# snarkify/sirius

Measured on AMD Instinct MI355X. Metric: IVC fold-steps/s (CycleFold IVC::next hot path, Poseidon-shaped synthetic trace, 2^k rows), higher is better.
Workload: dtype u256 (modular; 9 x 29-bit / 8 x 32-bit limbs)

## Files before the change

include/sirius_amd.h:

```cpp
#ifndef SIRIUS_AMD_H
#define SIRIUS_AMD_H

#include <stddef.h>
#include <stdint.h>

#ifdef __cplusplus
extern "C" {
#endif

typedef struct { uint64_t l[4]; } srs_fe;
typedef struct { srs_fe x, y; } srs_affine;

typedef struct srs_ck srs_ck;
typedef struct srs_structure srs_structure;

enum {
    SRS_OK = 0,
    SRS_ERR_TOO_LONG_INPUT = 1,
    SRS_ERR_NOT_POW2 = 2,
    SRS_ERR_K_TOO_LARGE = 3,
    SRS_ERR_INVALID = 4,
    SRS_ERR_DEVICE = 5,
    SRS_ERR_LAYOUT = 6,
    SRS_ERR_EVAL_INDEX = 7,
    SRS_ERR_IO = 8,
    SRS_ERR_INVALID_DATA = 9,
    SRS_ERR_UNSUPPORTED = 10
};

enum { SRS_CURVE_BN256 = 0, SRS_CURVE_GRUMPKIN = 1 };
enum { SRS_FIELD_FR = 0, SRS_FIELD_FQ = 1 };
enum { SRS_SPACE_HOST = 0, SRS_SPACE_DEVICE = 1 };
enum { SRS_REPR_MONT = 0, SRS_REPR_CANON = 1 };

int srs_init(int device_ordinal);
int srs_init_thread(int device_ordinal);
const char *srs_last_error(void);
const char *srs_version(void);
int srs_tuning_set(const char *name, int64_t value);
int srs_tuning_get(const char *name, int64_t *value);
void srs_tuning_reset(void);
const char *srs_tuning_name(int index);
int srs_scalar_field_of(int curve);
int srs_layout_selftest(int field, const srs_fe *one, const srs_fe *two);
int srs_layout_selftest_point(int curve, const srs_affine *generator);

int srs_dev_alloc(size_t bytes, void **out);
void srs_dev_free(void *p);
int srs_host_alloc(size_t bytes, void **out);
void srs_host_free(void *p);
int srs_upload(void *dst_dev, const void *src_host, size_t bytes, void *stream);
int srs_download(void *dst_host, const void *src_dev, size_t bytes, void *stream);

int srs_ck_create(int curve, const srs_affine *bases, size_t len, int space, srs_ck **out);
int srs_ck_create_sharded(int curve, const srs_affine *bases, size_t len, int space,
                          uint32_t rank, uint32_t world, srs_ck **out);
int srs_ck_setup_synthetic(int curve, size_t len, uint64_t seed, uint32_t rank, uint32_t world, srs_ck **out);
int srs_ck_setup_uniform_bytes(const uint8_t *label, size_t label_len, size_t first, size_t count, uint8_t *out);
int srs_ck_setup(int curve, uint32_t k, const uint8_t *label, size_t label_len, srs_ck **out);
int srs_ck_get_bases(const srs_ck *ck, srs_affine *out);
size_t srs_ck_local_len(const srs_ck *ck);
int srs_ck_load_file(int curve, const char *path, size_t k, uint32_t rank, uint32_t world, srs_ck **out);
int srs_ck_save_file(const srs_ck *ck, const char *path);
int srs_ck_count_off_curve(const srs_ck *ck, size_t *bad);
void srs_ck_free(srs_ck *ck);
size_t srs_ck_len(const srs_ck *ck);

int srs_commit(srs_ck *ck, const srs_fe *scalars, size_t n, int space, int repr, void *stream,
               srs_affine *out);
int srs_commit_batch(srs_ck *ck, const srs_fe *const *scalars, const size_t *n, size_t batch,
                     int space, int repr, void *stream, srs_affine *out);
int srs_commit_upload(srs_ck *ck, const srs_fe *scalars_host, size_t n, srs_fe *dev_copy, int repr, void *stream,
                      srs_affine *out);

size_t srs_concat_len(const size_t *lens, size_t n_columns, size_t pad_size);
int srs_concat_with_padding(srs_fe *out_dev, const srs_fe *const *columns_host, const size_t *lens, size_t n_columns, size_t pad_size,
                            void *stream);
int srs_commit_upload_columns(srs_ck *ck, const srs_fe *const *columns_host, const size_t *lens, size_t n_columns, size_t pad_size,
                              srs_fe *dev_copy, int repr, void *stream, srs_affine *out);

int srs_ck_create_multi(int curve, const srs_affine *bases, size_t len, int space, int n_devices, srs_ck **out);
int srs_ck_setup_synthetic_multi(int curve, size_t len, uint64_t seed, int n_devices, srs_ck **out);
int srs_ck_num_shards(const srs_ck *ck);
int srs_ck_msm_stats(const srs_ck *ck, uint64_t *out4);
int srs_ck_has_wide_table(const srs_ck *ck);
int srs_ck_is_compact(const srs_ck *ck);
size_t srs_ck_table_bytes(const srs_ck *ck);
int srs_glv_constants(int curve, srs_fe *lambda, srs_fe *beta);
int srs_glv_decompose(int curve, const srs_fe *k, int repr, srs_fe *k1_abs, srs_fe *k2_abs, int *neg1, int *neg2);
int srs_ck_shard_stats(const srs_ck *ck, int shard, uint64_t *out4);

int srs_point_sum(int curve, const srs_affine *points, size_t n, srs_affine *out);
int srs_point_mul(int curve, const srs_fe *scalar, int repr, const srs_affine *p, srs_affine *out);
int srs_point_lincomb(int curve, const srs_affine *acc, const srs_affine *points, const srs_fe *scalars, size_t n,
                      int repr, srs_affine *out);
int srs_fe_powers(int field, const srs_fe *r, size_t n, srs_fe *out);
int srs_point_lincomb_async(int curve, const srs_affine *acc, const srs_affine *points, const srs_fe *scalars, size_t n,
                            int repr, srs_affine *out, uint64_t *job);
int srs_job_wait(uint64_t job);

void srs_profile_enable(int on);
void srs_profile_reset(void);
void srs_profile_sampling(unsigned every);
int srs_profile_get(const char *name, double *total_ms, uint64_t *launches, uint64_t *units);

int srs_ntt(int field, srs_fe *a, size_t n, int inverse, int coset, int space, void *stream);
int srs_ntt_batch(int field, srs_fe *a, size_t n, size_t stride, size_t batch, int inverse, int coset,
                  int space, void *stream);
int srs_ntt_set_max_radix_bits(int bits);

enum { SRS_EX_CONST = 0, SRS_EX_POLY = 1, SRS_EX_CHALLENGE = 2, SRS_EX_NEG = 3, SRS_EX_SUM = 4,
       SRS_EX_PRODUCT = 5, SRS_EX_SCALED = 6, SRS_EX_END = 7 };
int srs_structure_create(int field, uint32_t k, size_t num_selectors, size_t num_fixed, size_t num_advice,
                         const uint8_t *const *selectors, const srs_fe *const *fixed, int space,
                         const uint64_t *gates, size_t gates_words, size_t num_gates, srs_structure **out);
int srs_structure_create_lookup(int field, uint32_t k, size_t num_selectors, size_t num_fixed, size_t num_advice,
                                const uint8_t *const *selectors, const srs_fe *const *fixed, int space,
                                const uint64_t *gates, size_t gates_words, size_t num_gates,
                                size_t num_lookups, int has_vector_lookup,
                                const uint64_t *lookup_exprs, size_t lookup_words, srs_structure **out);
void srs_structure_free(srs_structure *S);
int srs_structure_set_shard(srs_structure *S, uint32_t rank, uint32_t world);
int srs_structure_upload_shard_halo(const srs_structure *S, const srs_fe *witness_host, srs_fe *dev_copy, size_t n, int reference_compat,
                                    void *stream);
size_t srs_structure_num_witness_columns(const srs_structure *S);
size_t srs_structure_num_cross_terms(const srs_structure *S);
size_t srs_structure_num_challenges(const srs_structure *S);
size_t srs_structure_program_source(srs_structure *S, int which, char *buf, size_t cap, uint64_t *fingerprint, int *spec_id);
enum { SRS_KERNEL_INTERPRETER = 0, SRS_KERNEL_AHEAD_OF_TIME = 1, SRS_KERNEL_RUNTIME_COMPILED = 2 };
int srs_structure_kernel_kind(const srs_structure *S, int which);
int srs_jit_selfcheck(size_t *code_bytes, char *log, size_t log_cap);

int srs_cross_terms(srs_structure *S, const srs_fe *W1, const srs_fe *W2, const srs_fe *challenges,
                    size_t n_challenges, int space, void *stream, srs_fe *const *T_out);
int srs_commit_cross_terms(srs_structure *S, srs_ck *ck, const srs_fe *W1, const srs_fe *W2,
                           const srs_fe *challenges, size_t n_challenges, int space, void *stream,
                           srs_fe *const *T_out, srs_affine *commits_out);
int srs_eval_gates(srs_structure *S, int homogeneous, const srs_fe *W, const srs_fe *challenges,
                   size_t n_challenges, int space, void *stream, srs_fe *out);

int srs_is_sat_gates(srs_structure *S, int homogeneous, const srs_fe *W, const srs_fe *challenges, size_t n_challenges,
                     const srs_fe *E, int space, void *stream, size_t *mismatch_count);

typedef struct srs_poseidon srs_poseidon;
int srs_poseidon_new(int field, size_t t, size_t rate, size_t r_f, size_t r_p, srs_poseidon **out);
void srs_poseidon_free(srs_poseidon *H);
void srs_poseidon_reset(srs_poseidon *H);
int srs_poseidon_absorb_field(srs_poseidon *H, const srs_fe *v, size_t n);
int srs_poseidon_absorb_point(srs_poseidon *H, int curve, const srs_affine *p);
int srs_poseidon_squeeze(srs_poseidon *H, size_t num_bits, int out_field, srs_fe *out);
int srs_poseidon_squeeze_device(srs_poseidon *H, size_t num_bits, int out_field, srs_fe *out, double *kernel_ms);

typedef struct srs_sparse srs_sparse;
int srs_sparse_create(int field, size_t n, const uint64_t *rows, const uint64_t *cols, const srs_fe *values, size_t nnz,
                      srs_sparse **out);
void srs_sparse_free(srs_sparse *M);
int srs_sparse_matvec(srs_sparse *M, const srs_fe *Z, int space, void *stream, srs_fe *y);
int srs_is_sat_permutation(srs_sparse *M, const srs_fe *Z, int space, void *stream, size_t *mismatch_count);
int srs_is_sat_witness_commit(srs_ck *ck, const srs_fe *const *W, const size_t *n, size_t n_rounds,
                              const srs_affine *W_commitments, const srs_fe *E, size_t n_E, const srs_affine *E_commitment,
                              int space, void *stream, size_t *w_mismatch_count, int *e_mismatch);

int srs_lookup_coeff_1(srs_structure *S, const srs_fe *advice, const srs_fe *r, int space, void *stream,
                       srs_fe *const *ls, srs_fe *const *ts, srs_fe *const *ms);
int srs_lookup_coeff_2(int field, const srs_fe *l, const srs_fe *t, const srs_fe *m, const srs_fe *r, size_t n,
                       int space, void *stream, srs_fe *h, srs_fe *g);
int srs_is_sat_log_derivative(srs_structure *S, const srs_fe *W, int space, void *stream, size_t *mismatch_count);
int srs_batch_invert_assigned(int field, const srs_fe *numerators, const srs_fe *denominators, const uint8_t *has_denominator,
                              size_t n, int space, void *stream, srs_fe *out);

int srs_fold_witness(int field, srs_fe *out, const srs_fe *w1, const srs_fe *w2, const srs_fe *r, size_t n,
                     int space, void *stream);
int srs_fold_error(int field, srs_fe *out, const srs_fe *e, const srs_fe *const *T, size_t n_terms,
                   const srs_fe *r, size_t n, int space, void *stream);

int srs_sangria_prove(srs_structure *S, srs_ck *ck, srs_poseidon *ro, const srs_fe *challenges, size_t n_challenges, srs_fe *W1, const srs_fe *W2,
                      srs_fe *E, void *stream, srs_fe *r_io, srs_fe *const *T_dev, srs_affine *cross_term_commits,
                      const srs_affine *W_commitments, const srs_affine *E_commitment, srs_affine *folded_commitments, uint64_t *jobs);

int srs_sangria_prove_incoming(srs_structure *S, srs_ck *ck, srs_poseidon *ro, const srs_fe *challenges, size_t n_challenges, srs_fe *W1, srs_fe *W2,
                               const srs_fe *W2_host, const srs_fe *u2_tail, size_t n_u2_tail, srs_fe *E, void *stream, srs_fe *r_io,
                               srs_fe *const *T_dev, srs_affine *cross_term_commits, srs_affine *W_commitments, const srs_affine *E_commitment,
                               srs_affine *folded_commitments, uint64_t *jobs);

typedef struct {
    size_t count_of_evaluation_with_padding;
    size_t betas_count;
    size_t fft_points_count_F;
    size_t fft_points_count_G;
    size_t instances_to_fold;
    size_t lagrange_domain;
    uint32_t fft_log_domain_size_K;
} srs_pg_context;
int srs_pg_context_new(const srs_structure *S, size_t traces_len, srs_pg_context *out);
int srs_pg_prove(srs_structure *S, srs_poseidon *ro, const srs_fe *betas, size_t n_betas, const srs_fe *delta,
                 const srs_fe *const *W, const srs_fe *const *challenges, size_t n_challenges, size_t n_instances, int reference_compat,
                 void *stream, srs_fe *alpha_gamma, srs_fe *poly_F, srs_fe *poly_K, srs_fe *betas_stroke, srs_fe *e, srs_fe *lagrange,
                 srs_fe *W_folded);
int srs_pg_beta_stroke(const srs_fe *betas, size_t n, const srs_fe *alpha, const srs_fe *delta, srs_fe *out);
int srs_pg_compute_F(srs_structure *S, const srs_fe *betas, size_t n_betas, const srs_fe *delta, const srs_fe *W,
                     const srs_fe *challenges, size_t n_challenges, int space, int reference_compat, void *stream,
                     srs_fe *poly_F);
int srs_pg_compute_G(srs_structure *S, const srs_fe *betas_stroke, size_t n_betas, const srs_fe *const *W,
                     const srs_fe *const *challenges, size_t n_challenges, size_t n_instances, int space,
                     int reference_compat, void *stream, srs_fe *poly_G);
int srs_pg_compute_K_from_G(const srs_fe *poly_G, size_t n_G, const srs_fe *poly_F_in_alpha, size_t instances_to_fold,
                            uint32_t fft_log_domain_size_K, void *stream, srs_fe *poly_K);
int srs_pg_evaluate_e(srs_structure *S, const srs_fe *betas, size_t n_betas, const srs_fe *W, const srs_fe *challenges,
                      size_t n_challenges, int space, int reference_compat, void *stream, srs_fe *e);
int srs_pg_closed_form(const srs_fe *gate_values, size_t n_gates, uint32_t k, const srs_fe *weights, size_t n_weights,
                       const srs_fe *delta, srs_fe *out);
int srs_pg_calculate_e(const srs_fe *poly_F, size_t n_F, const srs_fe *poly_K, size_t n_K, const srs_fe *gamma,
                       const srs_fe *alpha, uint32_t log_n, srs_fe *out);
int srs_lagrange_eval(const srs_fe *X, uint32_t log_n, srs_fe *out);
int srs_poly_eval(const srs_fe *coeffs, size_t n, const srs_fe *x, srs_fe *out);
int srs_fold_lincomb(int field, srs_fe *out, const srs_fe *const *W, const srs_fe *coefs, size_t J, size_t n,
                     int space, void *stream);
int srs_fold_lincomb_sharded(int field, srs_fe *out, const srs_fe *const *W, const srs_fe *coefs, size_t J, size_t n, uint32_t rank,
                             uint32_t world, void *stream);
int srs_structure_fold_sharded(srs_structure *S, srs_fe *out, const srs_fe *const *W, const srs_fe *coefs, size_t J, int reference_compat,
                               void *stream);

#ifdef __cplusplus
}
#endif
#endif
```

shim/src/sys.rs:

```rust
#![allow(non_camel_case_types, non_snake_case, dead_code)]
use std::os::raw::{c_char, c_int, c_void};

#[repr(C)] #[derive(Clone, Copy, Debug, PartialEq, Eq)] pub struct srs_fe { pub l: [u64; 4] }
#[repr(C)] #[derive(Clone, Copy, Debug, PartialEq, Eq)] pub struct srs_affine { pub x: srs_fe, pub y: srs_fe }
#[repr(C)] pub struct srs_ck { _opaque: [u8; 0] }
#[repr(C)] pub struct srs_structure { _opaque: [u8; 0] }
#[repr(C)] pub struct srs_poseidon { _opaque: [u8; 0] }
#[repr(C)] pub struct srs_sparse { _opaque: [u8; 0] }
#[repr(C)] #[derive(Clone, Copy, Debug, Default)] pub struct srs_pg_context { pub count_of_evaluation_with_padding: usize, pub betas_count: usize, pub fft_points_count_F: usize, pub fft_points_count_G: usize, pub instances_to_fold: usize, pub lagrange_domain: usize, pub fft_log_domain_size_K: u32 }

pub const SRS_OK: c_int = 0;
pub const SRS_ERR_TOO_LONG_INPUT: c_int = 1;
pub const SRS_ERR_NOT_POW2: c_int = 2;
pub const SRS_ERR_K_TOO_LARGE: c_int = 3;
pub const SRS_ERR_INVALID: c_int = 4;
pub const SRS_ERR_DEVICE: c_int = 5;
pub const SRS_ERR_LAYOUT: c_int = 6;
pub const SRS_ERR_EVAL_INDEX: c_int = 7;
pub const SRS_ERR_IO: c_int = 8;
pub const SRS_ERR_INVALID_DATA: c_int = 9;
pub const SRS_ERR_UNSUPPORTED: c_int = 10;
pub const SRS_CURVE_BN256: c_int = 0;
pub const SRS_CURVE_GRUMPKIN: c_int = 1;
pub const SRS_FIELD_FR: c_int = 0;
pub const SRS_FIELD_FQ: c_int = 1;
pub const SRS_SPACE_HOST: c_int = 0;
pub const SRS_SPACE_DEVICE: c_int = 1;
pub const SRS_REPR_MONT: c_int = 0;
pub const SRS_REPR_CANON: c_int = 1;
pub const SRS_EX_CONST: c_int = 0;
pub const SRS_EX_POLY: c_int = 1;
pub const SRS_EX_CHALLENGE: c_int = 2;
pub const SRS_EX_NEG: c_int = 3;
pub const SRS_EX_SUM: c_int = 4;
pub const SRS_EX_PRODUCT: c_int = 5;
pub const SRS_EX_SCALED: c_int = 6;
pub const SRS_EX_END: c_int = 7;
pub const SRS_KERNEL_INTERPRETER: c_int = 0;
pub const SRS_KERNEL_AHEAD_OF_TIME: c_int = 1;
pub const SRS_KERNEL_RUNTIME_COMPILED: c_int = 2;

#[link(name = "sirius_amd")]
extern "C" {
    pub fn srs_init(device_ordinal: c_int) -> c_int;
    pub fn srs_init_thread(device_ordinal: c_int) -> c_int;
    pub fn srs_last_error() -> *const c_char;
    pub fn srs_version() -> *const c_char;
    pub fn srs_tuning_set(name: *const c_char, value: int64_t) -> c_int;
    pub fn srs_tuning_get(name: *const c_char, value: *mut int64_t) -> c_int;
    pub fn srs_tuning_reset();
    pub fn srs_tuning_name(index: c_int) -> *const c_char;
    pub fn srs_scalar_field_of(curve: c_int) -> c_int;
    pub fn srs_layout_selftest(field: c_int, one: *const srs_fe, two: *const srs_fe) -> c_int;
    pub fn srs_layout_selftest_point(curve: c_int, generator: *const srs_affine) -> c_int;
    pub fn srs_dev_alloc(bytes: usize, out: *mut *mut c_void) -> c_int;
    pub fn srs_dev_free(p: *mut c_void);
    pub fn srs_host_alloc(bytes: usize, out: *mut *mut c_void) -> c_int;
    pub fn srs_host_free(p: *mut c_void);
    pub fn srs_upload(dst_dev: *mut c_void, src_host: *const c_void, bytes: usize, stream: *mut c_void) -> c_int;
    pub fn srs_download(dst_host: *mut c_void, src_dev: *const c_void, bytes: usize, stream: *mut c_void) -> c_int;
    pub fn srs_ck_create(curve: c_int, bases: *const srs_affine, len: usize, space: c_int, out: *mut *mut srs_ck) -> c_int;
    pub fn srs_ck_create_sharded(curve: c_int, bases: *const srs_affine, len: usize, space: c_int, rank: u32, world: u32, out: *mut *mut srs_ck) -> c_int;
    pub fn srs_ck_setup_synthetic(curve: c_int, len: usize, seed: u64, rank: u32, world: u32, out: *mut *mut srs_ck) -> c_int;
    pub fn srs_ck_setup_uniform_bytes(label: *const u8, label_len: usize, first: usize, count: usize, out: *mut u8) -> c_int;
    pub fn srs_ck_setup(curve: c_int, k: u32, label: *const u8, label_len: usize, out: *mut *mut srs_ck) -> c_int;
    pub fn srs_ck_get_bases(ck: *const srs_ck, out: *mut srs_affine) -> c_int;
    pub fn srs_ck_local_len(ck: *const srs_ck) -> usize;
    pub fn srs_ck_load_file(curve: c_int, path: *const c_char, k: usize, rank: u32, world: u32, out: *mut *mut srs_ck) -> c_int;
    pub fn srs_ck_save_file(ck: *const srs_ck, path: *const c_char) -> c_int;
    pub fn srs_ck_count_off_curve(ck: *const srs_ck, bad: *mut usize) -> c_int;
    pub fn srs_ck_free(ck: *mut srs_ck);
    pub fn srs_ck_len(ck: *const srs_ck) -> usize;
    pub fn srs_commit(ck: *mut srs_ck, scalars: *const srs_fe, n: usize, space: c_int, repr: c_int, stream: *mut c_void, out: *mut srs_affine) -> c_int;
    pub fn srs_commit_batch(ck: *mut srs_ck, scalars: *const *const srs_fe, n: *const usize, batch: usize, space: c_int, repr: c_int, stream: *mut c_void, out: *mut srs_affine) -> c_int;
    pub fn srs_commit_upload(ck: *mut srs_ck, scalars_host: *const srs_fe, n: usize, dev_copy: *mut srs_fe, repr: c_int, stream: *mut c_void, out: *mut srs_affine) -> c_int;
    pub fn srs_concat_len(lens: *const usize, n_columns: usize, pad_size: usize) -> usize;
    pub fn srs_concat_with_padding(out_dev: *mut srs_fe, columns_host: *const *const srs_fe, lens: *const usize, n_columns: usize, pad_size: usize, stream: *mut c_void) -> c_int;
    pub fn srs_commit_upload_columns(ck: *mut srs_ck, columns_host: *const *const srs_fe, lens: *const usize, n_columns: usize, pad_size: usize, dev_copy: *mut srs_fe, repr: c_int, stream: *mut c_void, out: *mut srs_affine) -> c_int;
    pub fn srs_ck_create_multi(curve: c_int, bases: *const srs_affine, len: usize, space: c_int, n_devices: c_int, out: *mut *mut srs_ck) -> c_int;
    pub fn srs_ck_setup_synthetic_multi(curve: c_int, len: usize, seed: u64, n_devices: c_int, out: *mut *mut srs_ck) -> c_int;
    pub fn srs_ck_num_shards(ck: *const srs_ck) -> c_int;
    pub fn srs_ck_msm_stats(ck: *const srs_ck, out4: *mut u64) -> c_int;
    pub fn srs_ck_has_wide_table(ck: *const srs_ck) -> c_int;
    pub fn srs_ck_is_compact(ck: *const srs_ck) -> c_int;
    pub fn srs_ck_table_bytes(ck: *const srs_ck) -> usize;
    pub fn srs_glv_constants(curve: c_int, lambda: *mut srs_fe, beta: *mut srs_fe) -> c_int;
    pub fn srs_glv_decompose(curve: c_int, k: *const srs_fe, repr: c_int, k1_abs: *mut srs_fe, k2_abs: *mut srs_fe, neg1: *mut c_int, neg2: *mut c_int) -> c_int;
    pub fn srs_ck_shard_stats(ck: *const srs_ck, shard: c_int, out4: *mut u64) -> c_int;
    pub fn srs_point_sum(curve: c_int, points: *const srs_affine, n: usize, out: *mut srs_affine) -> c_int;
    pub fn srs_point_mul(curve: c_int, scalar: *const srs_fe, repr: c_int, p: *const srs_affine, out: *mut srs_affine) -> c_int;
    pub fn srs_point_lincomb(curve: c_int, acc: *const srs_affine, points: *const srs_affine, scalars: *const srs_fe, n: usize, repr: c_int, out: *mut srs_affine) -> c_int;
    pub fn srs_fe_powers(field: c_int, r: *const srs_fe, n: usize, out: *mut srs_fe) -> c_int;
    pub fn srs_point_lincomb_async(curve: c_int, acc: *const srs_affine, points: *const srs_affine, scalars: *const srs_fe, n: usize, repr: c_int, out: *mut srs_affine, job: *mut u64) -> c_int;
    pub fn srs_job_wait(job: u64) -> c_int;
    pub fn srs_profile_enable(on: c_int);
    pub fn srs_profile_reset();
    pub fn srs_profile_sampling(every: unsigned);
    pub fn srs_profile_get(name: *const c_char, total_ms: *mut f64, launches: *mut u64, units: *mut u64) -> c_int;
    pub fn srs_ntt(field: c_int, a: *mut srs_fe, n: usize, inverse: c_int, coset: c_int, space: c_int, stream: *mut c_void) -> c_int;
    pub fn srs_ntt_batch(field: c_int, a: *mut srs_fe, n: usize, stride: usize, batch: usize, inverse: c_int, coset: c_int, space: c_int, stream: *mut c_void) -> c_int;
    pub fn srs_ntt_set_max_radix_bits(bits: c_int) -> c_int;
    pub fn srs_structure_create(field: c_int, k: u32, num_selectors: usize, num_fixed: usize, num_advice: usize, selectors: *const *const u8, fixed: *const *const srs_fe, space: c_int, gates: *const u64, gates_words: usize, num_gates: usize, out: *mut *mut srs_structure) -> c_int;
    pub fn srs_structure_create_lookup(field: c_int, k: u32, num_selectors: usize, num_fixed: usize, num_advice: usize, selectors: *const *const u8, fixed: *const *const srs_fe, space: c_int, gates: *const u64, gates_words: usize, num_gates: usize, num_lookups: usize, has_vector_lookup: c_int, lookup_exprs: *const u64, lookup_words: usize, out: *mut *mut srs_structure) -> c_int;
    pub fn srs_structure_free(S: *mut srs_structure);
    pub fn srs_structure_set_shard(S: *mut srs_structure, rank: u32, world: u32) -> c_int;
    pub fn srs_structure_upload_shard_halo(S: *const srs_structure, witness_host: *const srs_fe, dev_copy: *mut srs_fe, n: usize, reference_compat: c_int, stream: *mut c_void) -> c_int;
    pub fn srs_structure_num_witness_columns(S: *const srs_structure) -> usize;
    pub fn srs_structure_num_cross_terms(S: *const srs_structure) -> usize;
    pub fn srs_structure_num_challenges(S: *const srs_structure) -> usize;
    pub fn srs_structure_program_source(S: *mut srs_structure, which: c_int, buf: *mut c_char, cap: usize, fingerprint: *mut u64, spec_id: *mut c_int) -> usize;
    pub fn srs_structure_kernel_kind(S: *const srs_structure, which: c_int) -> c_int;
    pub fn srs_jit_selfcheck(code_bytes: *mut usize, log: *mut c_char, log_cap: usize) -> c_int;
    pub fn srs_cross_terms(S: *mut srs_structure, W1: *const srs_fe, W2: *const srs_fe, challenges: *const srs_fe, n_challenges: usize, space: c_int, stream: *mut c_void, T_out: *const *mut srs_fe) -> c_int;
    pub fn srs_commit_cross_terms(S: *mut srs_structure, ck: *mut srs_ck, W1: *const srs_fe, W2: *const srs_fe, challenges: *const srs_fe, n_challenges: usize, space: c_int, stream: *mut c_void, T_out: *const *mut srs_fe, commits_out: *mut srs_affine) -> c_int;
    pub fn srs_eval_gates(S: *mut srs_structure, homogeneous: c_int, W: *const srs_fe, challenges: *const srs_fe, n_challenges: usize, space: c_int, stream: *mut c_void, out: *mut srs_fe) -> c_int;
    pub fn srs_is_sat_gates(S: *mut srs_structure, homogeneous: c_int, W: *const srs_fe, challenges: *const srs_fe, n_challenges: usize, E: *const srs_fe, space: c_int, stream: *mut c_void, mismatch_count: *mut usize) -> c_int;
    pub fn srs_poseidon_new(field: c_int, t: usize, rate: usize, r_f: usize, r_p: usize, out: *mut *mut srs_poseidon) -> c_int;
    pub fn srs_poseidon_free(H: *mut srs_poseidon);
    pub fn srs_poseidon_reset(H: *mut srs_poseidon);
    pub fn srs_poseidon_absorb_field(H: *mut srs_poseidon, v: *const srs_fe, n: usize) -> c_int;
    pub fn srs_poseidon_absorb_point(H: *mut srs_poseidon, curve: c_int, p: *const srs_affine) -> c_int;
    pub fn srs_poseidon_squeeze(H: *mut srs_poseidon, num_bits: usize, out_field: c_int, out: *mut srs_fe) -> c_int;
    pub fn srs_poseidon_squeeze_device(H: *mut srs_poseidon, num_bits: usize, out_field: c_int, out: *mut srs_fe, kernel_ms: *mut f64) -> c_int;
    pub fn srs_sparse_create(field: c_int, n: usize, rows: *const u64, cols: *const u64, values: *const srs_fe, nnz: usize, out: *mut *mut srs_sparse) -> c_int;
    pub fn srs_sparse_free(M: *mut srs_sparse);
    pub fn srs_sparse_matvec(M: *mut srs_sparse, Z: *const srs_fe, space: c_int, stream: *mut c_void, y: *mut srs_fe) -> c_int;
    pub fn srs_is_sat_permutation(M: *mut srs_sparse, Z: *const srs_fe, space: c_int, stream: *mut c_void, mismatch_count: *mut usize) -> c_int;
    pub fn srs_is_sat_witness_commit(ck: *mut srs_ck, W: *const *const srs_fe, n: *const usize, n_rounds: usize, W_commitments: *const srs_affine, E: *const srs_fe, n_E: usize, E_commitment: *const srs_affine, space: c_int, stream: *mut c_void, w_mismatch_count: *mut usize, e_mismatch: *mut c_int) -> c_int;
    pub fn srs_lookup_coeff_1(S: *mut srs_structure, advice: *const srs_fe, r: *const srs_fe, space: c_int, stream: *mut c_void, ls: *const *mut srs_fe, ts: *const *mut srs_fe, ms: *const *mut srs_fe) -> c_int;
    pub fn srs_lookup_coeff_2(field: c_int, l: *const srs_fe, t: *const srs_fe, m: *const srs_fe, r: *const srs_fe, n: usize, space: c_int, stream: *mut c_void, h: *mut srs_fe, g: *mut srs_fe) -> c_int;
    pub fn srs_is_sat_log_derivative(S: *mut srs_structure, W: *const srs_fe, space: c_int, stream: *mut c_void, mismatch_count: *mut usize) -> c_int;
    pub fn srs_batch_invert_assigned(field: c_int, numerators: *const srs_fe, denominators: *const srs_fe, has_denominator: *const u8, n: usize, space: c_int, stream: *mut c_void, out: *mut srs_fe) -> c_int;
    pub fn srs_fold_witness(field: c_int, out: *mut srs_fe, w1: *const srs_fe, w2: *const srs_fe, r: *const srs_fe, n: usize, space: c_int, stream: *mut c_void) -> c_int;
    pub fn srs_fold_error(field: c_int, out: *mut srs_fe, e: *const srs_fe, T: *const *const srs_fe, n_terms: usize, r: *const srs_fe, n: usize, space: c_int, stream: *mut c_void) -> c_int;
    pub fn srs_sangria_prove(S: *mut srs_structure, ck: *mut srs_ck, ro: *mut srs_poseidon, challenges: *const srs_fe, n_challenges: usize, W1: *mut srs_fe, W2: *const srs_fe, E: *mut srs_fe, stream: *mut c_void, r_io: *mut srs_fe, T_dev: *const *mut srs_fe, cross_term_commits: *mut srs_affine, W_commitments: *const srs_affine, E_commitment: *const srs_affine, folded_commitments: *mut srs_affine, jobs: *mut u64) -> c_int;
    pub fn srs_sangria_prove_incoming(S: *mut srs_structure, ck: *mut srs_ck, ro: *mut srs_poseidon, challenges: *const srs_fe, n_challenges: usize, W1: *mut srs_fe, W2: *mut srs_fe, W2_host: *const srs_fe, u2_tail: *const srs_fe, n_u2_tail: usize, E: *mut srs_fe, stream: *mut c_void, r_io: *mut srs_fe, T_dev: *const *mut srs_fe, cross_term_commits: *mut srs_affine, W_commitments: *mut srs_affine, E_commitment: *const srs_affine, folded_commitments: *mut srs_affine, jobs: *mut u64) -> c_int;
    pub fn srs_pg_context_new(S: *const srs_structure, traces_len: usize, out: *mut srs_pg_context) -> c_int;
    pub fn srs_pg_prove(S: *mut srs_structure, ro: *mut srs_poseidon, betas: *const srs_fe, n_betas: usize, delta: *const srs_fe, W: *const *const srs_fe, challenges: *const *const srs_fe, n_challenges: usize, n_instances: usize, reference_compat: c_int, stream: *mut c_void, alpha_gamma: *mut srs_fe, poly_F: *mut srs_fe, poly_K: *mut srs_fe, betas_stroke: *mut srs_fe, e: *mut srs_fe, lagrange: *mut srs_fe, W_folded: *mut srs_fe) -> c_int;
    pub fn srs_pg_beta_stroke(betas: *const srs_fe, n: usize, alpha: *const srs_fe, delta: *const srs_fe, out: *mut srs_fe) -> c_int;
    pub fn srs_pg_compute_F(S: *mut srs_structure, betas: *const srs_fe, n_betas: usize, delta: *const srs_fe, W: *const srs_fe, challenges: *const srs_fe, n_challenges: usize, space: c_int, reference_compat: c_int, stream: *mut c_void, poly_F: *mut srs_fe) -> c_int;
    pub fn srs_pg_compute_G(S: *mut srs_structure, betas_stroke: *const srs_fe, n_betas: usize, W: *const *const srs_fe, challenges: *const *const srs_fe, n_challenges: usize, n_instances: usize, space: c_int, reference_compat: c_int, stream: *mut c_void, poly_G: *mut srs_fe) -> c_int;
    pub fn srs_pg_compute_K_from_G(poly_G: *const srs_fe, n_G: usize, poly_F_in_alpha: *const srs_fe, instances_to_fold: usize, fft_log_domain_size_K: u32, stream: *mut c_void, poly_K: *mut srs_fe) -> c_int;
    pub fn srs_pg_evaluate_e(S: *mut srs_structure, betas: *const srs_fe, n_betas: usize, W: *const srs_fe, challenges: *const srs_fe, n_challenges: usize, space: c_int, reference_compat: c_int, stream: *mut c_void, e: *mut srs_fe) -> c_int;
    pub fn srs_pg_closed_form(gate_values: *const srs_fe, n_gates: usize, k: u32, weights: *const srs_fe, n_weights: usize, delta: *const srs_fe, out: *mut srs_fe) -> c_int;
    pub fn srs_pg_calculate_e(poly_F: *const srs_fe, n_F: usize, poly_K: *const srs_fe, n_K: usize, gamma: *const srs_fe, alpha: *const srs_fe, log_n: u32, out: *mut srs_fe) -> c_int;
    pub fn srs_lagrange_eval(X: *const srs_fe, log_n: u32, out: *mut srs_fe) -> c_int;
    pub fn srs_poly_eval(coeffs: *const srs_fe, n: usize, x: *const srs_fe, out: *mut srs_fe) -> c_int;
    pub fn srs_fold_lincomb(field: c_int, out: *mut srs_fe, W: *const *const srs_fe, coefs: *const srs_fe, J: usize, n: usize, space: c_int, stream: *mut c_void) -> c_int;
    pub fn srs_fold_lincomb_sharded(field: c_int, out: *mut srs_fe, W: *const *const srs_fe, coefs: *const srs_fe, J: usize, n: usize, rank: u32, world: u32, stream: *mut c_void) -> c_int;
    pub fn srs_structure_fold_sharded(S: *mut srs_structure, out: *mut srs_fe, W: *const *const srs_fe, coefs: *const srs_fe, J: usize, reference_compat: c_int, stream: *mut c_void) -> c_int;
}
```

sirius_amd/_lib.py:

```python
import ctypes as C
import os

_HERE = os.path.dirname(os.path.abspath(__file__))
LIB_PATH = os.path.join(_HERE, "csrc", "libsirius_amd.so")

OK, ERR_TOO_LONG_INPUT, ERR_NOT_POW2, ERR_K_TOO_LARGE, ERR_INVALID, ERR_DEVICE, ERR_LAYOUT, ERR_EVAL_INDEX, ERR_IO, ERR_INVALID_DATA, ERR_UNSUPPORTED = range(11)
CURVE_BN256, CURVE_GRUMPKIN = 0, 1
FIELD_FR, FIELD_FQ = 0, 1
SPACE_HOST, SPACE_DEVICE = 0, 1
REPR_MONT, REPR_CANON = 0, 1

_lib = None


class SiriusAmdError(RuntimeError):
    def __init__(self, rc, msg):
        super().__init__(f"sirius_amd rc={rc}: {msg}")
        self.rc = rc


def _prototypes():
    vp, sz, i32, u32 = C.c_void_p, C.c_size_t, C.c_int, C.c_uint32
    return {
        "srs_init": (i32, [i32]),
        "srs_init_thread": (i32, [i32]),
        "srs_last_error": (C.c_char_p, []),
        "srs_version": (C.c_char_p, []),
        "srs_tuning_set": (i32, [C.c_char_p, C.c_int64]),
        "srs_tuning_get": (i32, [C.c_char_p, C.POINTER(C.c_int64)]),
        "srs_tuning_reset": (None, []),
        "srs_tuning_name": (C.c_char_p, [i32]),
        "srs_scalar_field_of": (i32, [i32]),
        "srs_layout_selftest": (i32, [i32, vp, vp]),
        "srs_layout_selftest_point": (i32, [i32, vp]),
        "srs_dev_alloc": (i32, [sz, C.POINTER(vp)]),
        "srs_dev_free": (None, [vp]),
        "srs_host_alloc": (i32, [sz, C.POINTER(vp)]),
        "srs_host_free": (None, [vp]),
        "srs_upload": (i32, [vp, vp, sz, vp]),
        "srs_download": (i32, [vp, vp, sz, vp]),
        "srs_commit_upload": (i32, [vp, vp, sz, vp, i32, vp, vp]),
        "srs_concat_len": (sz, [C.POINTER(sz), sz, sz]),
        "srs_concat_with_padding": (i32, [vp, C.POINTER(vp), C.POINTER(sz), sz, sz, vp]),
        "srs_commit_upload_columns": (i32, [vp, C.POINTER(vp), C.POINTER(sz), sz, sz, vp, i32, vp, vp]),
        "srs_ck_create_multi": (i32, [i32, vp, sz, i32, i32, C.POINTER(vp)]),
        "srs_ck_setup_synthetic_multi": (i32, [i32, sz, C.c_uint64, i32, C.POINTER(vp)]),
        "srs_ck_num_shards": (i32, [vp]),
        "srs_ck_msm_stats": (i32, [vp, C.POINTER(C.c_uint64)]),
        "srs_ck_has_wide_table": (i32, [vp]),
        "srs_ck_is_compact": (i32, [vp]),
        "srs_ck_table_bytes": (sz, [vp]),
        "srs_glv_constants": (i32, [i32, vp, vp]),
        "srs_glv_decompose": (i32, [i32, vp, i32, vp, vp, C.POINTER(i32), C.POINTER(i32)]),
        "srs_ck_shard_stats": (i32, [vp, i32, C.POINTER(C.c_uint64)]),
        "srs_structure_kernel_kind": (i32, [vp, i32]),
        "srs_ck_create": (i32, [i32, vp, sz, i32, C.POINTER(vp)]),
        "srs_ck_create_sharded": (i32, [i32, vp, sz, i32, u32, u32, C.POINTER(vp)]),
        "srs_ck_setup_synthetic": (i32, [i32, sz, C.c_uint64, u32, u32, C.POINTER(vp)]),
        "srs_ck_setup_uniform_bytes": (i32, [C.c_char_p, sz, sz, sz, vp]),
        "srs_ck_setup": (i32, [i32, u32, C.c_char_p, sz, C.POINTER(vp)]),
        "srs_ck_get_bases": (i32, [vp, vp]),
        "srs_ck_local_len": (sz, [vp]),
        "srs_point_lincomb": (i32, [i32, vp, vp, vp, sz, i32, vp]),
        "srs_point_lincomb_async": (i32, [i32, vp, vp, vp, sz, i32, vp, C.POINTER(C.c_uint64)]),
        "srs_job_wait": (i32, [C.c_uint64]),
        "srs_fe_powers": (i32, [i32, vp, sz, vp]),
        "srs_jit_selfcheck": (i32, [C.POINTER(sz), C.c_char_p, sz]),
        "srs_profile_enable": (None, [i32]),
        "srs_profile_reset": (None, []),
        "srs_profile_sampling": (None, [C.c_uint]),
        "srs_profile_get": (i32, [C.c_char_p, C.POINTER(C.c_double), C.POINTER(C.c_uint64), C.POINTER(C.c_uint64)]),
        "srs_ck_load_file": (i32, [i32, C.c_char_p, sz, u32, u32, C.POINTER(vp)]),
        "srs_ck_save_file": (i32, [vp, C.c_char_p]),
        "srs_ck_count_off_curve": (i32, [vp, C.POINTER(sz)]),
        "srs_is_sat_gates": (i32, [vp, i32, vp, vp, sz, vp, i32, vp, C.POINTER(sz)]),
        "srs_ck_free": (None, [vp]),
        "srs_ck_len": (sz, [vp]),
        "srs_commit": (i32, [vp, vp, sz, i32, i32, vp, vp]),
        "srs_commit_batch": (i32, [vp, C.POINTER(vp), C.POINTER(sz), sz, i32, i32, vp, vp]),
        "srs_point_sum": (i32, [i32, vp, sz, vp]),
        "srs_point_mul": (i32, [i32, vp, i32, vp, vp]),
        "srs_structure_create": (i32, [i32, u32, sz, sz, sz, C.POINTER(vp), C.POINTER(vp), i32, vp, sz, sz, C.POINTER(vp)]),
        "srs_structure_create_lookup": (i32, [i32, u32, sz, sz, sz, C.POINTER(vp), C.POINTER(vp), i32, vp, sz, sz, sz, i32, vp, sz,
                                              C.POINTER(vp)]),
        "srs_structure_num_witness_columns": (sz, [vp]),
        "srs_lookup_coeff_1": (i32, [vp, vp, vp, i32, vp, C.POINTER(vp), C.POINTER(vp), C.POINTER(vp)]),
        "srs_lookup_coeff_2": (i32, [i32, vp, vp, vp, vp, sz, i32, vp, vp, vp]),
        "srs_is_sat_log_derivative": (i32, [vp, vp, i32, vp, C.POINTER(sz)]),
        "srs_sparse_create": (i32, [i32, sz, vp, vp, vp, sz, C.POINTER(vp)]),
        "srs_sparse_free": (None, [vp]),
        "srs_sparse_matvec": (i32, [vp, vp, i32, vp, vp]),
        "srs_is_sat_permutation": (i32, [vp, vp, i32, vp, C.POINTER(sz)]),
        "srs_is_sat_witness_commit": (i32, [vp, C.POINTER(vp), C.POINTER(sz), sz, vp, vp, sz, vp, i32, vp, C.POINTER(sz), C.POINTER(i32)]),
        "srs_structure_set_shard": (i32, [vp, u32, u32]),
        "srs_structure_upload_shard_halo": (i32, [vp, vp, vp, sz, i32, vp]),
        "srs_poseidon_new": (i32, [i32, sz, sz, sz, sz, C.POINTER(vp)]),
        "srs_poseidon_free": (None, [vp]),
        "srs_poseidon_reset": (None, [vp]),
        "srs_poseidon_absorb_field": (i32, [vp, vp, sz]),
        "srs_poseidon_absorb_point": (i32, [vp, i32, vp]),
        "srs_poseidon_squeeze": (i32, [vp, sz, i32, vp]),
        "srs_poseidon_squeeze_device": (i32, [vp, sz, i32, vp, C.POINTER(C.c_double)]),
        "srs_batch_invert_assigned": (i32, [i32, vp, vp, vp, sz, i32, vp, vp]),
        "srs_structure_free": (None, [vp]),
        "srs_structure_num_cross_terms": (sz, [vp]),
        "srs_structure_num_challenges": (sz, [vp]),
        "srs_structure_program_source": (sz, [vp, i32, vp, sz, C.POINTER(C.c_uint64), C.POINTER(i32)]),
        "srs_cross_terms": (i32, [vp, vp, vp, vp, sz, i32, vp, C.POINTER(vp)]),
        "srs_commit_cross_terms": (i32, [vp, vp, vp, vp, vp, sz, i32, vp, C.POINTER(vp), vp]),
        "srs_eval_gates": (i32, [vp, i32, vp, vp, sz, i32, vp, vp]),
        "srs_fold_witness": (i32, [i32, vp, vp, vp, vp, sz, i32, vp]),
        "srs_fold_error": (i32, [i32, vp, vp, C.POINTER(vp), sz, vp, sz, i32, vp]),
        "srs_pg_context_new": (i32, [vp, sz, vp]),
        "srs_pg_beta_stroke": (i32, [vp, sz, vp, vp, vp]),
        "srs_pg_prove": (i32, [vp, vp, vp, sz, vp, C.POINTER(vp), C.POINTER(vp), sz, sz, i32, vp, vp, vp, vp, vp, vp, vp, vp]),
        "srs_sangria_prove": (i32, [vp, vp, vp, vp, sz, vp, vp, vp, vp, vp, C.POINTER(vp), vp, vp, vp, vp, C.POINTER(C.c_uint64)]),
        "srs_sangria_prove_incoming": (i32, [vp, vp, vp, vp, sz, vp, vp, vp, vp, sz, vp, vp, vp, C.POINTER(vp), vp, vp, vp, vp,
                                             C.POINTER(C.c_uint64)]),
        "srs_pg_compute_F": (i32, [vp, vp, sz, vp, vp, vp, sz, i32, i32, vp, vp]),
        "srs_pg_compute_G": (i32, [vp, vp, sz, C.POINTER(vp), C.POINTER(vp), sz, sz, i32, i32, vp, vp]),
        "srs_pg_compute_K_from_G": (i32, [vp, sz, vp, sz, u32, vp, vp]),
        "srs_pg_evaluate_e": (i32, [vp, vp, sz, vp, vp, sz, i32, i32, vp, vp]),
        "srs_pg_closed_form": (i32, [vp, sz, u32, vp, sz, vp, vp]),
        "srs_pg_calculate_e": (i32, [vp, sz, vp, sz, vp, vp, u32, vp]),
        "srs_lagrange_eval": (i32, [vp, u32, vp]),
        "srs_poly_eval": (i32, [vp, sz, vp, vp]),
        "srs_fold_lincomb": (i32, [i32, vp, C.POINTER(vp), vp, sz, sz, i32, vp]),
        "srs_fold_lincomb_sharded": (i32, [i32, vp, C.POINTER(vp), vp, sz, sz, u32, u32, vp]),
        "srs_structure_fold_sharded": (i32, [vp, vp, vp, vp, sz, i32, vp]),
        "srs_ntt": (i32, [i32, vp, sz, i32, i32, i32, vp]),
        "srs_ntt_set_max_radix_bits": (i32, [i32]),
        "srs_ntt_batch": (i32, [i32, vp, sz, sz, sz, i32, i32, i32, vp]),
    }


def load(path=None):
    global _lib
    if _lib is not None and path is None:
        return _lib
    p = path or os.environ.get("SRS_AMD_LIB") or LIB_PATH
    if not os.path.exists(p):
        raise ImportError(
            f"{p} not found: build the HIP extension first (__graft_entry__.build()); "
            "sirius_amd has no CPU fallback")
    if path is None:
        try:
            import torch
        except Exception:
            pass
    lib = C.CDLL(p)
    for name, (res, args) in _prototypes().items():
        fn = getattr(lib, name)
        fn.restype = res
        fn.argtypes = args
    _lib = lib
    for item in filter(None, os.environ.get("SRS_TEST_TUNING", "").split(",")):
        name, _, value = item.partition("=")
        if lib.srs_tuning_set(name.strip().encode(), int(value)) != 0:
            raise ValueError(f"SRS_TEST_TUNING: unknown tunable {name!r}")
    return lib


def lib():
    return load()


def check(rc):
    if rc != OK:
        raise SiriusAmdError(rc, (lib().srs_last_error() or b"").decode())
```

sirius_amd/commitment.py:

```python
import ctypes as C

import numpy as np

from . import _lib as L


class TooLongInput(ValueError):

    def __init__(self, input_len, limit):
        super().__init__(f"Can't commit too long input: input len: {input_len}, but limit is {limit}")
        self.input_len, self.limit = input_len, limit


def _is_torch(x):
    return type(x).__module__.startswith("torch")


def _buf(x, last):
    if _is_torch(x):
        assert x.is_contiguous() and x.shape[-1] == last and x.element_size() == 8, (x.shape, x.dtype)
        space = L.SPACE_DEVICE if x.is_cuda else L.SPACE_HOST
        return x.data_ptr(), space, x.numel() // last, x
    a = np.ascontiguousarray(x, dtype=np.uint64)
    assert a.shape[-1] == last, a.shape
    return a.ctypes.data, L.SPACE_HOST, a.size // last, a


_torch_cuda = None


def _stream():
    global _torch_cuda
    if _torch_cuda is None:
        try:
            import torch
            if not torch.cuda.is_available():
                return None
            _torch_cuda = torch.cuda
        except Exception:
            return None
    return _torch_cuda.current_stream().cuda_stream


class CommitmentKey:

    def __init__(self, curve, bases, rank=0, world=1):
        addr, space, n, keep = _buf(bases, 8)
        self.curve, self._len = curve, n
        self.rank, self.world = rank, world
        h = C.c_void_p()
        L.check(L.lib().srs_ck_create_sharded(curve, addr, n, space, rank, world, C.byref(h)))
        self._h = h

    @classmethod
    def setup_synthetic(cls, curve, n, seed=0, rank=0, world=1):
        self = cls.__new__(cls)
        self.curve, self._len, self.rank, self.world = curve, n, rank, world
        h = C.c_void_p()
        L.check(L.lib().srs_ck_setup_synthetic(curve, n, seed, rank, world, C.byref(h)))
        self._h = h
        return self

    @staticmethod
    def setup_uniform_bytes(label, first, count):
        out = np.zeros((count, 32), dtype=np.uint8)
        L.check(L.lib().srs_ck_setup_uniform_bytes(bytes(label), len(label), first, count, out.ctypes.data))
        return out

    @classmethod
    def setup(cls, curve, k, label):
        assert k < 32
        h = C.c_void_p()
        L.check(L.lib().srs_ck_setup(curve, k, bytes(label), len(label), C.byref(h)))
        raise AssertionError("srs_ck_setup returned OK")

    @classmethod
    def create_multi(cls, curve, bases, n_devices=0):
        addr, space, n, keep = _buf(bases, 8)
        self = cls.__new__(cls)
        self.curve, self._len, self.rank, self.world = curve, n, 0, 1
        h = C.c_void_p()
        L.check(L.lib().srs_ck_create_multi(curve, addr, n, space, n_devices, C.byref(h)))
        self._h = h
        return self

    @classmethod
    def setup_synthetic_multi(cls, curve, n, seed=0, n_devices=0):
        self = cls.__new__(cls)
        self.curve, self._len, self.rank, self.world = curve, n, 0, 1
        h = C.c_void_p()
        L.check(L.lib().srs_ck_setup_synthetic_multi(curve, n, seed, n_devices, C.byref(h)))
        self._h = h
        return self

    @property
    def num_shards(self):
        return L.lib().srs_ck_num_shards(self._h)

    def msm_stats(self):
        out = (C.c_uint64 * 4)()
        L.check(L.lib().srs_ck_msm_stats(self._h, out))
        return dict(slot_sets=int(out[0]), hot_sets=int(out[1]), redo=int(out[2]), other_sets=int(out[3]))

    def shard_stats(self, shard):
        out = (C.c_uint64 * 4)()
        L.check(L.lib().srs_ck_shard_stats(self._h, shard, out))
        return dict(h2d_bytes=int(out[0]), peer_bytes=int(out[1]), streamed_commits=int(out[2]), device=int(out[3]))

    def has_wide_table(self):
        return bool(L.lib().srs_ck_has_wide_table(self._h))

    def is_compact(self):
        return bool(L.lib().srs_ck_is_compact(self._h))

    def table_bytes(self):
        return int(L.lib().srs_ck_table_bytes(self._h))

    @classmethod
    def load_from_file(cls, curve, file_path, k, rank=0, world=1):
        self = cls.__new__(cls)
        self.curve, self._len, self.rank, self.world = curve, 1 << k, rank, world
        h = C.c_void_p()
        rc = L.lib().srs_ck_load_file(curve, str(file_path).encode(), k, rank, world, C.byref(h))
        if rc == L.ERR_IO:
            raise IOError(L.lib().srs_last_error().decode())
        if rc == L.ERR_INVALID_DATA:
            raise ValueError(L.lib().srs_last_error().decode())
        L.check(rc)
        self._h = h
        return self

    def save_to_file(self, file_path):
        rc = L.lib().srs_ck_save_file(self._h, str(file_path).encode())
        if rc == L.ERR_IO:
            raise IOError(L.lib().srs_last_error().decode())
        L.check(rc)

    @classmethod
    def load_or_setup_cache(cls, curve, cache_folder, label, k, setup=None):
        import os
        path = os.path.join(str(cache_folder), label, f"{k}.bin")
        if os.path.exists(path):
            return cls.load_from_file(curve, path, k)
        if setup is None:
            raise FileNotFoundError(path)
        key = setup(k)
        os.makedirs(os.path.dirname(path), exist_ok=True)
        key.save_to_file(path)
        return key

    def count_off_curve(self):
        n = C.c_size_t()
        L.check(L.lib().srs_ck_count_off_curve(self._h, C.byref(n)))
        return n.value

    def bases(self):
        n = L.lib().srs_ck_local_len(self._h)
        out = np.zeros((n, 8), dtype=np.uint64)
        L.check(L.lib().srs_ck_get_bases(self._h, out.ctypes.data))
        return out

    def __len__(self):
        return self._len

    def close(self):
        if getattr(self, "_h", None):
            L.lib().srs_ck_free(self._h)
            self._h = None

    def __del__(self):
        try:
            self.close()
        except Exception:
            pass

    def commit(self, v, repr=L.REPR_MONT):
        addr, space, n, keep = _buf(v, 4)
        if n > self._len:
            raise TooLongInput(n, self._len)
        out = np.zeros(8, dtype=np.uint64)
        L.check(L.lib().srs_commit(self._h, addr, n, space, repr, _stream(), out.ctypes.data))
        return out

    def commit_upload(self, v_host, dev_copy=None, repr=L.REPR_MONT):
        a = np.ascontiguousarray(v_host, dtype=np.uint64)
        assert a.shape[-1] == 4
        n = a.size // 4
        if n > self._len:
            raise TooLongInput(n, self._len)
        dptr = None
        if dev_copy is not None:
            assert _is_torch(dev_copy) and dev_copy.is_contiguous() and dev_copy.numel() == 4 * n
            dptr = dev_copy.data_ptr()
        out = np.zeros(8, dtype=np.uint64)
        L.check(L.lib().srs_commit_upload(self._h, a.ctypes.data, n, dptr, repr, _stream(), out.ctypes.data))
        return out

    def commit_upload_columns(self, columns, pad_size, dev_copy=None, repr=L.REPR_MONT):
        cols = [np.ascontiguousarray(c, dtype=np.uint64).reshape(-1, 4) for c in columns]
        lens = (C.c_size_t * max(len(cols), 1))(*[c.shape[0] for c in cols])
        ptrs = (C.c_void_p * max(len(cols), 1))(*[c.ctypes.data for c in cols])
        n = L.lib().srs_concat_len(lens, len(cols), pad_size)
        if n > self._len:
            raise TooLongInput(n, self._len)
        dptr = None
        if dev_copy is not None:
            assert _is_torch(dev_copy) and dev_copy.is_contiguous() and dev_copy.numel() == 4 * n
            dptr = dev_copy.data_ptr()
        out = np.zeros(8, dtype=np.uint64)
        L.check(L.lib().srs_commit_upload_columns(self._h, ptrs, lens, len(cols), pad_size, dptr, repr, _stream(), out.ctypes.data))
        return out

    def commit_batch(self, vs, repr=L.REPR_MONT):
        bufs = [_buf(v, 4) for v in vs]
        if not bufs:
            return np.zeros((0, 8), dtype=np.uint64)
        spaces = {b[1] for b in bufs}
        assert len(spaces) == 1, "all vectors of a batch must live in the same memory space"
        for b in bufs:
            if b[2] > self._len:
                raise TooLongInput(b[2], self._len)
        ptrs = (C.c_void_p * len(bufs))(*[b[0] for b in bufs])
        ns = (C.c_size_t * len(bufs))(*[b[2] for b in bufs])
        out = np.zeros((len(bufs), 8), dtype=np.uint64)
        L.check(L.lib().srs_commit_batch(self._h, ptrs, ns, len(bufs), spaces.pop(), repr, _stream(), out.ctypes.data))
        return out


def point_sum(curve, points):
    a = np.ascontiguousarray(points, dtype=np.uint64).reshape(-1, 8)
    out = np.zeros(8, dtype=np.uint64)
    L.check(L.lib().srs_point_sum(curve, a.ctypes.data, a.shape[0], out.ctypes.data))
    return out


def point_lincomb(curve, acc, points, scalars, repr=L.REPR_MONT):
    pts = np.ascontiguousarray(points, dtype=np.uint64).reshape(-1, 8)
    sc = np.ascontiguousarray(scalars, dtype=np.uint64).reshape(-1, 4)
    assert pts.shape[0] == sc.shape[0]
    a = None if acc is None else np.ascontiguousarray(acc, dtype=np.uint64).reshape(8)
    out = np.zeros(8, dtype=np.uint64)
    L.check(L.lib().srs_point_lincomb(curve, None if a is None else a.ctypes.data, pts.ctypes.data, sc.ctypes.data,
                                      pts.shape[0], repr, out.ctypes.data))
    return out


class PendingPoint:

    def __init__(self, job, out, lib):
        self._job, self._out, self._lib = job, out, lib

    def wait(self):
        if self._job is not None:
            L.check(self._lib.srs_job_wait(self._job))
            self._job = None
# ... 61 lines not shown
```

sirius_amd/csrc/capi.hip:

```cpp
#include "../../include/sirius_amd.h"

#include <cstdio>
#include <cstring>
#include <deque>
#include <map>
#include <memory>
#include <set>
#include <thread>
#include <condition_variable>
#include <functional>
#include <mutex>
#include <atomic>
#include <chrono>
#include <string>
#include <vector>

#include "curve.cuh"
#include "decider.h"
#include "devrt.h"
#include "msm.h"
#include "ntt.h"
#include "poseidon.h"
#include "prof.h"
#include "rowprog.h"
// ... 624 lines not shown

static int read_shard_bases(const msm::Key &key, hipStream_t st, srs_affine *out) {
    if (!key.len) return SRS_OK;
    affine_t *tmp = nullptr;
    SRS_HIP_CHECK(hipMalloc((void **)&tmp, key.len * sizeof(affine_t)));
    try {
        msm::read_bases(key, tmp, st);
        SRS_HIP_CHECK(hipMemcpyAsync(out, tmp, key.len * sizeof(affine_t), hipMemcpyDeviceToHost, st));
        SRS_HIP_CHECK(hipStreamSynchronize(st));
    } catch (...) {
        (void)hipFree(tmp);
        throw;
    }
    (void)hipFree(tmp);
    return SRS_OK;
}

int srs_ck_get_bases(const srs_ck *ck, srs_affine *out) {
    if (!ck || ((ck->key.len || !ck->shards.empty()) && !out)) return fail(SRS_ERR_INVALID, "srs_ck_get_bases: bad argument");
    int rc = ensure_device();
    if (rc) return rc;
    if (!ck->shards.empty()) {
        return guarded([&]() -> int {
            const uint32_t world = (uint32_t)ck->shards.size();
            for (uint32_t d = 0; d < world; ++d) {
                CkShard *sh = ck->shards[d].get();
                std::vector<srs_affine> loc(sh->key.len);
                SRS_HIP_CHECK(hipSetDevice(sh->device));
                read_shard_bases(sh->key, sh->stream, loc.data());
                Stripes{d, world}.each_piece(0, ck->key.global_len, [&](size_t g, size_t l, size_t cnt) {
                    std::memcpy(out + g, loc.data() + l, cnt * sizeof(srs_affine));
                });
            }
            return ensure_device();
        });
    }
    return guarded([&]() -> int {
        if (ck->key.len) {
            affine_t *tmp = nullptr;
            SRS_HIP_CHECK(hipMalloc((void **)&tmp, ck->key.len * sizeof(affine_t)));
            try {
                msm::read_bases(ck->key, tmp, nullptr);
                SRS_HIP_CHECK(hipMemcpy(out, tmp, ck->key.len * sizeof(affine_t), hipMemcpyDeviceToHost));
            } catch (...) {
                (void)hipFree(tmp);
                throw;
            }
            (void)hipFree(tmp);
        }
        return SRS_OK;
    });
}
size_t srs_ck_local_len(const srs_ck *ck) { return ck ? (ck->shards.empty() ? ck->key.len : ck->key.global_len) : 0; }

int srs_ck_load_file(int curve, const char *path, size_t k, uint32_t rank, uint32_t world, srs_ck **out) {
    if (!valid_curve(curve) || !path || !out) return fail(SRS_ERR_INVALID, "srs_ck_load_file: bad argument");
    if (k > 27) return fail(SRS_ERR_INVALID, "srs_ck_load_file: key longer than 2^27 bases");
    const size_t len = (size_t)1 << k;
    std::vector<srs_affine> host;
    int rc = guarded([&]() -> int {
        host.resize(len);
        FILE *f = std::fopen(path, "rb");
        if (!f) return fail(SRS_ERR_IO, std::string("srs_ck_load_file: cannot open ") + path);
        size_t got = std::fread(host.data(), sizeof(srs_affine), len, f);
        std::fclose(f);
        if (got != len) return fail(SRS_ERR_IO, "srs_ck_load_file: failed to fill whole buffer");
        return SRS_OK;
    });
    if (rc) return rc;
    srs_ck *ck = nullptr;
    rc = srs_ck_create_sharded(curve, host.data(), len, SRS_SPACE_HOST, rank, world, &ck);
    if (rc) return rc;
    size_t bad = 0;
    rc = srs_ck_count_off_curve(ck, &bad);
    if (rc == SRS_OK && bad) rc = fail(SRS_ERR_INVALID_DATA, "Wrong file in cache, some ptr out of curve");
    if (rc) { srs_ck_free(ck); return rc; }
    *out = ck;
    return SRS_OK;
}

int srs_ck_save_file(const srs_ck *ck, const char *path) {
    if (!ck || !path) return fail(SRS_ERR_INVALID, "srs_ck_save_file: bad argument");
    if (ck->key.world != 1) return fail(SRS_ERR_INVALID, "srs_ck_save_file: sharded key");
    std::vector<srs_affine> host(srs_ck_local_len(ck));
    int rc = srs_ck_get_bases(ck, host.data());
    if (rc) return rc;
    FILE *f = std::fopen(path, "wb");
    if (!f) return fail(SRS_ERR_IO, std::string("srs_ck_save_file: cannot create ") + path);
    size_t put = std::fwrite(host.data(), sizeof(srs_affine), host.size(), f);
    int cl = std::fclose(f);
    if (put != host.size() || cl != 0) return fail(SRS_ERR_IO, "srs_ck_save_file: short write");
    return SRS_OK;
}

int srs_ck_count_off_curve(const srs_ck *ck, size_t *bad) {
    if (!ck || !bad) return fail(SRS_ERR_INVALID, "srs_ck_count_off_curve: bad argument");
    int rc = ensure_device();
    if (rc) return rc;
    return guarded([&]() -> int {
        if (ck->shards.empty()) {
            *bad = msm::count_off_curve(ck->key, nullptr);
            return SRS_OK;
        }
        size_t total = 0;
        for (auto &sp : ck->shards) {
            SRS_HIP_CHECK(hipSetDevice(sp->device));
            total += msm::count_off_curve(sp->key, sp->stream);
        }
        *bad = total;
        return ensure_device();
    });
}

int srs_ck_create(int curve, const srs_affine *bases, size_t len, int space, srs_ck **out) {
    return srs_ck_create_sharded(curve, bases, len, space, 0, 1, out);
}

int srs_ck_create_multi(int curve, const srs_affine *bases, size_t len, int space, int n_devices, srs_ck **out) {
    if (!valid_curve(curve) || !out || (!bases && len) || n_devices < 0) return fail(SRS_ERR_INVALID, "srs_ck_create_multi: bad argument");
    if (len > ((size_t)1 << 27)) return fail(SRS_ERR_INVALID, "srs_ck_create_multi: key longer than 2^27 bases");
    int rc = ensure_device();
    if (rc) return rc;
    return guarded([&]() -> int {
        return create_multi(curve, len, n_devices, [&](CkShard &sh) {
            const hipMemcpyKind kind = space == SRS_SPACE_DEVICE ? hipMemcpyDeviceToDevice : hipMemcpyHostToDevice;
            Stripes{sh.key.rank, sh.key.world}.each_piece(0, len, [&](size_t g, size_t l, size_t cnt) {
                SRS_HIP_CHECK(hipMemcpyAsync(sh.key.table + l, bases + g, cnt * sizeof(affine_t), kind, sh.stream));
            });
        }, out);
    });
}
int srs_ck_setup_synthetic_multi(int curve, size_t len, uint64_t seed, int n_devices, srs_ck **out) {
    if (!valid_curve(curve) || !out || n_devices < 0) return fail(SRS_ERR_INVALID, "srs_ck_setup_synthetic_multi: bad argument");
    if (len > ((size_t)1 << 27)) return fail(SRS_ERR_INVALID, "srs_ck_setup_synthetic_multi: key longer than 2^27 bases");
    int rc = ensure_device();
    if (rc) return rc;
    return guarded([&]() -> int {
        return create_multi(curve, len, n_devices, [&](CkShard &sh) { msm::generate_bases(sh.key, seed, sh.stream); }, out);
    });
}
int srs_ck_num_shards(const srs_ck *ck) { return ck ? (ck->shards.empty() ? 1 : (int)ck->shards.size()) : 0; }
int srs_ck_msm_stats(const srs_ck *ck, uint64_t *out) {
    if (!ck || !out) return fail(SRS_ERR_INVALID, "srs_ck_msm_stats: bad argument");
    for (int i = 0; i < 4; ++i) out[i] = 0;
    auto add = [&](const msm::Key &k) {
        out[0] += k.stat_slot_sets;
        out[1] += k.stat_hot_sets;
        out[2] += k.stat_redo;
        out[3] += k.stat_other_sets;
    };
    if (ck->shards.empty()) add(ck->key);
    for (const auto &sh : ck->shards) add(sh->key);
    return SRS_OK;
}

int srs_ck_shard_stats(const srs_ck *ck, int shard, uint64_t *out) {
    if (!ck || !out || shard < 0) return fail(SRS_ERR_INVALID, "srs_ck_shard_stats: bad argument");
    for (int i = 0; i < 4; ++i) out[i] = 0;
    if (ck->shards.empty()) {
        if (shard != 0) return fail(SRS_ERR_INVALID, "srs_ck_shard_stats: no such shard");
        out[3] = (uint64_t)home_device();
        return SRS_OK;
    }
    if ((size_t)shard >= ck->shards.size()) return fail(SRS_ERR_INVALID, "srs_ck_shard_stats: no such shard");
    const CkShard *sh = ck->shards[shard].get();
    out[0] = sh->stat_h2d_bytes;
    out[1] = sh->stat_peer_bytes;
    out[2] = sh->stat_streamed;
    out[3] = (uint64_t)sh->device;
    return SRS_OK;
}

int srs_ck_has_wide_table(const srs_ck *ck) {
    if (!ck) return 0;
    if (ck->shards.empty()) return ck->key.table_w != nullptr ? 1 : 0;
    for (const auto &sh : ck->shards)
        if (sh->key.len && !sh->key.table_w) return 0;
    return 1;
}

int srs_ck_is_compact(const srs_ck *ck) {
    if (!ck) return 0;
    if (ck->shards.empty()) return ck->key.compact ? 1 : 0;
    for (const auto &sh : ck->shards)
        if (!sh->key.compact) return 0;
    return 1;
}
size_t srs_ck_table_bytes(const srs_ck *ck) {
    if (!ck) return 0;
    if (ck->shards.empty()) return msm::table_bytes(ck->key);
    size_t total = 0;
    for (const auto &sh : ck->shards) total += msm::table_bytes(sh->key);
    return total;
}

int srs_glv_constants(int curve, srs_fe *lambda, srs_fe *beta) {
    if (!valid_curve(curve) || !lambda || !beta) return fail(SRS_ERR_INVALID, "srs_glv_constants: bad argument");
    auto go = [&](auto tag) {
        using K = GlvConsts<decltype(tag)::ID>;
        fe_t l, b;
        for (int i = 0; i < 8; ++i) {
            l.v[i] = K::lambda(i);
            b.v[i] = K::beta(i);
        }
        std::memcpy(lambda, &l, 32);
        std::memcpy(beta, &b, 32);
    };
    if (curve == SRS_CURVE_BN256) go(Bn256{}); else go(Grumpkin{});
    return SRS_OK;
}
int srs_glv_decompose(int curve, const srs_fe *k, int repr, srs_fe *k1_abs, srs_fe *k2_abs, int *neg1, int *neg2) {
    if (!valid_curve(curve) || !k || !k1_abs || !k2_abs || !neg1 || !neg2) return fail(SRS_ERR_INVALID, "srs_glv_decompose: bad argument");
    auto go = [&](auto tag) {
        using C = decltype(tag);
        fe_t s;
        std::memcpy(&s, k, 32);
        if (repr == SRS_REPR_MONT) s = C::S::from_mont(s);
        const glv_t g = glv_decompose<C>(s);
        fe_t a, b;
        for (int i = 0; i < 8; ++i) {
            a.v[i] = i < 4 ? g.k1[i] : 0u;
            b.v[i] = i < 4 ? g.k2[i] : 0u;
        }
        std::memcpy(k1_abs, &a, 32);
        std::memcpy(k2_abs, &b, 32);
        *neg1 = g.neg1 ? 1 : 0;
        *neg2 = g.neg2 ? 1 : 0;
    };
    if (curve == SRS_CURVE_BN256) go(Bn256{}); else go(Grumpkin{});
    return SRS_OK;
}

void srs_ck_free(srs_ck *ck) {
    if (!ck) return;
    if (!ck->shards.empty()) {
        free_shards(ck);
        (void)ensure_device();
    }
    for (hipEvent_t e : ck->events) (void)hipEventDestroy(e);
    if (ck->copy_stream) (void)hipStreamDestroy(ck->copy_stream);
    if (ck->key.table) (void)hipFree(ck->key.table);
    msm::release(ck->key);
    ck->staging.release();
    delete ck;
}

size_t srs_ck_len(const srs_ck *ck) { return ck ? ck->key.global_len : 0; }

int srs_commit_batch(srs_ck *ck, const srs_fe *const *scalars, const size_t *n, size_t batch, int space,
                     int repr, void *stream, srs_affine *out) {
    if (!ck || !out || (batch && (!scalars || !n))) return fail(SRS_ERR_INVALID, "srs_commit: bad argument");
    if (batch == 0) return SRS_OK;
    std::lock_guard<std::recursive_mutex> key_lock(ck->mu);
    for (size_t m = 0; m < batch; ++m) {
        if (n[m] > ck->key.global_len)
            return fail(SRS_ERR_TOO_LONG_INPUT, "Can't commit too long input: input len: " + std::to_string(n[m]) +
                                                    ", but limit is " + std::to_string(ck->key.global_len));
        if (n[m] && !scalars[m]) return fail(SRS_ERR_INVALID, "srs_commit: null scalar vector");
    }
    int rc = ensure_device();
    if (rc) return rc;
    if (!ck->shards.empty()) {
        return guarded([&]() -> int {
            hipStream_t st = (hipStream_t)stream;
            hipEvent_t ready = nullptr;
            if (space == SRS_SPACE_DEVICE) {
                if (ck->events.empty()) { hipEvent_t e; SRS_HIP_CHECK(hipEventCreateWithFlags(&e, hipEventDisableTiming)); ck->events.push_back(e); }
                ready = ck->events[0];
                SRS_HIP_CHECK(hipEventRecord(ready, st));
            }
            std::vector<xyzz_t> res(batch);
            int mrc = multi_commit(ck, scalars, n, batch, space, repr, ready, res.data());
            if (mrc) return mrc;
            std::vector<affine_t> aff(batch);
            to_affine_batch(ck->key.curve, res.data(), aff.data(), batch);
            std::memcpy(out, aff.data(), batch * sizeof(affine_t));
            return SRS_OK;
        });
    }
    return guarded([&]() -> int {
        hipStream_t st = (hipStream_t)stream;
        const uint32_t world = ck->key.world, rank = ck->key.rank;
        std::vector<uint32_t> nloc(batch);
        std::vector<const fe_t *> dptr(batch);
        for (size_t m = 0; m < batch; ++m) nloc[m] = (uint32_t)Stripes{rank, world}.count(n[m]);
        if (space == SRS_SPACE_DEVICE) {
            for (size_t m = 0; m < batch; ++m) dptr[m] = reinterpret_cast<const fe_t *>(scalars[m]);
        } else {
            size_t total = 0;
            for (size_t m = 0; m < batch; ++m) total += Arena::pad(n[m] * sizeof(fe_t));
            ck->staging.reserve(total + 256);
            ck->staging.reset();
            for (size_t m = 0; m < batch; ++m) {
                fe_t *d = ck->staging.take<fe_t>(n[m] ? n[m] : 1);
                if (n[m]) SRS_HIP_CHECK(hipMemcpyAsync(d, scalars[m], n[m] * sizeof(fe_t), hipMemcpyHostToDevice, st));
                dptr[m] = d;
            }
        }
        std::vector<xyzz_t> res(batch);
        msm::run(ck->key, dptr.data(), nloc.data(), (uint32_t)batch, repr == SRS_REPR_MONT, st, res.data());
        std::vector<affine_t> aff(batch);
        to_affine_batch(ck->key.curve, res.data(), aff.data(), batch);
        std::memcpy(out, aff.data(), batch * sizeof(affine_t));
        return SRS_OK;
    });
}
// ... 1651 lines not shown
```

sirius_amd/csrc/curve29.cuh:

```cuda
#pragma once
#include "curve.cuh"
#include "field29.cuh"

namespace srs {

struct aff29_t {
    f29_t x, y;
};
struct xyzz29_t {
    f29_t x, y, zz, zzz;
};

template <int K>
SRS_D f29_t quad_bcast29(const f29_t &x) {
    f29_t o;
    quad_bcast_words<K, 9>(x.v, o.v);
    return o;
}
SRS_D f29_t quad_select29(uint32_t q, f29_t a0, f29_t a1, f29_t a2, f29_t a3) {
    f29_t o;
#pragma unroll
    for (int i = 0; i < 9; ++i) {
        uint32_t x = a0.v[i];
        x = q == 1 ? a1.v[i] : x;
// ... 131 lines not shown
            return o;
        }
        f29_t u2 = F::mul(a.zz, q.x);
        f29_t s2 = F::mul(a.zzz, q.y);
        f29_t p = F::normalize(F::template sub_lazy<10, 0>(u2, a.x));
        f29_t rpos = F::template sub_lazy<6, 0>(s2, a.y);
        f29_t rneg = F::template neg_lazy<8, 1>(F::add_lazy(s2, a.y));
        f29_t r = F::normalize(F::select(neg, rneg, rpos));
        f29_t pp = F::sqr(p);
        f29_t rr = F::sqr(r);
        if (F::is_zero_mod(pp)) {
            if (F::is_zero_mod(rr)) {
                aff29_t qq = q;
                if (neg) qq.y = F::normalize(F::template neg_lazy<1, 0>(q.y));
                xyzz29_t d = dbl_affine(qq);
                d.y = F::normalize(d.y);
                return d;
            }
            return identity();
        }
        f29_t ppp = F::mul(p, pp);
        f29_t qv = F::mul(a.x, pp);
        xyzz29_t o;
        f29_t sub = F::add_lazy(ppp, F::add_lazy(qv, qv));
        o.x = F::normalize(F::template sub_lazy<7, 2>(rr, sub));
        f29_t t = F::normalize(F::template sub_lazy<10, 0>(qv, o.x));
        f29_t yn = F::template neg_lazy<6, 0>(a.y);
        o.y = F::mul2(t, r, yn, ppp);
        o.zz = F::mul(a.zz, pp);
        o.zzz = F::mul(a.zzz, ppp);
        return o;
    }
    SRS_HD static xyzz29_t madd_signed_fast(const xyzz29_t &a, const aff29_t &q, bool neg, bool &exc) {
        f29_t u2 = F::mul(a.zz, q.x);
        f29_t s2 = F::mul(a.zzz, q.y);
        f29_t p = F::normalize(F::template sub_lazy<10, 0>(u2, a.x));
        f29_t rpos = F::template sub_lazy<6, 0>(s2, a.y);
        f29_t rneg = F::template neg_lazy<8, 1>(F::add_lazy(s2, a.y));
        f29_t r = F::normalize(F::select(neg, rneg, rpos));
        f29_t pp = F::sqr(p);
        f29_t rr = F::sqr(r);
        exc = exc || F::is_zero_mod(pp) || F::is_zero_exact(q.y) || F::is_zero_exact(a.zz);
        f29_t ppp = F::mul(p, pp);
        f29_t qv = F::mul(a.x, pp);
        xyzz29_t o;
        f29_t sub = F::add_lazy(ppp, F::add_lazy(qv, qv));
        o.x = F::normalize(F::template sub_lazy<7, 2>(rr, sub));
        f29_t t = F::normalize(F::template sub_lazy<10, 0>(qv, o.x));
        f29_t yn = F::template neg_lazy<6, 0>(a.y);
        o.y = F::mul2(t, r, yn, ppp);
        o.zz = F::mul(a.zz, pp);
        o.zzz = F::mul(a.zzz, ppp);
        return o;
    }
    SRS_HD static aff29_t load_raw(const affine_t &q) {
        aff29_t o;
        o.x = F::unpack(q.x);
        o.y = F::unpack(q.y);
        return o;
    }

    SRS_HD static xyzz29_t unpack(const xyzz_t &p) {
        xyzz29_t o;
        o.x = F::unpack(p.x);
        o.y = F::unpack(p.y);
        o.zz = F::unpack(p.zz);
        o.zzz = F::unpack(p.zzz);
        return o;
    }
    SRS_HD static xyzz_t pack(const xyzz29_t &a) {
        xyzz_t o;
        o.x = F::to_canonical_fe(F::reduce_lazy(F::normalize(a.x)));
        o.y = F::to_canonical_fe(F::reduce_lazy(F::normalize(a.y)));
        o.zz = F::to_canonical_fe(a.zz);
        o.zzz = F::to_canonical_fe(a.zzz);
        return o;
    }
    SRS_HD static xyzz29_t dbl(const xyzz29_t &a) {
        if (is_identity(a)) return a;
        xyzz29_t o;
        const f29_t yn = F::normalize(a.y);
        const f29_t u = F::add_lazy(yn, yn);
        const f29_t v = F::sqr(u);
        const f29_t w = F::mul(u, v);
        const f29_t s = F::mul(a.x, v);
        const f29_t xx = F::sqr(a.x);
        const f29_t m = F::normalize(F::add_lazy(F::add_lazy(xx, xx), xx));
        const f29_t mm = F::sqr(m);
        o.x = F::normalize(F::template sub_lazy<5, 1>(mm, F::add_lazy(s, s)));
        const f29_t t = F::template sub_lazy<8, 0>(s, o.x);
        const f29_t m1 = F::mul(t, m);
        const f29_t m2 = F::mul(yn, w);
        o.y = F::template sub_lazy<3, 0>(m1, m2);
        o.zz = F::mul(v, a.zz);
        o.zzz = F::mul(w, a.zzz);
        return o;
    }
    SRS_HD static xyzz29_t add(const xyzz29_t &a, const xyzz29_t &b) {
        if (is_identity(b)) return a;
        if (is_identity(a)) return b;
        const f29_t u1 = F::mul(a.x, b.zz);
        const f29_t u2 = F::mul(b.x, a.zz);
        const f29_t s1 = F::mul(a.y, b.zzz);
        const f29_t s2 = F::mul(b.y, a.zzz);
        const f29_t p = F::normalize(F::template sub_lazy<3, 0>(u2, u1));
        const f29_t r = F::normalize(F::template sub_lazy<3, 0>(s2, s1));
        const f29_t pp = F::sqr(p);
        const f29_t rr = F::sqr(r);
        if (F::is_zero_mod(pp)) {
            if (F::is_zero_mod(rr)) return dbl(a);
            return identity();
        }
        const f29_t ppp = F::mul(p, pp);
        const f29_t qv = F::mul(u1, pp);
        xyzz29_t o;
        o.x = F::normalize(F::template sub_lazy<7, 2>(rr, F::add_lazy(ppp, F::add_lazy(qv, qv))));
        const f29_t t = F::template sub_lazy<10, 0>(qv, o.x);
        const f29_t m1 = F::mul(t, r);
        const f29_t m2 = F::mul(s1, ppp);
        o.y = F::template sub_lazy<3, 0>(m1, m2);
        o.zz = F::mul(F::mul(a.zz, b.zz), pp);
        o.zzz = F::mul(F::mul(a.zzz, b.zzz), ppp);
        return o;
    }

    SRS_D static xyzz29_t add_quad(const xyzz29_t &a, const xyzz29_t &b, uint32_t q) {
        const bool ia = is_identity(a), ib = is_identity(b);
        xyzz29_t o;
        if (ia || ib) {
            o.x = F::select(ib, a.x, b.x);
            o.y = F::select(ib, a.y, b.y);
            o.zz = F::select(ib, a.zz, b.zz);
            o.zzz = F::select(ib, a.zzz, b.zzz);
            return o;
        }
        const f29_t m1 = F::mul(quad_select29(q, a.x, b.x, a.y, b.y), quad_select29(q, b.zz, a.zz, b.zzz, a.zzz));
        const f29_t u1 = quad_bcast29<0>(m1), u2 = quad_bcast29<1>(m1), s1 = quad_bcast29<2>(m1), s2 = quad_bcast29<3>(m1);
        const f29_t p = F::normalize(F::template sub_lazy<3, 0>(u2, u1)), r = F::normalize(F::template sub_lazy<3, 0>(s2, s1));
        const f29_t m2 = F::mul(quad_select29(q, p, r, a.zz, a.zzz), quad_select29(q, p, r, b.zz, b.zzz));
        const f29_t pp = quad_bcast29<0>(m2), rr = quad_bcast29<1>(m2), zzz12 = quad_bcast29<3>(m2);
        const f29_t m3 = F::mul(quad_select29(q, p, u1, m2, p), pp);
        const f29_t ppp = quad_bcast29<0>(m3), qv = quad_bcast29<1>(m3), zz3 = quad_bcast29<2>(m3);
        const f29_t x3 = F::normalize(F::template sub_lazy<7, 2>(rr, F::add_lazy(ppp, F::add_lazy(qv, qv))));
        const f29_t m4 = F::mul(quad_select29(q, F::template sub_lazy<10, 0>(qv, x3), s1, zzz12, s1), quad_select29(q, r, ppp, ppp, ppp));
        const f29_t t2 = quad_bcast29<0>(m4), t1 = quad_bcast29<1>(m4), zzz3 = quad_bcast29<2>(m4);
        o.x = x3;
        o.y = F::template sub_lazy<3, 0>(t2, t1);
        o.zz = zz3;
        o.zzz = zzz3;
        if (F::is_zero_mod(pp)) o = F::is_zero_mod(rr) ? dbl(a) : identity();
        return o;
    }

    SRS_HD static xyzz_t to_xyzz(const xyzz29_t &a) {
        f29_t c;
#pragma unroll
        for (int i = 0; i < 9; ++i) c.v[i] = r256_limb(i);
        xyzz_t o;
        o.x = F::to_canonical_fe(F::mul(a.x, c));
        o.y = F::to_canonical_fe(F::mul(a.y, c));
        o.zz = F::to_canonical_fe(F::mul(a.zz, c));
        o.zzz = F::to_canonical_fe(F::mul(a.zzz, c));
        return o;
    }
    SRS_HD static affine_t table_form(const affine_t &q) {
        using G = typename C::F;
        fe_t c = G::one();
        for (int d = 0; d < 5; ++d) c = G::dbl(c);
        affine_t o;
        o.x = G::mul(q.x, c);
        o.y = G::mul(q.y, c);
        return o;
    }
};

}
```

sirius_amd/csrc/msm.h:

```cpp
#pragma once
#include "curve.cuh"
#include "devrt.h"
#include "glv.cuh"
#include "stripes.h"
#include "tuning.h"

#include <cstdlib>

namespace srs {
namespace msm {

constexpr int WBITS = 16;
constexpr int NWIN = 16;
constexpr int NWIN_COMPACT = 8;
constexpr uint32_t PAY_ENDO = 1u << 30;
constexpr uint32_t NBUCKET = 1u << (WBITS - 1);

constexpr uint32_t SORT_THREADS = 1024;
constexpr uint32_t SORT_TILE_MIN = 8192;
constexpr uint32_t SORT_TARGET_BLOCKS = 256;
constexpr uint32_t SEG = 128, SEG_BUCKETS = NBUCKET / SEG;
constexpr uint32_t SORT_TILE2 = 8192;
constexpr uint64_t TWO_PASS_MIN_SLOTS = 1ull << 23;
constexpr uint32_t PLAN_THREADS = 1024;
constexpr uint32_t ACC_THREADS = 256;
constexpr uint32_t ACC_L0_LOG = 4, ACC_L0 = 1u << ACC_L0_LOG;
constexpr uint32_t ACC_L1_LOG = 3, ACC_L1 = 1u << ACC_L1_LOG;
constexpr uint32_t FINAL_THREADS = 256;
constexpr uint32_t FINAL_FANIN = 512;
constexpr int MAX_LEVELS = 8;
constexpr uint32_t RED_ROWS = 256;
constexpr uint32_t RED_COLS = NBUCKET / RED_ROWS;
constexpr uint32_t RED_THREADS = 4 * RED_COLS;
constexpr uint32_t ACC1_QUAD_MAX = 1u << 17;
constexpr uint32_t BATCH_ARGS = 16;
constexpr uint32_t LANDING_SLOTS = 16;
constexpr uint32_t NORM_G = 16;
constexpr uint32_t SLOT_LOG = 6;
constexpr uint32_t SLOT_L0_MIN_LOG = 2, SLOT_L0_MAX_LOG = 16;
constexpr int WBITS_W = 20;
constexpr int NWIN_W = 13;
constexpr uint32_t NSEG_W = 16;
constexpr uint32_t WIDE_THREADS = 256, WIDE_PER = 2, WIDE_TILE = WIDE_THREADS * WIDE_PER;
constexpr uint32_t WIDE_MIN_KEY_LOG = 23;
constexpr uint32_t WIDE_MIN_N_LOG = 23;

static_assert(RED_ROWS == 256 && RED_COLS == 128, "k_rowcol lane layout");
static_assert(NBUCKET % PLAN_THREADS == 0, "k_plan tiling");

inline bool expect_ovf_initial() { return tuning::get_or(tuning::MSM_EXPECT_OVF, 1) != 0; }

struct Key {
    int curve = 0;
    size_t len = 0;
    size_t global_len = 0;
    uint32_t rank = 0, world = 1;
    bool compact = false;
    bool compact_scalars = false;
    affine_t *table = nullptr;
    affine_t *table_w = nullptr;
    uint64_t stat_slot_sets = 0, stat_hot_sets = 0, stat_redo = 0, stat_other_sets = 0;
    uint64_t last_entries = 0;
    uint64_t last_scalars = 0;

    Arena arena;
    void *h_result = nullptr;
    struct Landing { bool wide = false, slot_mode = false, ovf_on = false; uint32_t batch = 0; } landing[LANDING_SLOTS];
    xyzz_t *fold_buckets = nullptr;
    xyzz_t *slots = nullptr;
    size_t slots_pts = 0;
    uint8_t *used = nullptr;
    uint32_t *h_ovf = nullptr;
    uint32_t slot_s = 0;
    uint32_t seq = 0;
    bool commit_ovf = false;
    bool expect_ovf = expect_ovf_initial();
    uint32_t cold_streak = 0;
};

int choose_windows(Key &k);
void build_table(Key &k, hipStream_t stream);
size_t table_bytes(const Key &k);
void release(Key &k);
void generate_bases(Key &k, uint64_t seed, hipStream_t stream);

void read_bases(const Key &k, affine_t *out_dev, hipStream_t stream);

size_t count_off_curve(const Key &k, hipStream_t stream);

size_t workspace_bytes(uint32_t n_max, uint32_t batch);

void run(Key &k, const fe_t *const *scalars_dev, const uint32_t *n_host, uint32_t batch, int is_mont,
         hipStream_t stream, xyzz_t *result_host);

enum Fold { FOLD_NONE = 0, FOLD_FIRST = 1, FOLD_MIDDLE = 2, FOLD_LAST = 3 };
bool enqueue(Key &k, const fe_t *const *scalars_dev, const uint32_t *n_host, const uint32_t *base_host, uint32_t batch, int is_mont,
             hipStream_t stream, uint32_t slot, Fold fold = FOLD_NONE);
void finish(Key &k, uint32_t batch, uint32_t slot, bool launched, xyzz_t *result_host);
void reserve(Key &k, uint32_t n_max, uint32_t batch);
bool overflow_missed(const Key &k, uint32_t slot);
void note_commit(Key &k, const uint32_t *slots_used, uint32_t n_slots, uint64_t scalars);

}
}
```

sirius_amd/csrc/msm.hip:

```cpp
#define SRS_F29_CHAIN 1
#include "msm.h"
#include "tuning.h"
#include "curve29.cuh"
#include "prof.h"

#include <algorithm>
#include <cstdlib>
#include <numeric>
#include <vector>

namespace srs {
namespace msm {

__device__ __forceinline__ uint32_t upper_bucket(const uint32_t *__restrict__ tp, uint32_t t) {
    uint32_t lo = 0, hi = NBUCKET;
    while (hi - lo > 1) {
        uint32_t mid = (lo + hi) >> 1;
        if (tp[mid] <= t) lo = mid; else hi = mid;
    }
    return lo;
}

template <class C>
__global__ void k_table_step(const affine_t *__restrict__ prev, xyzz_t *__restrict__ tmp, uint32_t n, int nbits) {
// ... 911 lines not shown
    __shared__ uint32_t tile[NBUCKET + NBUCKET / PER];
    __shared__ uint32_t lds[64];
    const uint32_t t = threadIdx.x, m = blockIdx.x, role = blockIdx.y;
    const uint32_t *cnt = count + (size_t)m * NBUCKET;
    uint32_t *pl = plan + (size_t)m * plan_stride;
    {
        uint32_t c[PER];
#pragma unroll
        for (uint32_t j = 0; j < PER; ++j) c[j] = cnt[t + j * PLAN_THREADS];
#pragma unroll
        for (uint32_t j = 0; j < PER; ++j) {
            const uint32_t i = t + j * PLAN_THREADS;
            tile[i + i / PER] = c[j];
        }
    }
    __syncthreads();
    const uint32_t base = t * PER + t;
    uint32_t local = 0;
#pragma unroll 8
    for (uint32_t j = 0; j < PER; ++j) local += tile[base + j];
    uint32_t total_entries;
    uint32_t run = block_exclusive_scan(local, lds, &total_entries);
    const uint32_t l0_log = slot_l0_log(total_entries, S, want_cap);
    uint32_t total = total_entries;
    const bool dense = role == (uint32_t)nlevels + 1;
    const uint32_t lv = role >= 2 && !dense ? role - 1 : 0;
    auto value = [&](uint32_t c) -> uint32_t {
        if (role == 0) return c;
        uint32_t p = (c + (1u << l0_log) - 1) >> l0_log;
        if (dense) return p;
        p = p > S - 1 ? p - (S - 1) : 0u;
        for (uint32_t l = 0; l < lv; ++l) p = (p + (1u << l1_log) - 1) >> l1_log;
        return p;
    };
    if (role != 0) {
        local = 0;
        uint32_t mx = 0;
#pragma unroll 4
        for (uint32_t j = 0; j < PER; ++j) {
            const uint32_t c = tile[base + j];
            local += value(c);
            if (!dense) {
                const uint32_t p = (c + (1u << l0_log) - 1) >> l0_log, o = p > S - 1 ? p - (S - 1) : 0u;
                mx = o > mx ? o : mx;
            }
        }
        if (!dense) {
            uint32_t p = block_max(mx, lds);
            int needed = 1;
            while (p > FINAL_FANIN && needed < nlevels) {
                p = (p + (1u << l1_log) - 1) >> l1_log;
                ++needed;
            }
            if (role == 1 && t == 0) {
                pl[plan_stride - 4] = (uint32_t)needed;
                pl[plan_stride - 3] = 0;
                pl[plan_stride - 2] = l0_log;
            }
            if ((int)role - 1 >= needed) return;
        }
        run = block_exclusive_scan(local, lds, &total);
    }
    static_assert(PER == 32, "k_plan_s: used[] travels as 2 x uint4 per thread");
    uint32_t was_w[8] = {0, 0, 0, 0, 0, 0, 0, 0}, now_w[8] = {0, 0, 0, 0, 0, 0, 0, 0};
    if (dense && !first) {
        const uint4 *up = reinterpret_cast<const uint4 *>(used_prev + (size_t)m * NBUCKET + (size_t)t * PER);
        const uint4 a = up[0], b = up[1];
        was_w[0] = a.x; was_w[1] = a.y; was_w[2] = a.z; was_w[3] = a.w; was_w[4] = b.x; was_w[5] = b.y; was_w[6] = b.z; was_w[7] = b.w;
    }
#pragma unroll
    for (uint32_t j = 0; j < PER; ++j) {
        const uint32_t c = tile[base + j], v = value(c);
        tile[base + j] = run;
        run += v;
        if (dense) {
            const uint32_t now = v < S - 1 ? v : S - 1, was = (was_w[j >> 2] >> (8 * (j & 3))) & 0xFFu;
            now_w[j >> 2] |= (now > was ? now : was) << (8 * (j & 3));
        }
    }
    if (dense) {
        uint4 *un = reinterpret_cast<uint4 *>(used_next + (size_t)m * NBUCKET + (size_t)t * PER);
        uint4 lo, hi;
        lo.x = now_w[0]; lo.y = now_w[1]; lo.z = now_w[2]; lo.w = now_w[3];
        hi.x = now_w[4]; hi.y = now_w[5]; hi.z = now_w[6]; hi.w = now_w[7];
        un[0] = lo;
        un[1] = hi;
    }
    __syncthreads();
    uint32_t *o = pl + (size_t)role * (NBUCKET + 1);
    uint32_t *cur = cursor + (size_t)m * NBUCKET;
    for (uint32_t i = t; i < NBUCKET; i += PLAN_THREADS) {
        const uint32_t v = tile[i + i / PER];
        o[i] = v;
        if (role == 0) cur[i] = v;
    }
    if (t == PLAN_THREADS - 1) {
        o[NBUCKET] = total;
        if (role == 1) {
            pl[plan_stride - 1] = total;
            h_ovf[m] = total;
        }
        if (role == 0) h_ovf[(size_t)LANDING_SLOTS * BATCH_ARGS + m] = total;
    }
}

__global__ void k_link(const uint32_t *__restrict__ plan, size_t plan_stride, int nlevels, Link *__restrict__ link) {
    const uint32_t t = threadIdx.x;
    for (int l = 0; l < nlevels; ++l) {
        uint32_t c = 0;
        if (t < NSEG_W) {
            const uint32_t *pl = plan + (size_t)t * plan_stride;
            if ((uint32_t)l < pl[plan_stride - 4]) c = pl[(size_t)(l + 1) * (NBUCKET + 1) + NBUCKET];
        }
        uint32_t x = c;
#pragma unroll
        for (uint32_t d = 1; d < NSEG_W; d <<= 1) {
            uint32_t y = __shfl_up(x, d, 64);
            if (t >= d) x += y;
        }
        if (t < NSEG_W) link->base[l][t] = x - c;
        if (t == NSEG_W - 1) link->base[l][NSEG_W] = x;
    }
}

__global__ void SRS_KERNEL_BOUNDS(256, 1)
    k_expand(const uint32_t *__restrict__ plan, size_t plan_stride, uint16_t *__restrict__ tb, size_t tb_stride,
             const Link *__restrict__ link, uint32_t arr ) {
    const uint32_t m = blockIdx.y, lane = threadIdx.x & 63u;
    const uint32_t b = blockIdx.x * 4 + (threadIdx.x >> 6);
    const uint32_t *tp = plan + (size_t)m * plan_stride + (size_t)arr * (NBUCKET + 1);
    uint16_t *out = tb + (link ? (size_t)link->base[0][m] : (size_t)m * tb_stride);
    const uint32_t s = tp[b], e = tp[b + 1];
    for (uint32_t t = s + lane; t < e; t += 64) out[t] = (uint16_t)b;
}

template <class C, bool COMPACT>
__device__ __forceinline__ aff29_t load_entry(const affine_t &p, uint32_t v) {
    aff29_t q = Ec29<C>::load_raw(p);
    if (COMPACT) {
        if (v & PAY_ENDO) {
            f29_t beta;
#pragma unroll
            for (int i = 0; i < 9; ++i) beta.v[i] = GlvConsts<C::ID>::beta29(i);
            q.x = Ec29<C>::F::mul(q.x, beta);
        }
    }
    return q;
}
template <bool COMPACT>
__device__ __forceinline__ uint32_t entry_index(uint32_t v) { return v & (COMPACT ? PAY_ENDO - 1u : 0x7FFFFFFFu); }

template <class C, bool COMPACT>
__device__ __forceinline__ xyzz29_t accumulate_part(const uint32_t *__restrict__ src, uint32_t s, uint32_t e, const affine_t *__restrict__ table,
                                                    const xyzz_t *__restrict__ init) {
    using E29 = Ec29<C>;
    using F = typename E29::F;
    bool exc = false;
    xyzz29_t acc;
    {
        uint32_t v = src[s];
        uint32_t vn = s + 1 < e ? src[s + 1] : 0u;
        affine_t p = table[entry_index<COMPACT>(v)];
        uint32_t j = s;
        if (init) {
            acc = E29::unpack(*init);
        } else {
            affine_t pn = p;
            uint32_t vnn = 0;
            if (s + 1 < e) {
                pn = table[entry_index<COMPACT>(vn)];
                if (s + 2 < e) vnn = src[s + 2];
            }
            const aff29_t q = load_entry<C, COMPACT>(p, v);
            acc.x = q.x;
            acc.y = (v >> 31) ? F::normalize(F::template neg_lazy<1, 0>(q.y)) : q.y;
            acc.zz = E29::one();
            acc.zzz = acc.zz;
            exc = F::is_zero_exact(q.y);
            v = vn;
            vn = vnn;
            p = pn;
            j = s + 1;
        }
        for (; j < e; ++j) {
            uint32_t vnn = 0;
            affine_t pn = p;
            if (j + 1 < e) {
                pn = table[entry_index<COMPACT>(vn)];
                if (j + 2 < e) vnn = src[j + 2];
            }
            acc = E29::madd_signed_fast(acc, load_entry<C, COMPACT>(p, v), (v >> 31) != 0, exc);
            v = vn;
            vn = vnn;
            p = pn;
        }
    }
    if (exc) {
        acc = init ? E29::unpack(*init) : E29::identity();
#pragma unroll 1
        for (uint32_t j = s; j < e; ++j) {
            const uint32_t v = src[j];
            acc = E29::madd_signed(acc, load_entry<C, COMPACT>(table[entry_index<COMPACT>(v)], v), (v >> 31) != 0);
        }
    }
    return acc;
}

template <class C, bool COMPACT>
__device__ __forceinline__ void accum0_thread(const uint32_t *__restrict__ sorted, size_t sorted_stride, const uint32_t *__restrict__ plan,
                                              size_t plan_stride, const uint16_t *__restrict__ tb, size_t tb_stride,
                                              const affine_t *__restrict__ table, xyzz_t *__restrict__ parts, size_t parts_stride, uint32_t l0,
                                              const Link *__restrict__ link) {
    uint32_t m = blockIdx.y;
    uint32_t t = blockIdx.x * blockDim.x + threadIdx.x;
    size_t slot;
    if (link) {
        if (t >= link->base[0][NSEG_W]) return;
        m = link_segment(link->base[0], t);
        slot = t;
        t -= link->base[0][m];
    } else {
        slot = (size_t)m * parts_stride + t;
    }
    const uint32_t *off = plan + (size_t)m * plan_stride;
    const uint32_t *tp = off + (NBUCKET + 1);
    if (t >= tp[NBUCKET]) return;
    uint32_t b = tb[link ? slot : (size_t)m * tb_stride + t];
    uint32_t part = t - tp[b];
    uint32_t s = off[b] + part * l0;
    uint32_t e = off[b + 1];
    if (e > s + l0) e = s + l0;
    const uint32_t *src = link ? sorted : sorted + (size_t)m * sorted_stride;
    using E29 = Ec29<C>;
    const xyzz29_t acc = s < e ? accumulate_part<C, COMPACT>(src, s, e, table, nullptr) : E29::identity();
    parts[slot] = E29::pack(acc);
}
template <class C>
__global__ void SRS_KERNEL_BOUNDS(ACC_THREADS, 1)
    k_accum0(const uint32_t *__restrict__ sorted, size_t sorted_stride, const uint32_t *__restrict__ plan,
             size_t plan_stride, const uint16_t *__restrict__ tb, size_t tb_stride, const affine_t *__restrict__ table,
             xyzz_t *__restrict__ parts, size_t parts_stride, uint32_t l0, const Link *__restrict__ link) {
    accum0_thread<C, false>(sorted, sorted_stride, plan, plan_stride, tb, tb_stride, table, parts, parts_stride, l0, link);
}
template <class C>
__global__ void SRS_KERNEL_BOUNDS(ACC_THREADS, 1)
    k_accum0c(const uint32_t *__restrict__ sorted, size_t sorted_stride, const uint32_t *__restrict__ plan,
              size_t plan_stride, const uint16_t *__restrict__ tb, size_t tb_stride, const affine_t *__restrict__ table,
              xyzz_t *__restrict__ parts, size_t parts_stride, uint32_t l0, const Link *__restrict__ link) {
    accum0_thread<C, true>(sorted, sorted_stride, plan, plan_stride, tb, tb_stride, table, parts, parts_stride, l0, link);
}

__device__ __forceinline__ xyzz_t shfl_down_point(const xyzz_t &p, unsigned delta) {
    xyzz_t o;
    shfl_down_words<32>(reinterpret_cast<const uint32_t *>(&p), reinterpret_cast<uint32_t *>(&o), delta, 64);
    return o;
}

__device__ __forceinline__ xyzz29_t shfl_down_point29(const xyzz29_t &p, unsigned delta, int width) {
    xyzz29_t o;
    shfl_down_words<36>(reinterpret_cast<const uint32_t *>(&p), reinterpret_cast<uint32_t *>(&o), delta, width);
    return o;
}

template <class C>
__global__ void SRS_KERNEL_BOUNDS(ACC_THREADS, 1)
    k_accum1(const xyzz_t *__restrict__ in, size_t in_stride, const uint32_t *__restrict__ plan,
             size_t plan_stride, int level, xyzz_t *__restrict__ out, size_t out_stride, uint32_t l1,
             const Link *__restrict__ link, uint32_t quad_max) {
    uint32_t m = blockIdx.y;
    const uint32_t lin = blockIdx.x * blockDim.x + threadIdx.x;
    uint32_t t;
    bool quad;
    size_t in_off, out_off;
    if (link) {
        const uint32_t n_all = link->base[level][NSEG_W];
        quad = n_all <= quad_max;
        t = quad ? (lin >> 2) : lin;
        if (t >= n_all) return;
        m = link_segment(link->base[level], t);
        t -= link->base[level][m];
        in_off = link->base[(level - 1) & 1][m];
        out_off = link->base[level & 1][m];
    } else {
        in_off = (size_t)m * in_stride;
        out_off = (size_t)m * out_stride;
    }
    if ((uint32_t)level >= plan[(size_t)m * plan_stride + plan_stride - 4]) return;
    const uint32_t *tp_prev = plan + (size_t)m * plan_stride + (size_t)level * (NBUCKET + 1);
    const uint32_t *tp = tp_prev + (NBUCKET + 1);
    const uint32_t n_out = tp[NBUCKET];
    if (!link) {
        quad = (uint64_t)n_out * gridDim.y <= quad_max;
        t = quad ? (lin >> 2) : lin;
    }
    if (t >= n_out) return;
    uint32_t b = upper_bucket(tp, t);
    uint32_t part = t - tp[b];
    uint32_t s = tp_prev[b] + part * l1;
    uint32_t e = tp_prev[b + 1];
    if (e > s + l1) e = s + l1;
    using E29 = Ec29<C>;
    const xyzz_t *src = in + in_off;
    xyzz29_t acc = E29::unpack(src[s]);
    if (quad) {
        const uint32_t q = threadIdx.x & 3u;
        for (uint32_t j = s + 1; j < e; ++j) acc = E29::add_quad(acc, E29::unpack(src[j]), q);
        if (q == 0) out[out_off + t] = E29::pack(acc);
    } else {
        for (uint32_t j = s + 1; j < e; ++j) acc = E29::add(acc, E29::unpack(src[j]));
        out[out_off + t] = E29::pack(acc);
    }
}

template <class C>
__global__ void SRS_KERNEL_BOUNDS(FINAL_THREADS, 1)
    k_accum_final(const xyzz_t *__restrict__ ping, size_t ping_stride, const xyzz_t *__restrict__ pong,
                  size_t pong_stride, const uint32_t *__restrict__ plan, size_t plan_stride,
                  xyzz_t *__restrict__ buckets, const Link *__restrict__ link) {
    uint32_t m = blockIdx.y;
    if (plan[(size_t)m * plan_stride + plan_stride - 3]) return;
    const uint32_t level = plan[(size_t)m * plan_stride + plan_stride - 4];
    const xyzz_t *in = (level & 1u) ? ping : pong;
    const size_t in_stride = (level & 1u) ? ping_stride : pong_stride;
    const uint32_t *tp = plan + (size_t)m * plan_stride + (size_t)level * (NBUCKET + 1);
    uint32_t lane = threadIdx.x & 63u;
    uint32_t b = blockIdx.x * (blockDim.x >> 6) + (threadIdx.x >> 6);
    uint32_t s = tp[b], e = tp[b + 1];
    const xyzz_t *src = in + (link ? (size_t)link->base[(level - 1u) & 1u][m] : (size_t)m * in_stride);
    xyzz_t *dst = buckets + (size_t)m * NBUCKET;
    if (e - s == 1) {
        if (lane == 0) dst[b] = src[s];
        return;
    }
    using E29 = Ec29<C>;
    xyzz29_t acc = E29::identity();
    for (uint32_t j = s + lane; j < e; j += 64) acc = E29::add(acc, E29::unpack(src[j]));
    for (unsigned d = 32; d >= 1; d >>= 1) {
        xyzz29_t other = shfl_down_point29(acc, d, 64);
        if (lane < d) acc = E29::add(acc, other);
    }
    if (lane == 0) dst[b] = E29::pack(acc);
}

template <class C, bool COMPACT>
__device__ __forceinline__ void accum0s_thread(const uint32_t *__restrict__ sorted, size_t sorted_stride, const uint32_t *__restrict__ plan,
                                               size_t plan_stride, uint32_t arr, const uint16_t *__restrict__ tb, size_t tb_stride,
                                               const affine_t *__restrict__ table, xyzz_t *__restrict__ slots, uint32_t S,
                                               const uint8_t *__restrict__ used_prev, int first, xyzz_t *__restrict__ ovf, size_t ovf_stride) {
    const uint32_t m = blockIdx.y;
    const uint32_t t = blockIdx.x * blockDim.x + threadIdx.x;
    const uint32_t *off = plan + (size_t)m * plan_stride;
    const uint32_t *tp = off + (size_t)arr * (NBUCKET + 1);
    if (t >= tp[NBUCKET]) return;
    const uint32_t *tpo = off + (NBUCKET + 1);
    const uint32_t l0 = 1u << off[plan_stride - 2];
    const uint32_t b = tb[(size_t)m * tb_stride + t];
    const uint32_t part = t - tp[b];
    uint32_t s = off[b] + part * l0;
    uint32_t e = off[b + 1];
    if (e > s + l0) e = s + l0;
    const uint32_t *src = sorted + (size_t)m * sorted_stride;
    using E29 = Ec29<C>;
    const bool regular = part < S - 1;
    xyzz_t *slot = regular ? slots + ((size_t)m * NBUCKET + b) * S + part : ovf + (size_t)m * ovf_stride + tpo[b] + (part - (S - 1));
    const bool resume = regular && !first && part < (uint32_t)used_prev[(size_t)m * NBUCKET + b];
    *slot = E29::pack(accumulate_part<C, COMPACT>(src, s, e, table, resume ? slot : nullptr));
}
template <class C>
__global__ void SRS_KERNEL_BOUNDS(ACC_THREADS, 1)
    k_accum0s(const uint32_t *__restrict__ sorted, size_t sorted_stride, const uint32_t *__restrict__ plan, size_t plan_stride, uint32_t arr,
              const uint16_t *__restrict__ tb, size_t tb_stride, const affine_t *__restrict__ table, xyzz_t *__restrict__ slots, uint32_t S,
              const uint8_t *__restrict__ used_prev, int first, xyzz_t *__restrict__ ovf, size_t ovf_stride) {
    accum0s_thread<C, false>(sorted, sorted_stride, plan, plan_stride, arr, tb, tb_stride, table, slots, S, used_prev, first, ovf, ovf_stride);
}
template <class C>
__global__ void SRS_KERNEL_BOUNDS(ACC_THREADS, 1)
    k_accum0sc(const uint32_t *__restrict__ sorted, size_t sorted_stride, const uint32_t *__restrict__ plan, size_t plan_stride, uint32_t arr,
               const uint16_t *__restrict__ tb, size_t tb_stride, const affine_t *__restrict__ table, xyzz_t *__restrict__ slots, uint32_t S,
               const uint8_t *__restrict__ used_prev, int first, xyzz_t *__restrict__ ovf, size_t ovf_stride) {
    accum0s_thread<C, true>(sorted, sorted_stride, plan, plan_stride, arr, tb, tb_stride, table, slots, S, used_prev, first, ovf, ovf_stride);
}

template <class C>
__global__ void SRS_KERNEL_BOUNDS(FINAL_THREADS, 1)
    k_ovf_final(const xyzz_t *__restrict__ ping, size_t ping_stride, const xyzz_t *__restrict__ pong, size_t pong_stride,
                const uint32_t *__restrict__ plan, size_t plan_stride, xyzz_t *__restrict__ slots, uint32_t S, int first) {
    const uint32_t m = blockIdx.y;
    const uint32_t level = plan[(size_t)m * plan_stride + plan_stride - 4];
    const xyzz_t *in = (level & 1u) ? ping + (size_t)m * ping_stride : pong + (size_t)m * pong_stride;
    const uint32_t *tp = plan + (size_t)m * plan_stride + (size_t)level * (NBUCKET + 1);
    const uint32_t lane = threadIdx.x & 63u;
    const uint32_t b = blockIdx.x * (blockDim.x >> 6) + (threadIdx.x >> 6);
    const uint32_t s = tp[b], e = tp[b + 1];
    xyzz_t *dst = slots + ((size_t)m * NBUCKET + b) * S + (S - 1);
    using E29 = Ec29<C>;
    if (e == s) {
        if (first && lane == 0) *dst = E29::pack(E29::identity());
        return;
    }
    xyzz29_t acc = E29::identity();
    for (uint32_t j = s + lane; j < e; j += 64) acc = E29::add(acc, E29::unpack(in[j]));
    for (unsigned d = 32; d >= 1; d >>= 1) {
        xyzz29_t other = shfl_down_point29(acc, d, 64);
        if (lane < d) acc = E29::add(acc, other);
    }
    if (lane == 0) {
        if (!first) acc = E29::add(acc, E29::unpack(*dst));
        *dst = E29::pack(acc);
    }
}

template <class C, bool QUAD>
__global__ void SRS_KERNEL_BOUNDS(256, 1)
    k_slot_reduce(const xyzz_t *__restrict__ in, uint32_t in_pb, const uint8_t *__restrict__ used, size_t used_stride, int extra,
                  xyzz_t *__restrict__ out, uint32_t out_pb) {
    using E29 = Ec29<C>;
    const uint32_t m = blockIdx.y;
    const uint32_t lin = blockIdx.x * blockDim.x + threadIdx.x, t = QUAD ? (lin >> 2) : lin, q = lin & 3u;
    if (t >= NBUCKET * out_pb) return;
    const uint32_t g = t / NBUCKET, b = t % NBUCKET;
    const uint32_t lim = used ? (uint32_t)used[(size_t)m * used_stride + b] : in_pb;
    const xyzz_t *src = in + ((size_t)m * NBUCKET + b) * in_pb;
    xyzz29_t acc = E29::identity();
    for (uint32_t idx = g; idx < in_pb; idx += out_pb) {
        if (!(idx < lim || (int)idx == extra)) continue;
        const xyzz29_t x = E29::unpack(src[idx]);
        if (QUAD) acc = E29::add_quad(acc, x, q); else acc = E29::add(acc, x);
    }
    if (!QUAD || q == 0) out[((size_t)m * NBUCKET + b) * out_pb + g] = E29::pack(acc);
}

template <class C>
__global__ void SRS_KERNEL_BOUNDS(64, 1)
    k_bucket_fold(const xyzz_t *__restrict__ buckets, const xyzz_t *__restrict__ ping, const xyzz_t *__restrict__ pong,
                  const uint32_t *__restrict__ plan, size_t plan_stride, xyzz_t *__restrict__ total, int first) {
    using E29 = Ec29<C>;
    const uint32_t b = blockIdx.x * blockDim.x + threadIdx.x;
    const uint32_t *hdr = plan + plan_stride - 4;
    const xyzz_t *B = hdr[1] ? ((hdr[0] & 1u) ? ping : pong) : buckets;
    if (first) {
        total[b] = B[b];
    } else {
        total[b] = E29::pack(E29::add(E29::unpack(total[b]), E29::unpack(B[b])));
    }
}

template <class C>
__device__ __forceinline__ void lds_tree_sum(xyzz_t *v, uint32_t n_pow2) {
    for (uint32_t s = n_pow2 >> 1; s >= 1; s >>= 1) {
        if (threadIdx.x < s) v[threadIdx.x] = Ec<C>::add(v[threadIdx.x], v[threadIdx.x + s]);
        __syncthreads();
    }
}

__device__ __forceinline__ xyzz_t shfl_down_point_w(const xyzz_t &p, unsigned delta, int width) {
    xyzz_t o;
    shfl_down_words<32>(reinterpret_cast<const uint32_t *>(&p), reinterpret_cast<uint32_t *>(&o), delta, width);
    return o;
}

template <class C>
__global__ void SRS_KERNEL_BOUNDS(128, 1)
    k_rowcol(const xyzz_t *__restrict__ buckets, const xyzz_t *__restrict__ ping, size_t ping_stride,
             const xyzz_t *__restrict__ pong, size_t pong_stride, const uint32_t *__restrict__ plan, size_t plan_stride,
             xyzz_t *__restrict__ rc , const Link *__restrict__ link, int from_buckets) {
    constexpr uint32_t SER = 8;
    __shared__ xyzz_t half[1];
    const uint32_t m = blockIdx.y, wave = threadIdx.x >> 6, lane = threadIdx.x & 63u;
    const uint32_t q = lane & 3u, vl = lane >> 2;
    const uint32_t *hdr = plan + (size_t)m * plan_stride + plan_stride - 4;
    const size_t ping_off = link ? (size_t)link->base[0][m] : (size_t)m * ping_stride;
    const size_t pong_off = link ? (size_t)link->base[1][m] : (size_t)m * pong_stride;
    const xyzz_t *B = (hdr[1] && !from_buckets) ? ((hdr[0] & 1u) ? ping + ping_off : pong + pong_off) : buckets + (size_t)m * NBUCKET;
    using E29 = Ec29<C>;
    xyzz_t *out = rc + (size_t)m * (RED_ROWS + RED_COLS);
    const bool is_row = blockIdx.x < RED_ROWS / 2;
    xyzz29_t acc;
    if (is_row) {
        const uint32_t hi = blockIdx.x * 2 + wave;
        const xyzz_t *src = B + (size_t)hi * RED_COLS + vl * SER;
        acc = E29::unpack(src[0]);
        xyzz_t nx = src[1];
        for (uint32_t j = 1; j < SER; ++j) {
            xyzz_t cur = nx;
            if (j + 1 < SER) nx = src[j + 1];
            acc = E29::add_quad(acc, E29::unpack(cur), q);
        }
    } else {
        const uint32_t lo = blockIdx.x - RED_ROWS / 2, sub = wave * 16 + vl;
        const xyzz_t *src = B + (size_t)(sub * SER) * RED_COLS + lo;
        acc = E29::unpack(src[0]);
        xyzz_t nx = src[RED_COLS];
        for (uint32_t j = 1; j < SER; ++j) {
            xyzz_t cur = nx;
            if (j + 1 < SER) nx = src[(size_t)(j + 1) * RED_COLS];
            acc = E29::add_quad(acc, E29::unpack(cur), q);
        }
    }
    for (unsigned d = 8; d >= 1; d >>= 1) {
        xyzz29_t o = shfl_down_point29(acc, 4 * d, 64);
        if (vl < d) acc = E29::add_quad(acc, o, q);
    }
    if (is_row) {
        if (lane == 0) out[blockIdx.x * 2 + wave] = E29::pack(acc);
        return;
    }
    if (wave == 1 && lane == 0) half[0] = E29::pack(acc);
    __syncthreads();
    if (wave == 0 && vl == 0) {
        acc = E29::add_quad(acc, E29::unpack(half[0]), q);
        if (q == 0) out[RED_ROWS + (blockIdx.x - RED_ROWS / 2)] = E29::pack(acc);
    }
}

template <class C>
__global__ void SRS_KERNEL_BOUNDS(RED_THREADS, 1)
    k_reduce_final(const xyzz_t *__restrict__ rc, xyzz_t *__restrict__ out) {
    constexpr uint32_t N = RED_COLS;
    using E29 = Ec29<C>;
    __shared__ xyzz29_t v[N];
    const uint32_t m = blockIdx.y, t = threadIdx.x >> 2, q = threadIdx.x & 3u, which = blockIdx.x;
    const xyzz_t *rows = rc + (size_t)m * (RED_ROWS + RED_COLS), *cols = rows + RED_ROWS;
    xyzz29_t x;
    if (which == 0) x = E29::add_quad(E29::unpack(rows[2 * t]), E29::unpack(rows[2 * t + 1]), q);
    else if (which == 1 || which == 3) x = E29::unpack(cols[t]);
    else x = E29::unpack(rows[2 * t + 1]);
    if (which < 2) {
        if (q == 0) v[t] = x;
        __syncthreads();
        for (uint32_t s = 1; s < N; s <<= 1) {
            const bool has = t + s < N;
            xyzz29_t o = has ? v[t + s] : E29::identity();
            __syncthreads();
            if (has) x = E29::add_quad(x, o, q);
            if (q == 0) v[t] = x;
            __syncthreads();
        }
        if (which == 0 && t == 0) x = E29::identity();
    }
    if (q == 0) v[t] = x;
    __syncthreads();
    for (uint32_t s = N >> 1; s >= 1; s >>= 1) {
        if (t < s) {
            x = E29::add_quad(x, v[t + s], q);
            if (q == 0) v[t] = x;
        }
        __syncthreads();
    }
    if (threadIdx.x == 0) out[(size_t)m * gridDim.x + which] = E29::pack(v[0]);
}

template <class C>
__global__ void SRS_KERNEL_BOUNDS(256, 1)
    k_wide_combine(const xyzz_t *__restrict__ in , xyzz_t *__restrict__ out ) {
    using E29 = Ec29<C>;
    const uint32_t which = threadIdx.x >> 6, lane = threadIdx.x & 63u, q = lane & 3u, vl = lane >> 2;
    xyzz29_t x = E29::unpack(in[vl * 4 + which]);
    if (which == 3) {
        for (uint32_t s = 1; s < NSEG_W; s <<= 1) {
            xyzz29_t o = shfl_down_point29(x, 4 * s, 64);
            if (vl + s < NSEG_W) x = E29::add_quad(x, o, q);
        }
        if (vl == 0) x = E29::identity();
    }
    for (unsigned d = NSEG_W / 2; d >= 1; d >>= 1) {
        xyzz29_t o = shfl_down_point29(x, 4 * d, 64);
        if (vl < d) x = E29::add_quad(x, o, q);
    }
    if (lane == 0) out[which] = E29::pack(x);
}

static inline uint32_t ceil_div(uint64_t a, uint64_t b) { return (uint32_t)((a + b - 1) / b); }

template <class C>
static void expand_windows(affine_t *table, uint32_t n, int nwin, int nbits, xyzz_t *tmp, hipStream_t stream) {
    for (int w = 1; w < nwin; ++w) {
        const affine_t *prev = table + (size_t)(w - 1) * n;
        affine_t *cur = table + (size_t)w * n;
        SRS_LAUNCH((k_table_step<C>), (ceil_div(n, 256)), (256), 0, stream, prev, tmp, n, nbits);
        SRS_LAUNCH((k_normalize<C>), (ceil_div(ceil_div(n, NORM_G), 128)), (128), 0, stream, (const xyzz_t *)tmp, cur, n);
    }
}

static bool wants_wide_table(size_t len) {
    static const int env_forced = [] { const char *e = std::getenv("SRS_MSM_WIDE"); return e ? std::atoi(e) : -1; }();
    const int forced = (int)tuning::get_or(tuning::MSM_WIDE, env_forced);
    if (forced == 0 || len == 0) return false;
    return forced == 1 || len >= ((size_t)1 << WIDE_MIN_KEY_LOG);
}

template <class C>
static void build_table_t(Key &k, hipStream_t stream) {
    const uint32_t n = (uint32_t)k.len;
    if (k.table_w) {
        SRS_HIP_CHECK(hipFree(k.table_w));
        k.table_w = nullptr;
    }
    if (n == 0) return;
    xyzz_t *tmp = nullptr;
    SRS_HIP_CHECK(hipMalloc((void **)&tmp, (size_t)n * sizeof(xyzz_t)));
    if (!k.compact && wants_wide_table(n) && hipMalloc((void **)&k.table_w, (size_t)n * NWIN_W * sizeof(affine_t)) != hipSuccess) {
        (void)hipGetLastError();
        k.table_w = nullptr;
    }
    if (k.table_w) {
        SRS_HIP_CHECK(hipMemcpyAsync(k.table_w, k.table, (size_t)n * sizeof(affine_t), hipMemcpyDeviceToDevice, stream));
        expand_windows<C>(k.table_w, n, NWIN_W, WBITS_W, tmp, stream);
        const size_t total_w = (size_t)n * NWIN_W;
        SRS_LAUNCH((k_table_form<C>), (ceil_div(total_w, 256)), (256), 0, stream, k.table_w, total_w);
    }
    const int nwin = k.compact ? NWIN_COMPACT : NWIN;
    expand_windows<C>(k.table, n, nwin, WBITS, tmp, stream);
    const size_t total = (size_t)n * nwin;
    SRS_LAUNCH((k_table_form<C>), (ceil_div(total, 256)), (256), 0, stream, k.table, total);
    SRS_HIP_CHECK(hipStreamSynchronize(stream));
    SRS_HIP_CHECK(hipFree(tmp));
}

template <class C>
static void generate_t(Key &k, uint64_t seed, hipStream_t stream) {
    const uint32_t n = (uint32_t)k.len;
    if (n == 0) return;
    xyzz_t *tmp = nullptr;
    SRS_HIP_CHECK(hipMalloc((void **)&tmp, (size_t)n * sizeof(xyzz_t)));
    SRS_LAUNCH((k_gen_bases<C>), (ceil_div(n, 128)), (128), 0, stream, tmp, n, seed, k.rank, k.world);
    SRS_LAUNCH((k_normalize<C>), (ceil_div(ceil_div(n, NORM_G), 128)), (128), 0, stream, (const xyzz_t *)tmp, k.table, n);
    SRS_HIP_CHECK(hipStreamSynchronize(stream));
    SRS_HIP_CHECK(hipFree(tmp));
}
void generate_bases(Key &k, uint64_t seed, hipStream_t stream) {
    if (k.curve == 0) generate_t<Bn256>(k, seed, stream); else generate_t<Grumpkin>(k, seed, stream);
}

size_t count_off_curve(const Key &k, hipStream_t stream) {
    if (k.len == 0) return 0;
    uint32_t *d_bad = nullptr, bad = 0;
    SRS_HIP_CHECK(hipMalloc((void **)&d_bad, sizeof(uint32_t)));
    SRS_HIP_CHECK(hipMemsetAsync(d_bad, 0, sizeof(uint32_t), stream));
    const uint32_t n = (uint32_t)k.len;
    if (k.curve == 0) SRS_LAUNCH((k_on_curve<Bn256>), (ceil_div(n, 256)), (256), 0, stream, (const affine_t *)k.table, n, d_bad);
    else SRS_LAUNCH((k_on_curve<Grumpkin>), (ceil_div(n, 256)), (256), 0, stream, (const affine_t *)k.table, n, d_bad);
    SRS_HIP_CHECK(hipMemcpyAsync(&bad, d_bad, sizeof(uint32_t), hipMemcpyDeviceToHost, stream));
    SRS_HIP_CHECK(hipStreamSynchronize(stream));
    (void)hipFree(d_bad);
    return bad;
}

void read_bases(const Key &k, affine_t *out_dev, hipStream_t stream) {
    if (k.len == 0) return;
    if (k.curve == 0) SRS_LAUNCH((k_table_unform<Bn256>), (ceil_div(k.len, 256)), (256), 0, stream, (const affine_t *)k.table, out_dev, k.len);
    else SRS_LAUNCH((k_table_unform<Grumpkin>), (ceil_div(k.len, 256)), (256), 0, stream, (const affine_t *)k.table, out_dev, k.len);
}

void build_table(Key &k, hipStream_t stream) {
    if (k.curve == 0) build_table_t<Bn256>(k, stream); else build_table_t<Grumpkin>(k, stream);
}

int choose_windows(Key &k) {
    k.compact = tuning::get_or(tuning::MSM_COMPACT, 0) == 1;
    if (k.compact && (uint64_t)NWIN_COMPACT * k.len > PAY_ENDO) {
        set_error("compact key (msm_compact = 1): 8 x " + std::to_string(k.len) + " table entries do not fit below the endomorphism flag (2^30)");
        throw DeviceError{4};
    }
    return k.compact ? NWIN_COMPACT : NWIN;
}
size_t table_bytes(const Key &k) {
    if (!k.table) return 0;
    return k.len * sizeof(affine_t) * ((k.compact ? NWIN_COMPACT : NWIN) + (k.table_w ? NWIN_W : 0));
}


static uint32_t l0_log_for(uint64_t M) {
    const int forced = (int)tuning::get_or(tuning::MSM_L0, 0);
    if (forced >= 1 && forced <= 7) return (uint32_t)forced;
    if (M < (1ull << 20)) return 2;
    if (M < (1ull << 22)) return 3;
    uint32_t lg = ACC_L0_LOG;
    while (lg < 7 && (M >> (lg + 1)) >= (5ull << 20)) ++lg;
    return lg;
}

static uint32_t acc1_quad_max() {
    const int64_t lg = tuning::get_or(tuning::MSM_QUAD_MAX, 0);
    return (lg >= 1 && lg <= 24) ? (1u << lg) : ACC1_QUAD_MAX;
}

static int levels_for(uint64_t parts) {
    int levels = 1;
    while (parts > FINAL_FANIN && levels < MAX_LEVELS) {
        parts = (parts + ACC_L1 - 1) / ACC_L1;
        ++levels;
    }
    return levels;
}

static bool use_two_pass(uint64_t M, uint32_t batch) {
    const int forced = (int)tuning::get_or(tuning::MSM_SORT, 0);
    if (forced == 1) return false;
    if (forced == 2) return true;
    return M * batch >= TWO_PASS_MIN_SLOTS;
}

static uint32_t slot_log() {
    const int64_t lg = tuning::get_or(tuning::MSM_SLOT_LOG, 0);
    return (lg >= 2 && lg <= 8) ? (uint32_t)lg : SLOT_LOG;
}
static uint32_t slot_want_cap() { return 4u; }

struct LevelShape {
    uint64_t M;
    int levels;
    size_t plan_stride;
    uint64_t cap0, cap1;
    uint32_t quad_max;
};
struct SetShape : LevelShape {
    bool two_pass;
    uint32_t tile, tiles;
};
struct NarrowShape : SetShape { uint32_t l0_log; };
struct SlotShape : SetShape { uint32_t S, nred; };
struct WideShape : LevelShape { uint32_t l0_log, T, tiles_g; };
// ... 53 lines not shown
};
template <class Walk>
static size_t sized(Walk walk) {
    Sizer s;
    walk(s);
    return s.used;
}
template <class Walk>
static auto carve(Arena &A, Walk walk) {
    const size_t need = sized(walk);
    A.reserve(need);
    A.reset();
    const auto bufs = walk(A);
    if (A.used != need) {
        set_error("internal: msm workspace: the arena walk and the sizer disagree");
        throw DeviceError{5};
    }
    return bufs;
}

struct SetBufs {
    xyzz_t *d_out, *ping, *pong, *rc;
    uint16_t *dig, *tb;
    uint32_t *sorted, *count, *cursor, *plan;
    uint16_t *gkey;
    uint32_t *gpay, *tile_hist;
};
struct NarrowBufs : SetBufs { xyzz_t *buckets; };
struct SlotBufs : SetBufs { xyzz_t *red_a, *red_b; };
template <class W>
static void take_set_head(W &A, const SetShape &h, uint32_t batch, SetBufs &b) {
    b.d_out = A.template take<xyzz_t>(3 * (size_t)batch);
    b.dig = A.template take<uint16_t>(h.M * batch);
    b.sorted = A.template take<uint32_t>(h.M * batch);
    b.count = A.template take<uint32_t>((size_t)NBUCKET * batch);
    b.cursor = A.template take<uint32_t>((size_t)NBUCKET * batch);
    b.plan = A.template take<uint32_t>(h.plan_stride * batch);
    b.ping = A.template take<xyzz_t>(h.cap0 * batch);
    b.tb = A.template take<uint16_t>(h.cap0 * batch);
    b.pong = A.template take<xyzz_t>(h.cap1 * batch);
}
template <class W>
static void take_set_tail(W &A, const SetShape &h, uint32_t batch, SetBufs &b) {
    b.rc = A.template take<xyzz_t>((size_t)(RED_ROWS + RED_COLS) * batch);
    b.gkey = h.two_pass ? A.template take<uint16_t>(h.M * batch) : nullptr;
    b.gpay = h.two_pass ? A.template take<uint32_t>(h.M * batch) : nullptr;
    b.tile_hist = h.two_pass ? A.template take<uint32_t>((size_t)SEG * (SORT_TARGET_BLOCKS + 2 * NWIN) * batch) : nullptr;
}
template <class W>
static NarrowBufs narrow_layout(W &A, const NarrowShape &h, uint32_t batch) {
    NarrowBufs b;
    take_set_head(A, h, batch, b);
    b.buckets = A.template take<xyzz_t>((size_t)NBUCKET * batch);
    take_set_tail(A, h, batch, b);
    return b;
}
template <class W>
static SlotBufs slot_layout(W &A, const SlotShape &h, uint32_t batch) {
    SlotBufs b;
    take_set_head(A, h, batch, b);
    b.red_a = A.template take<xyzz_t>((size_t)NBUCKET * (h.S / 8 + 1) * batch);
    b.red_b = A.template take<xyzz_t>((size_t)NBUCKET * (h.S / 64 + 1) * batch);
    take_set_tail(A, h, batch, b);
    return b;
}
struct WideBufs {
    xyzz_t *d_out, *d_seg, *ping, *pong, *buckets, *rc;
    uint16_t *gkey, *gkey2, *tb;
    uint32_t *gpay, *gpay2, *tile_cnt, *tile_hist;
    uint32_t *seg3;
    uint32_t *sorted, *count, *cursor, *plan;
    Link *link;
};
template <class W>
static WideBufs wide_layout(W &A, const WideShape &w) {
    WideBufs b;
    b.d_out = A.template take<xyzz_t>(4);
    b.d_seg = A.template take<xyzz_t>(4 * NSEG_W);
    b.gkey = A.template take<uint16_t>(w.M);
    b.gpay = A.template take<uint32_t>(w.M);
    b.sorted = A.template take<uint32_t>(w.M);
    b.tile_cnt = A.template take<uint32_t>((size_t)NSEG_W * w.T);
    b.gkey2 = A.template take<uint16_t>(w.M);
    b.gpay2 = A.template take<uint32_t>(w.M);
    b.tile_hist = A.template take<uint32_t>((size_t)SEG * w.tiles_g);
    b.seg3 = A.template take<uint32_t>(4 * (NSEG_W + 2));
    b.link = A.template take<Link>(1);
    b.count = A.template take<uint32_t>((size_t)NSEG_W * NBUCKET);
    b.cursor = A.template take<uint32_t>((size_t)NSEG_W * NBUCKET);
    b.plan = A.template take<uint32_t>(w.plan_stride * NSEG_W);
    b.ping = A.template take<xyzz_t>(w.cap0);
    b.tb = A.template take<uint16_t>(w.cap0);
    b.pong = A.template take<xyzz_t>(w.cap1);
    b.buckets = A.template take<xyzz_t>((size_t)NSEG_W * NBUCKET);
    b.rc = A.template take<xyzz_t>((size_t)NSEG_W * (RED_ROWS + RED_COLS));
    return b;
}

size_t workspace_bytes(uint32_t n_max, uint32_t batch) {
    return sized([&](auto &A) { return narrow_layout(A, narrow_shape(n_max, batch), batch); });
}
static size_t workspace_bytes_slots(uint32_t n_max, uint32_t batch) {
    return sized([&](auto &A) { return slot_layout(A, slot_shape(n_max, batch), batch); });
}
static size_t workspace_bytes_wide(uint32_t n) {
    return sized([&](auto &A) { return wide_layout(A, wide_shape(n)); });
}

template <class C, class LaunchPlan>
static void sort_front(const Key &k, const SetShape &h, const SetBufs &b, const fe_t *const *scalars_dev, const uint32_t *n_host,
                       const uint32_t *base_host, uint32_t batch, uint32_t n_max, int is_mont, hipStream_t stream, LaunchPlan launch_plan,
                       bool group_maps, uint32_t arr) {
    BatchDesc bd;
    for (uint32_t m = 0; m < BATCH_ARGS; ++m) {
        bd.ptr[m] = m < batch ? scalars_dev[m] : nullptr;
        bd.n[m] = m < batch ? n_host[m] : 0;
        bd.base[m] = (m < batch && base_host) ? base_host[m] : 0;
    }
    const uint32_t s_rank = k.compact_scalars ? 0u : k.rank, s_world = k.compact_scalars ? 1u : k.world;
    const size_t M = (size_t)h.M;
    const auto digits = k.compact ? &k_digits<C, true> : &k_digits<C, false>;
    const auto group = k.compact ? &k_group<true> : &k_group<false>;
    const auto scatter = k.compact ? &k_scatter<true> : &k_scatter<false>;
    SRS_LAUNCH(digits, (ceil_div(n_max, 256), batch), (256), 0, stream, bd, b.dig, M, is_mont, s_rank, s_world, b.count,
               (uint32_t)(NBUCKET * batch));
    SRS_LAUNCH(k_hist, (h.tiles, NWIN, batch), (SORT_THREADS), 0, stream, (const uint16_t *)b.dig, M, bd, b.count, h.tile, b.tile_hist);
    launch_plan();
    if (h.two_pass) {
        const uint32_t T1 = h.tiles * NWIN;
        SRS_LAUNCH(k_scan_seg, (SEG, batch), (1024), 0, stream, b.tile_hist, T1, (const uint32_t *)b.plan, h.plan_stride);
        SRS_LAUNCH(group, (h.tiles, NWIN, batch), (SORT_THREADS), 0, stream, (const uint16_t *)b.dig, M, bd, (const uint32_t *)b.tile_hist,
                   b.gkey, b.gpay, M, (uint32_t)k.len, h.tile, group_maps ? (const uint32_t *)b.plan : nullptr,
                   group_maps ? h.plan_stride : (size_t)0, group_maps ? b.tb : nullptr, group_maps ? (size_t)h.cap0 : (size_t)0,
                   group_maps ? arr : 0u);
        SRS_LAUNCH(k_scatter2, (8 * ceil_div(ceil_div(M, SORT_TILE2), 8), batch), (SORT_THREADS), 0, stream, (const uint16_t *)b.gkey,
                   (const uint32_t *)b.gpay, M, (const uint32_t *)b.plan, h.plan_stride, b.cursor, b.sorted, M, (uint32_t)SORT_TILE2);
    } else {
        SRS_LAUNCH(scatter, (h.tiles, NWIN, batch), (SORT_THREADS), 0, stream, (const uint16_t *)b.dig, M, bd, b.cursor, b.sorted, M,
                   (uint32_t)k.len, h.tile);
    }
    if (!(h.two_pass && group_maps))
        SRS_LAUNCH(k_expand, (NBUCKET / 4, batch), (256), 0, stream, (const uint32_t *)b.plan, h.plan_stride, b.tb, (size_t)h.cap0,
                   (const Link *)nullptr, arr);
}

struct Parts {
    const uint32_t *plan; size_t plan_stride;
    xyzz_t *ping; size_t stride0;
    xyzz_t *pong; size_t stride1;
    const Link *link;
};

template <class C>
static void accum_levels(const Parts &p, const LevelShape &h, uint64_t cap_inc, uint32_t batch, hipStream_t stream) {
    xyzz_t *cur = p.ping, *nxt = p.pong;
    size_t cur_stride = p.stride0, nxt_stride = p.stride1;
    uint64_t cap = h.cap0;
    for (int level = 1; level < h.levels; ++level) {
        cap = cap / ACC_L1 + cap_inc;
        SRS_LAUNCH((k_accum1<C>), (ceil_div(std::max<uint64_t>(cap, 4 * std::min<uint64_t>(cap, h.quad_max)), ACC_THREADS), batch),
                   (ACC_THREADS), 0, stream, (const xyzz_t *)cur, cur_stride, p.plan, h.plan_stride, level, nxt, nxt_stride, (uint32_t)ACC_L1,
                   p.link, h.quad_max);
        std::swap(cur, nxt);
        std::swap(cur_stride, nxt_stride);
    }
}

template <class C>
static void reduce_buckets(const Parts &p, uint32_t nmsm, const xyzz_t *from, int from_buckets, xyzz_t *rc, uint32_t sums, xyzz_t *d_sums,
                           hipStream_t stream) {
    SRS_LAUNCH((k_rowcol<C>), (RED_ROWS / 2 + RED_COLS, nmsm), (128), 0, stream, from, (const xyzz_t *)p.ping, p.stride0,
               (const xyzz_t *)p.pong, p.stride1, p.plan, p.plan_stride, rc, p.link, from_buckets);
    SRS_LAUNCH((k_reduce_final<C>), (sums, nmsm), (RED_THREADS), 0, stream, (const xyzz_t *)rc, d_sums);
}

static void land(Key &k, const xyzz_t *d_out, size_t n, uint32_t slot, hipStream_t stream) {
    if (!k.h_result) SRS_HIP_CHECK(hipHostMalloc(&k.h_result, 3 * (size_t)BATCH_ARGS * LANDING_SLOTS * sizeof(xyzz_t)));
    xyzz_t *dst = static_cast<xyzz_t *>(k.h_result) + 3 * (size_t)BATCH_ARGS * slot;
    SRS_HIP_CHECK(hipMemcpyAsync(dst, d_out, n * sizeof(xyzz_t), hipMemcpyDeviceToHost, stream));
}

template <class C>
static bool enqueue_t(Key &k, const fe_t *const *scalars_dev, const uint32_t *n_host, const uint32_t *base_host, uint32_t batch,
                      uint32_t n_max, int is_mont, hipStream_t stream, uint32_t slot, Fold fold) {
    if (n_max == 0) return false;
    const NarrowShape h = narrow_shape(n_max, batch);
    const NarrowBufs b = carve(k.arena, [&](auto &A) { return narrow_layout(A, h, batch); });
    sort_front<C>(k, h, b, scalars_dev, n_host, base_host, batch, n_max, is_mont, stream, [&] {
        SRS_LAUNCH(k_plan, (batch, h.levels + 1), (PLAN_THREADS), 0, stream, (const uint32_t *)b.count, b.cursor, b.plan, h.plan_stride,
                   h.levels, h.l0_log, (uint32_t)ACC_L1_LOG, (const uint32_t *)nullptr);
    }, false, 1u);
    const Parts p{b.plan, h.plan_stride, b.ping, (size_t)h.cap0, b.pong, (size_t)h.cap1, nullptr};
    const uint64_t units = std::accumulate(n_host, n_host + batch, (uint64_t)0);
    const auto accum0 = k.compact ? &k_accum0c<C> : &k_accum0<C>;
    SRS_LAUNCH_TIMED("msm_accum0", units, accum0, (ceil_div(h.cap0, ACC_THREADS), batch), (ACC_THREADS), 0, stream,
                     (const uint32_t *)b.sorted, (size_t)h.M, p.plan, p.plan_stride, (const uint16_t *)b.tb, p.stride0,
                     (const affine_t *)k.table, p.ping, p.stride0, 1u << h.l0_log, p.link);
    accum_levels<C>(p, h, NBUCKET + 1, batch, stream);
    SRS_LAUNCH((k_accum_final<C>), (NBUCKET / (FINAL_THREADS / 64), batch), (FINAL_THREADS), 0, stream, (const xyzz_t *)p.ping, p.stride0,
               (const xyzz_t *)p.pong, p.stride1, p.plan, p.plan_stride, b.buckets, p.link);
    const xyzz_t *red_from = b.buckets;
    int from_buckets = 0;
    if (fold != FOLD_NONE) {
        if (!k.fold_buckets) SRS_HIP_CHECK(hipMalloc((void **)&k.fold_buckets, (size_t)NBUCKET * sizeof(xyzz_t)));
        SRS_LAUNCH((k_bucket_fold<C>), (NBUCKET / 64), (64), 0, stream, (const xyzz_t *)b.buckets, (const xyzz_t *)p.ping,
                   (const xyzz_t *)p.pong, p.plan, p.plan_stride, k.fold_buckets, fold == FOLD_FIRST ? 1 : 0);
        if (fold != FOLD_LAST) return true;
        red_from = k.fold_buckets;
        from_buckets = 1;
    }
    reduce_buckets<C>(p, batch, red_from, from_buckets, b.rc, 3, b.d_out, stream);
    land(k, b.d_out, 3 * (size_t)batch, slot, stream);
    k.landing[slot].wide = false;
    return true;
}

static bool use_wide(const Key &k, uint32_t n_max, uint32_t batch);
static bool use_slots(const Key &k, uint32_t n_max, uint32_t batch, Fold fold) {
    const int mode = (int)tuning::get_or(tuning::MSM_SLOTS, 1);
    if (mode == 0) return false;
    if (fold != FOLD_NONE) return batch == 1;
    return mode == 2 && !use_wide(k, n_max, batch);
}

template <class C>
static bool enqueue_slots_t(Key &k, const fe_t *const *scalars_dev, const uint32_t *n_host, const uint32_t *base_host, uint32_t batch,
                            uint32_t n_max, int is_mont, hipStream_t stream, uint32_t slot, Fold fold) {
    if (n_max == 0) return false;
    const bool first = fold == FOLD_NONE || fold == FOLD_FIRST, last = fold == FOLD_NONE || fold == FOLD_LAST;
    const SlotShape h = slot_shape(n_max, batch);
    const uint32_t S = h.S;
    if (first) {
        k.slot_s = S;
        k.seq = 0;
        k.commit_ovf = k.expect_ovf;
        const size_t need = (size_t)batch * NBUCKET * S;
        if (k.slots_pts < need) {
            if (k.slots) SRS_HIP_CHECK(hipFree(k.slots));
            k.slots = nullptr;
            k.slots_pts = 0;
            SRS_HIP_CHECK(hipMalloc((void **)&k.slots, need * sizeof(xyzz_t)));
            k.slots_pts = need;
        }
        if (!k.used) SRS_HIP_CHECK(hipMalloc((void **)&k.used, 2 * (size_t)BATCH_ARGS * NBUCKET));
        if (!k.h_ovf) {
            SRS_HIP_CHECK(hipHostMalloc((void **)&k.h_ovf, 2 * (size_t)LANDING_SLOTS * BATCH_ARGS * sizeof(uint32_t)));
            for (size_t i = 0; i < 2 * (size_t)LANDING_SLOTS * BATCH_ARGS; ++i) k.h_ovf[i] = 0;
        }
    } else if (k.slot_s != S || batch != 1) {
        set_error("internal: msm slot mode: a commit's sets must share the slot layout");
        throw DeviceError{5};
    }
    const uint8_t *used_prev = k.used + (size_t)(k.seq & 1u) * BATCH_ARGS * NBUCKET;
    uint8_t *used_next = k.used + (size_t)((k.seq + 1) & 1u) * BATCH_ARGS * NBUCKET;
    ++k.seq;

    const SlotBufs b = carve(k.arena, [&](auto &A) { return slot_layout(A, h, batch); });
    const uint32_t arr = (uint32_t)h.levels + 1;
    sort_front<C>(k, h, b, scalars_dev, n_host, base_host, batch, n_max, is_mont, stream, [&] {
        SRS_LAUNCH(k_plan_s, (batch, h.levels + 2), (PLAN_THREADS), 0, stream, (const uint32_t *)b.count, b.cursor, b.plan, h.plan_stride,
                   h.levels, S, (uint32_t)ACC_L1_LOG, used_prev, used_next, first ? 1 : 0, k.h_ovf + (size_t)slot * BATCH_ARGS, slot_want_cap());
    }, true, arr);
    const Parts p{b.plan, h.plan_stride, b.ping, (size_t)h.cap0, b.pong, (size_t)h.cap1, nullptr};
    const uint64_t units = std::accumulate(n_host, n_host + batch, (uint64_t)0);
    const auto accum0s = k.compact ? &k_accum0sc<C> : &k_accum0s<C>;
    SRS_LAUNCH_TIMED("msm_accum0", units, accum0s, (ceil_div(h.cap0, ACC_THREADS), batch), (ACC_THREADS), 0, stream,
                     (const uint32_t *)b.sorted, (size_t)h.M, p.plan, p.plan_stride, arr, (const uint16_t *)b.tb, p.stride0,
                     (const affine_t *)k.table, k.slots, S, used_prev, first ? 1 : 0, p.ping, p.stride0);
    if (k.commit_ovf) {
        accum_levels<C>(p, h, NBUCKET + 1, batch, stream);
        SRS_LAUNCH((k_ovf_final<C>), (NBUCKET / (FINAL_THREADS / 64), batch), (FINAL_THREADS), 0, stream, (const xyzz_t *)p.ping, p.stride0,
                   (const xyzz_t *)p.pong, p.stride1, p.plan, p.plan_stride, k.slots, S, first ? 1 : 0);
    }
    k.landing[slot] = {false, true, k.commit_ovf, batch};
    ++k.stat_slot_sets;
    if (!last) return true;
    const xyzz_t *in = k.slots;
    uint32_t in_pb = S;
    xyzz_t *outs[2] = {b.red_a, b.red_b};
    for (uint32_t l = 0; l < h.nred; ++l) {
        const uint32_t out_pb = (in_pb + 7) / 8, n_out = NBUCKET * out_pb;
        xyzz_t *out = outs[l & 1u];
        const uint8_t *used = l == 0 ? used_next : nullptr;
        const int extra = (l == 0 && k.commit_ovf) ? (int)S - 1 : -1;
        if (l + 1 == h.nred) {
            SRS_LAUNCH((k_slot_reduce<C, true>), (ceil_div((uint64_t)n_out * 4, 256), batch), (256), 0, stream, in, in_pb, used, (size_t)NBUCKET, extra,
                       out, out_pb);
        } else {
            SRS_LAUNCH((k_slot_reduce<C, false>), (ceil_div(n_out, 256), batch), (256), 0, stream, in, in_pb, used, (size_t)NBUCKET, extra, out,
                       out_pb);
        }
        in = out;
        in_pb = out_pb;
    }
    reduce_buckets<C>(p, batch, in, 1, b.rc, 3, b.d_out, stream);
    land(k, b.d_out, 3 * (size_t)batch, slot, stream);
    return true;
}

bool overflow_missed(const Key &k, uint32_t slot) {
    if (slot >= LANDING_SLOTS || !k.landing[slot].slot_mode || k.landing[slot].ovf_on || !k.h_ovf) return false;
    for (uint32_t m = 0; m < k.landing[slot].batch; ++m)
        if (k.h_ovf[(size_t)slot * BATCH_ARGS + m]) return true;
    return false;
}
void note_commit(Key &k, const uint32_t *slots_used, uint32_t n_slots, uint64_t scalars) {
    bool any = false, slot_sets = false;
    uint64_t entries = 0;
    for (uint32_t i = 0; i < n_slots; ++i) {
        const uint32_t sl = slots_used[i];
        if (sl >= LANDING_SLOTS || !k.landing[sl].slot_mode || !k.h_ovf) continue;
        slot_sets = true;
        for (uint32_t m = 0; m < k.landing[sl].batch; ++m) entries += k.h_ovf[(size_t)(LANDING_SLOTS + sl) * BATCH_ARGS + m];
        bool hot = false;
        for (uint32_t m = 0; m < k.landing[sl].batch; ++m) hot = hot || k.h_ovf[(size_t)sl * BATCH_ARGS + m] != 0;
        if (hot) ++k.stat_hot_sets;
        any = any || hot;
    }
    constexpr uint32_t COLD_COMMITS = 3;
    if (!slot_sets) {
        k.last_entries = k.last_scalars = 0;
        return;
    }
    k.last_entries = entries;
    k.last_scalars = scalars;
    if (any) {
        k.expect_ovf = true;
        k.cold_streak = 0;
    } else if (k.expect_ovf && ++k.cold_streak >= COLD_COMMITS) {
        k.expect_ovf = false;
        k.cold_streak = 0;
    }
}

static bool use_wide(const Key &k, uint32_t n_max, uint32_t batch) {
    const int min_log = (int)tuning::get_or(tuning::MSM_WIDE_MIN, (int64_t)WIDE_MIN_N_LOG);
    return k.table_w != nullptr && batch == 1 && n_max >= (1u << min_log);
}

template <class C>
static bool enqueue_wide_t(Key &k, const fe_t *scalars_dev, uint32_t n, uint32_t base, int is_mont, hipStream_t stream, uint32_t slot) {
    const WideShape w = wide_shape(n);
    const WideBufs b = carve(k.arena, [&](auto &A) { return wide_layout(A, w); });
    uint32_t *seg_total = b.seg3, *seg_off = b.seg3 + (NSEG_W + 2), *tile_base = b.seg3 + 2 * (NSEG_W + 2), *tile_base2 = b.seg3 + 3 * (NSEG_W + 2);

    WideDesc wd;
    wd.ptr = scalars_dev;
    wd.n = n;
    wd.base = base;
    wd.rank = k.compact_scalars ? 0u : k.rank;
    wd.world = k.compact_scalars ? 1u : k.world;
    wd.is_mont = is_mont;
    const uint32_t table_stride = (uint32_t)k.len;

    SRS_HIP_CHECK(hipMemsetAsync(seg_total, 0, (NSEG_W + 1) * sizeof(uint32_t), stream));
    SRS_HIP_CHECK(hipMemsetAsync(b.count, 0, (size_t)NSEG_W * NBUCKET * sizeof(uint32_t), stream));
    SRS_LAUNCH((k_seg_pass<C, false>), (w.T), (WIDE_THREADS), 0, stream, wd, b.tile_cnt, w.T, seg_total, (uint16_t *)nullptr,
               (uint32_t *)nullptr, table_stride);
    const uint32_t small_tiles = (w.M >> 19) < 64 ? 1u : 0u, tile2_host = small_tiles ? SORT_TILE2 / 4 : SORT_TILE2;
    SRS_LAUNCH(k_seg_scan, (NSEG_W), (1024), 0, stream, b.tile_cnt, w.T, (const uint32_t *)seg_total, seg_off, tile_base, tile_base2, small_tiles);
    SRS_LAUNCH((k_seg_pass<C, true>), (w.T), (WIDE_THREADS), 0, stream, wd, b.tile_cnt, w.T, seg_total, b.gkey, b.gpay, table_stride);
    SRS_LAUNCH(k_hist_g, (w.tiles_g), (SORT_THREADS), 0, stream, (const uint16_t *)b.gkey, (const uint32_t *)seg_off,
               (const uint32_t *)tile_base, b.count, b.tile_hist);
    SRS_LAUNCH(k_plan, (NSEG_W, w.levels + 1), (PLAN_THREADS), 0, stream, (const uint32_t *)b.count, b.cursor, b.plan, w.plan_stride, w.levels,
               w.l0_log, (uint32_t)ACC_L1_LOG, (const uint32_t *)seg_off);
    SRS_LAUNCH(k_scan_seg_g, (SEG, NSEG_W), (1024), 0, stream, b.tile_hist, w.tiles_g, (const uint32_t *)tile_base, (const uint32_t *)b.plan,
               w.plan_stride);
    SRS_LAUNCH(k_group_g, (w.tiles_g), (SORT_THREADS), 0, stream, (const uint16_t *)b.gkey, (const uint32_t *)b.gpay, (const uint32_t *)seg_off,
               (const uint32_t *)tile_base, (const uint32_t *)b.tile_hist, b.gkey2, b.gpay2);
    SRS_LAUNCH(k_scatter2_g, (8 * ceil_div(ceil_div(w.M, tile2_host) + NSEG_W, 8)), (SORT_THREADS), 0, stream, (const uint16_t *)b.gkey2,
               (const uint32_t *)b.gpay2, (const uint32_t *)seg_off, (const uint32_t *)tile_base2, b.cursor, b.sorted);
    SRS_LAUNCH(k_link, (1), (64), 0, stream, (const uint32_t *)b.plan, w.plan_stride, w.levels, b.link);
    const Parts p{b.plan, w.plan_stride, b.ping, 0, b.pong, 0, b.link};
    SRS_LAUNCH(k_expand, (NBUCKET / 4, NSEG_W), (256), 0, stream, p.plan, p.plan_stride, b.tb, (size_t)0, p.link, 1u);
    SRS_LAUNCH_TIMED("msm_accum0", n, (k_accum0<C>), (ceil_div(w.cap0, ACC_THREADS)), (ACC_THREADS), 0, stream, (const uint32_t *)b.sorted,
                     (size_t)0, p.plan, p.plan_stride, (const uint16_t *)b.tb, (size_t)0, (const affine_t *)k.table_w, p.ping, (size_t)0,
                     1u << w.l0_log, p.link);
    accum_levels<C>(p, w, (uint64_t)NSEG_W * (NBUCKET + 1), 1, stream);
    SRS_LAUNCH((k_accum_final<C>), (NBUCKET / (FINAL_THREADS / 64), NSEG_W), (FINAL_THREADS), 0, stream, (const xyzz_t *)p.ping, p.stride0,
               (const xyzz_t *)p.pong, p.stride1, p.plan, p.plan_stride, b.buckets, p.link);
    reduce_buckets<C>(p, NSEG_W, b.buckets, 0, b.rc, 4, b.d_seg, stream);
    SRS_LAUNCH((k_wide_combine<C>), (1), (256), 0, stream, (const xyzz_t *)b.d_seg, b.d_out);
    land(k, b.d_out, 4, slot, stream);
    k.landing[slot].wide = true;
    return true;
}

template <class C>
static void finish_t(Key &k, uint32_t batch, uint32_t slot, bool launched, xyzz_t *result_host) {
    if (!launched) {
        for (uint32_t m = 0; m < batch; ++m) result_host[m] = Ec<C>::identity();
        return;
    }
    const xyzz_t *raw = static_cast<const xyzz_t *>(k.h_result) + 3 * (size_t)BATCH_ARGS * slot;
    using F = typename C::F;
    fe_t c = F::one();
    for (int d = 0; d < 5; ++d) c = F::halve(c);
    std::vector<xyzz_t> two(3 * (size_t)batch + (k.landing[slot].wide ? 1 : 0));
    for (size_t i = 0; i < two.size(); ++i) {
        two[i].x = F::mul(raw[i].x, c);
        two[i].y = F::mul(raw[i].y, c);
        two[i].zz = F::mul(raw[i].zz, c);
        two[i].zzz = F::mul(raw[i].zzz, c);
    }
    for (uint32_t m = 0; m < batch; ++m) {
        xyzz_t a = Ec<C>::add(Ec<C>::dbl(two[3 * m]), two[3 * m + 2]);
        for (uint32_t j = 1; j < RED_COLS; j <<= 1) a = Ec<C>::dbl(a);
        result_host[m] = Ec<C>::add(a, two[3 * m + 1]);
    }
    if (k.landing[slot].wide) {
        xyzz_t u = two[3];
        for (uint32_t j = 1; j < NBUCKET; j <<= 1) u = Ec<C>::dbl(u);
        result_host[0] = Ec<C>::add(result_host[0], u);
    }
}

bool enqueue(Key &k, const fe_t *const *scalars_dev, const uint32_t *n_host, const uint32_t *base_host, uint32_t batch, int is_mont,
             hipStream_t stream, uint32_t slot, Fold fold) {
    if (batch > BATCH_ARGS || slot >= LANDING_SLOTS) {
        set_error("internal: msm::enqueue batch / slot out of range");
        throw DeviceError{5};
    }
    if (fold != FOLD_NONE && batch != 1) {
        set_error("internal: msm::enqueue fold needs one MSM per set");
        throw DeviceError{5};
    }
    if (batch == 1 && fold == FOLD_NONE && use_wide(k, n_host[0], 1)) {
        const uint32_t base = base_host ? base_host[0] : 0;
        k.landing[slot].slot_mode = false;
        ++k.stat_other_sets;
        return k.curve == 0 ? enqueue_wide_t<Bn256>(k, scalars_dev[0], n_host[0], base, is_mont, stream, slot)
                            : enqueue_wide_t<Grumpkin>(k, scalars_dev[0], n_host[0], base, is_mont, stream, slot);
    }
    uint32_t n_max = 0;
    for (uint32_t m = 0; m < batch; ++m) n_max = std::max(n_max, n_host[m]);
    const bool first = fold == FOLD_NONE || fold == FOLD_FIRST;
    const bool slots = first ? use_slots(k, n_max, batch, fold) : k.slot_s != 0;
    if (slots)
        return k.curve == 0 ? enqueue_slots_t<Bn256>(k, scalars_dev, n_host, base_host, batch, n_max, is_mont, stream, slot, fold)
                            : enqueue_slots_t<Grumpkin>(k, scalars_dev, n_host, base_host, batch, n_max, is_mont, stream, slot, fold);
    if (first) k.slot_s = 0;
    k.landing[slot].slot_mode = false;
    ++k.stat_other_sets;
    return k.curve == 0 ? enqueue_t<Bn256>(k, scalars_dev, n_host, base_host, batch, n_max, is_mont, stream, slot, fold)
                        : enqueue_t<Grumpkin>(k, scalars_dev, n_host, base_host, batch, n_max, is_mont, stream, slot, fold);
}
void finish(Key &k, uint32_t batch, uint32_t slot, bool launched, xyzz_t *result_host) {
    if (k.curve == 0) finish_t<Bn256>(k, batch, slot, launched, result_host); else finish_t<Grumpkin>(k, batch, slot, launched, result_host);
}
void reserve(Key &k, uint32_t n_max, uint32_t batch) {
    size_t b = use_wide(k, n_max, batch) ? std::max(workspace_bytes_wide(n_max), workspace_bytes(n_max, batch)) : workspace_bytes(n_max, batch);
    if (batch == 1) b = std::max(b, workspace_bytes_slots(n_max, batch));
    k.arena.reserve(b);
}

void release(Key &k) {
    if (k.table_w) (void)hipFree(k.table_w);
    k.table_w = nullptr;
    if (k.fold_buckets) (void)hipFree(k.fold_buckets);
    k.fold_buckets = nullptr;
    if (k.h_result) (void)hipHostFree(k.h_result);
    k.h_result = nullptr;
    if (k.slots) (void)hipFree(k.slots);
    k.slots = nullptr;
    k.slots_pts = 0;
    if (k.used) (void)hipFree(k.used);
    k.used = nullptr;
    if (k.h_ovf) (void)hipHostFree(k.h_ovf);
    k.h_ovf = nullptr;
    k.arena.release();
}

void run(Key &k, const fe_t *const *scalars_dev, const uint32_t *n_host, uint32_t batch, int is_mont,
         hipStream_t stream, xyzz_t *result_host) {
    for (uint32_t at = 0; at < batch;) {
        uint32_t b = std::min<uint32_t>(BATCH_ARGS, batch - at);
        if (use_wide(k, n_host[at], 1)) b = 1;
        bool launched = enqueue(k, scalars_dev + at, n_host + at, nullptr, b, is_mont, stream, 0);
        if (launched) {
            SRS_HIP_CHECK(hipStreamSynchronize(stream));
            SRS_HIP_CHECK(hipGetLastError());
            const uint32_t sl = 0;
            if (overflow_missed(k, sl)) {
                k.expect_ovf = true;
                ++k.stat_redo;
                launched = enqueue(k, scalars_dev + at, n_host + at, nullptr, b, is_mont, stream, 0);
                SRS_HIP_CHECK(hipStreamSynchronize(stream));
                SRS_HIP_CHECK(hipGetLastError());
            }
            uint64_t total = 0;
            for (uint32_t m = 0; m < b; ++m) total += n_host[at + m];
            note_commit(k, &sl, 1, total);
        }
        finish(k, b, 0, launched, result_host + at);
        prof::collect();
        at += b;
    }
}

}
}
```

Measured before the change: 98.62.

## Use fast incomplete point addition with exception-triggered complete recompute in MSM reductions

Adds an add_quad_fast variant that skips the doubling and equal-point handling of the complete quad-lane XYZZ addition and raises an exception flag when the inputs would need it. The MSM accumulation, slot reduction, row/column and final reduction kernels run the fast path first and redo the work with the complete formula only when the flag is set, and a device counter records how many recomputes occur. k_rowcol is also restructured to 512 threads with less serial work per thread, and a recompute-count API is exposed. This is meant to cut per-addition arithmetic and branching in the hot bucket-reduction path. The cost is extra atomics, block-wide syncs and, on rare exceptions, duplicated work.

New measurement: 94.53. 0.958x the previous value.

```diff
diff --git a/include/sirius_amd.h b/include/sirius_amd.h
--- a/include/sirius_amd.h
+++ b/include/sirius_amd.h
@@ -83,6 +83,7 @@
 int srs_ck_setup_synthetic_multi(int curve, size_t len, uint64_t seed, int n_devices, srs_ck **out);
 int srs_ck_num_shards(const srs_ck *ck);
 int srs_ck_msm_stats(const srs_ck *ck, uint64_t *out4);
+int srs_ck_msm_recomputes(const srs_ck *ck, uint64_t *out);
 int srs_ck_has_wide_table(const srs_ck *ck);
 int srs_ck_is_compact(const srs_ck *ck);
 size_t srs_ck_table_bytes(const srs_ck *ck);
diff --git a/shim/src/sys.rs b/shim/src/sys.rs
--- a/shim/src/sys.rs
+++ b/shim/src/sys.rs
@@ -81,6 +81,7 @@
     pub fn srs_ck_setup_synthetic_multi(curve: c_int, len: usize, seed: u64, n_devices: c_int, out: *mut *mut srs_ck) -> c_int;
     pub fn srs_ck_num_shards(ck: *const srs_ck) -> c_int;
     pub fn srs_ck_msm_stats(ck: *const srs_ck, out4: *mut u64) -> c_int;
+    pub fn srs_ck_msm_recomputes(ck: *const srs_ck, out: *mut u64) -> c_int;
     pub fn srs_ck_has_wide_table(ck: *const srs_ck) -> c_int;
     pub fn srs_ck_is_compact(ck: *const srs_ck) -> c_int;
     pub fn srs_ck_table_bytes(ck: *const srs_ck) -> usize;
diff --git a/sirius_amd/_lib.py b/sirius_amd/_lib.py
--- a/sirius_amd/_lib.py
+++ b/sirius_amd/_lib.py
@@ -47,6 +47,7 @@
         "srs_ck_setup_synthetic_multi": (i32, [i32, sz, C.c_uint64, i32, C.POINTER(vp)]),
         "srs_ck_num_shards": (i32, [vp]),
         "srs_ck_msm_stats": (i32, [vp, C.POINTER(C.c_uint64)]),
+        "srs_ck_msm_recomputes": (i32, [vp, C.POINTER(C.c_uint64)]),
         "srs_ck_has_wide_table": (i32, [vp]),
         "srs_ck_is_compact": (i32, [vp]),
         "srs_ck_table_bytes": (sz, [vp]),
diff --git a/sirius_amd/commitment.py b/sirius_amd/commitment.py
--- a/sirius_amd/commitment.py
+++ b/sirius_amd/commitment.py
@@ -101,6 +101,11 @@
         out = (C.c_uint64 * 4)()
         L.check(L.lib().srs_ck_msm_stats(self._h, out))
         return dict(slot_sets=int(out[0]), hot_sets=int(out[1]), redo=int(out[2]), other_sets=int(out[3]))
+
+    def msm_recomputes(self):
+        out = C.c_uint64()
+        L.check(L.lib().srs_ck_msm_recomputes(self._h, C.byref(out)))
+        return int(out.value)
 
     def shard_stats(self, shard):
         out = (C.c_uint64 * 4)()
diff --git a/sirius_amd/csrc/capi.hip b/sirius_amd/csrc/capi.hip
--- a/sirius_amd/csrc/capi.hip
+++ b/sirius_amd/csrc/capi.hip
@@ -800,6 +800,15 @@
     if (ck->shards.empty()) add(ck->key);
     for (const auto &sh : ck->shards) add(sh->key);
     return SRS_OK;
+}
+
+int srs_ck_msm_recomputes(const srs_ck *ck, uint64_t *out) {
+    if (!ck || !out) return fail(SRS_ERR_INVALID, "srs_ck_msm_recomputes: bad argument");
+    return guarded([&]() -> int {
+        *out = ck->shards.empty() ? msm::recomputes(ck->key) : 0;
+        for (const auto &sh : ck->shards) *out += msm::recomputes(sh->key);
+        return SRS_OK;
+    });
 }
 
 int srs_ck_shard_stats(const srs_ck *ck, int shard, uint64_t *out) {
diff --git a/sirius_amd/csrc/curve29.cuh b/sirius_amd/csrc/curve29.cuh
--- a/sirius_amd/csrc/curve29.cuh
+++ b/sirius_amd/csrc/curve29.cuh
@@ -307,6 +307,37 @@
         return o;
     }
 
+    SRS_D static xyzz29_t add_quad_fast(const xyzz29_t &a, const xyzz29_t &b, uint32_t q, bool &exc) {
+        const bool ia = is_identity(a), ib = is_identity(b);
+        xyzz29_t o;
+        if (ia || ib) {
+            o.x = F::select(ib, a.x, b.x);
+            o.y = F::select(ib, a.y, b.y);
+            o.zz = F::select(ib, a.zz, b.zz);
+            o.zzz = F::select(ib, a.zzz, b.zzz);
+            return o;
+        }
+        const f29_t m1 = F::mul(quad_select29(q, a.x, b.x, a.y, b.y), quad_select29(q, b.zz, a.zz, b.zzz, a.zzz));
+        const f29_t u1 = quad_bcast29<0>(m1), u2 = quad_bcast29<1>(m1), s1 = quad_bcast29<2>(m1), s2 = quad_bcast29<3>(m1);
+        const f29_t p = F::normalize(F::template sub_lazy<3, 0>(u2, u1)), r = F::normalize(F::template sub_lazy<3, 0>(s2, s1));
+        const f29_t m2 = F::mul(quad_select29(q, p, r, a.zz, a.zzz), quad_select29(q, p, r, b.zz, b.zzz));
+        const f29_t pp = quad_bcast29<0>(m2), rr = quad_bcast29<1>(m2), zzz12 = quad_bcast29<3>(m2);
+        exc = exc || F::is_zero_mod(pp);
+        const f29_t m3 = F::mul(quad_select29(q, p, u1, m2, p), pp);
+        const f29_t ppp = quad_bcast29<0>(m3), qv = quad_bcast29<1>(m3);
+        o.zz = quad_bcast29<2>(m3);
+        o.x = F::normalize(F::template sub_lazy<7, 2>(rr, F::add_lazy(ppp, F::add_lazy(qv, qv))));
+        const f29_t m4 = F::mul(quad_select29(q, F::template sub_lazy<10, 0>(qv, o.x), s1, zzz12, s1), quad_select29(q, r, ppp, ppp, ppp));
+        o.y = F::template sub_lazy<3, 0>(quad_bcast29<0>(m4), quad_bcast29<1>(m4));
+        o.zzz = quad_bcast29<2>(m4);
+        return o;
+    }
+    template <bool FAST>
+    SRS_D static xyzz29_t add_quad_as(const xyzz29_t &a, const xyzz29_t &b, uint32_t q, bool &exc) {
+        if (FAST) return add_quad_fast(a, b, q, exc);
+        return add_quad(a, b, q);
+    }
+
     SRS_HD static xyzz_t to_xyzz(const xyzz29_t &a) {
         f29_t c;
 #pragma unroll
diff --git a/sirius_amd/csrc/msm.h b/sirius_amd/csrc/msm.h
--- a/sirius_amd/csrc/msm.h
+++ b/sirius_amd/csrc/msm.h
@@ -76,10 +76,12 @@
     bool commit_ovf = false;
     bool expect_ovf = expect_ovf_initial();
     uint32_t cold_streak = 0;
+    uint32_t *recomputes = nullptr;
 };
 
 int choose_windows(Key &k);
 void build_table(Key &k, hipStream_t stream);
+uint64_t recomputes(const Key &k);
 size_t table_bytes(const Key &k);
 void release(Key &k);
 void generate_bases(Key &k, uint64_t seed, hipStream_t stream);
diff --git a/sirius_amd/csrc/msm.hip b/sirius_amd/csrc/msm.hip
--- a/sirius_amd/csrc/msm.hip
+++ b/sirius_amd/csrc/msm.hip
@@ -1087,7 +1087,7 @@
 
 template <class C, bool COMPACT>
 __device__ __forceinline__ xyzz29_t accumulate_part(const uint32_t *__restrict__ src, uint32_t s, uint32_t e, const affine_t *__restrict__ table,
-                                                    const xyzz_t *__restrict__ init) {
+                                                    const xyzz_t *__restrict__ init, uint32_t *__restrict__ redo) {
     using E29 = Ec29<C>;
     using F = typename E29::F;
     bool exc = false;
@@ -1131,6 +1131,7 @@
         }
     }
     if (exc) {
+        atomicAdd(redo, 1u);
         acc = init ? E29::unpack(*init) : E29::identity();
 #pragma unroll 1
         for (uint32_t j = s; j < e; ++j) {
@@ -1145,7 +1146,7 @@
 __device__ __forceinline__ void accum0_thread(const uint32_t *__restrict__ sorted, size_t sorted_stride, const uint32_t *__restrict__ plan,
                                               size_t plan_stride, const uint16_t *__restrict__ tb, size_t tb_stride,
                                               const affine_t *__restrict__ table, xyzz_t *__restrict__ parts, size_t parts_stride, uint32_t l0,
-                                              const Link *__restrict__ link) {
+                                              const Link *__restrict__ link, uint32_t *__restrict__ redo) {
     uint32_t m = blockIdx.y;
     uint32_t t = blockIdx.x * blockDim.x + threadIdx.x;
     size_t slot;
@@ -1167,22 +1168,22 @@
     if (e > s + l0) e = s + l0;
     const uint32_t *src = link ? sorted : sorted + (size_t)m * sorted_stride;
     using E29 = Ec29<C>;
-    const xyzz29_t acc = s < e ? accumulate_part<C, COMPACT>(src, s, e, table, nullptr) : E29::identity();
+    const xyzz29_t acc = s < e ? accumulate_part<C, COMPACT>(src, s, e, table, nullptr, redo) : E29::identity();
     parts[slot] = E29::pack(acc);
 }
 template <class C>
 __global__ void SRS_KERNEL_BOUNDS(ACC_THREADS, 1)
     k_accum0(const uint32_t *__restrict__ sorted, size_t sorted_stride, const uint32_t *__restrict__ plan,
              size_t plan_stride, const uint16_t *__restrict__ tb, size_t tb_stride, const affine_t *__restrict__ table,
-             xyzz_t *__restrict__ parts, size_t parts_stride, uint32_t l0, const Link *__restrict__ link) {
-    accum0_thread<C, false>(sorted, sorted_stride, plan, plan_stride, tb, tb_stride, table, parts, parts_stride, l0, link);
+             xyzz_t *__restrict__ parts, size_t parts_stride, uint32_t l0, const Link *__restrict__ link, uint32_t *__restrict__ redo) {
+    accum0_thread<C, false>(sorted, sorted_stride, plan, plan_stride, tb, tb_stride, table, parts, parts_stride, l0, link, redo);
 }
 template <class C>
 __global__ void SRS_KERNEL_BOUNDS(ACC_THREADS, 1)
     k_accum0c(const uint32_t *__restrict__ sorted, size_t sorted_stride, const uint32_t *__restrict__ plan,
               size_t plan_stride, const uint16_t *__restrict__ tb, size_t tb_stride, const affine_t *__restrict__ table,
-              xyzz_t *__restrict__ parts, size_t parts_stride, uint32_t l0, const Link *__restrict__ link) {
-    accum0_thread<C, true>(sorted, sorted_stride, plan, plan_stride, tb, tb_stride, table, parts, parts_stride, l0, link);
+              xyzz_t *__restrict__ parts, size_t parts_stride, uint32_t l0, const Link *__restrict__ link, uint32_t *__restrict__ redo) {
+    accum0_thread<C, true>(sorted, sorted_stride, plan, plan_stride, tb, tb_stride, table, parts, parts_stride, l0, link, redo);
 }
 
 __device__ __forceinline__ xyzz_t shfl_down_point(const xyzz_t &p, unsigned delta) {
@@ -1197,11 +1198,41 @@
     return o;
 }
 
+template <class C, bool FAST>
+__device__ __forceinline__ xyzz29_t wave_tree_sum(xyzz29_t x, uint32_t n, uint32_t vl, uint32_t q, bool &exc) {
+    for (uint32_t d = n >> 1; d >= 1; d >>= 1) {
+        const xyzz29_t o = shfl_down_point29(x, 4 * d, 64);
+        if (vl < d) x = Ec29<C>::template add_quad_as<FAST>(x, o, q, exc);
+    }
+    return x;
+}
+template <class C, bool FAST>
+__device__ __forceinline__ xyzz29_t wave_suffix_scan(xyzz29_t x, uint32_t n, uint32_t vl, uint32_t q, bool &exc) {
+    for (uint32_t s = 1; s < n; s <<= 1) {
+        const xyzz29_t o = shfl_down_point29(x, 4 * s, 64);
+        if (vl + s < n) x = Ec29<C>::template add_quad_as<FAST>(x, o, q, exc);
+    }
+    return x;
+}
+template <class Body>
+__device__ __forceinline__ void fast_then_complete(uint32_t *redo, Body body) {
+    __shared__ uint32_t flagged;
+    if (threadIdx.x == 0) flagged = 0;
+    __syncthreads();
+    bool exc = false;
+    body(std::true_type{}, exc);
+    if (exc) flagged = 1;
+    __syncthreads();
+    if (!flagged) return;
+    if (threadIdx.x == 0) atomicAdd(redo, 1u);
+    body(std::false_type{}, exc);
+}
+
 template <class C>
 __global__ void SRS_KERNEL_BOUNDS(ACC_THREADS, 1)
     k_accum1(const xyzz_t *__restrict__ in, size_t in_stride, const uint32_t *__restrict__ plan,
              size_t plan_stride, int level, xyzz_t *__restrict__ out, size_t out_stride, uint32_t l1,
-             const Link *__restrict__ link, uint32_t quad_max) {
+             const Link *__restrict__ link, uint32_t quad_max, uint32_t *__restrict__ redo) {
     uint32_t m = blockIdx.y;
     const uint32_t lin = blockIdx.x * blockDim.x + threadIdx.x;
     uint32_t t;
@@ -1239,7 +1270,14 @@
     xyzz29_t acc = E29::unpack(src[s]);
     if (quad) {
         const uint32_t q = threadIdx.x & 3u;
-        for (uint32_t j = s + 1; j < e; ++j) acc = E29::add_quad(acc, E29::unpack(src[j]), q);
+        bool exc = false;
+        for (uint32_t j = s + 1; j < e; ++j) acc = E29::add_quad_fast(acc, E29::unpack(src[j]), q, exc);
+        if (exc) {
+            acc = E29::unpack(src[s]);
+#pragma unroll 1
+            for (uint32_t j = s + 1; j < e; ++j) acc = E29::add_quad(acc, E29::unpack(src[j]), q);
+            if (q == 0) atomicAdd(redo, 1u);
+        }
         if (q == 0) out[out_off + t] = E29::pack(acc);
     } else {
         for (uint32_t j = s + 1; j < e; ++j) acc = E29::add(acc, E29::unpack(src[j]));
@@ -1281,7 +1319,8 @@
 __device__ __forceinline__ void accum0s_thread(const uint32_t *__restrict__ sorted, size_t sorted_stride, const uint32_t *__restrict__ plan,
                                                size_t plan_stride, uint32_t arr, const uint16_t *__restrict__ tb, size_t tb_stride,
                                                const affine_t *__restrict__ table, xyzz_t *__restrict__ slots, uint32_t S,
-                                               const uint8_t *__restrict__ used_prev, int first, xyzz_t *__restrict__ ovf, size_t ovf_stride) {
+                                               const uint8_t *__restrict__ used_prev, int first, xyzz_t *__restrict__ ovf, size_t ovf_stride,
+                                               uint32_t *__restrict__ redo) {
     const uint32_t m = blockIdx.y;
     const uint32_t t = blockIdx.x * blockDim.x + threadIdx.x;
     const uint32_t *off = plan + (size_t)m * plan_stride;
@@ -1299,21 +1338,21 @@
     const bool regular = part < S - 1;
     xyzz_t *slot = regular ? slots + ((size_t)m * NBUCKET + b) * S + part : ovf + (size_t)m * ovf_stride + tpo[b] + (part - (S - 1));
     const bool resume = regular && !first && part < (uint32_t)used_prev[(size_t)m * NBUCKET + b];
-    *slot = E29::pack(accumulate_part<C, COMPACT>(src, s, e, table, resume ? slot : nullptr));
+    *slot = E29::pack(accumulate_part<C, COMPACT>(src, s, e, table, resume ? slot : nullptr, redo));
 }
 template <class C>
 __global__ void SRS_KERNEL_BOUNDS(ACC_THREADS, 1)
     k_accum0s(const uint32_t *__restrict__ sorted, size_t sorted_stride, const uint32_t *__restrict__ plan, size_t plan_stride, uint32_t arr,
               const uint16_t *__restrict__ tb, size_t tb_stride, const affine_t *__restrict__ table, xyzz_t *__restrict__ slots, uint32_t S,
-              const uint8_t *__restrict__ used_prev, int first, xyzz_t *__restrict__ ovf, size_t ovf_stride) {
-    accum0s_thread<C, false>(sorted, sorted_stride, plan, plan_stride, arr, tb, tb_stride, table, slots, S, used_prev, first, ovf, ovf_stride);
+              const uint8_t *__restrict__ used_prev, int first, xyzz_t *__restrict__ ovf, size_t ovf_stride, uint32_t *__restrict__ redo) {
+    accum0s_thread<C, false>(sorted, sorted_stride, plan, plan_stride, arr, tb, tb_stride, table, slots, S, used_prev, first, ovf, ovf_stride, redo);
 }
 template <class C>
 __global__ void SRS_KERNEL_BOUNDS(ACC_THREADS, 1)
     k_accum0sc(const uint32_t *__restrict__ sorted, size_t sorted_stride, const uint32_t *__restrict__ plan, size_t plan_stride, uint32_t arr,
                const uint16_t *__restrict__ tb, size_t tb_stride, const affine_t *__restrict__ table, xyzz_t *__restrict__ slots, uint32_t S,
-               const uint8_t *__restrict__ used_prev, int first, xyzz_t *__restrict__ ovf, size_t ovf_stride) {
-    accum0s_thread<C, true>(sorted, sorted_stride, plan, plan_stride, arr, tb, tb_stride, table, slots, S, used_prev, first, ovf, ovf_stride);
+               const uint8_t *__restrict__ used_prev, int first, xyzz_t *__restrict__ ovf, size_t ovf_stride, uint32_t *__restrict__ redo) {
+    accum0s_thread<C, true>(sorted, sorted_stride, plan, plan_stride, arr, tb, tb_stride, table, slots, S, used_prev, first, ovf, ovf_stride, redo);
 }
 
 template <class C>
@@ -1348,7 +1387,7 @@
 template <class C, bool QUAD>
 __global__ void SRS_KERNEL_BOUNDS(256, 1)
     k_slot_reduce(const xyzz_t *__restrict__ in, uint32_t in_pb, const uint8_t *__restrict__ used, size_t used_stride, int extra,
-                  xyzz_t *__restrict__ out, uint32_t out_pb) {
+                  xyzz_t *__restrict__ out, uint32_t out_pb, uint32_t *__restrict__ redo) {
     using E29 = Ec29<C>;
     const uint32_t m = blockIdx.y;
     const uint32_t lin = blockIdx.x * blockDim.x + threadIdx.x, t = QUAD ? (lin >> 2) : lin, q = lin & 3u;
@@ -1357,10 +1396,18 @@
     const uint32_t lim = used ? (uint32_t)used[(size_t)m * used_stride + b] : in_pb;
     const xyzz_t *src = in + ((size_t)m * NBUCKET + b) * in_pb;
     xyzz29_t acc = E29::identity();
+    bool exc = false;
     for (uint32_t idx = g; idx < in_pb; idx += out_pb) {
         if (!(idx < lim || (int)idx == extra)) continue;
         const xyzz29_t x = E29::unpack(src[idx]);
-        if (QUAD) acc = E29::add_quad(acc, x, q); else acc = E29::add(acc, x);
+        if (QUAD) acc = E29::add_quad_fast(acc, x, q, exc); else acc = E29::add(acc, x);
+    }
+    if (QUAD && exc) {
+        acc = E29::identity();
+#pragma unroll 1
+        for (uint32_t idx = g; idx < in_pb; idx += out_pb)
+            if (idx < lim || (int)idx == extra) acc = E29::add_quad(acc, E29::unpack(src[idx]), q);
+        if (q == 0) atomicAdd(redo, 1u);
     }
     if (!QUAD || q == 0) out[((size_t)m * NBUCKET + b) * out_pb + g] = E29::pack(acc);
 }
@@ -1394,13 +1441,15 @@
     return o;
 }
 
-template <class C>
-__global__ void SRS_KERNEL_BOUNDS(128, 1)
+constexpr uint32_t RC_THREADS = 512, RC_SER = 2;
+static_assert(RED_COLS == 4 * 16 * RC_SER && RED_ROWS == 8 * 16 * RC_SER && RC_THREADS == 8 * 64, "k_rowcol: 4 wavefronts per row, 8 per column");
+template <class C>
+__global__ void SRS_KERNEL_BOUNDS(RC_THREADS, 1)
     k_rowcol(const xyzz_t *__restrict__ buckets, const xyzz_t *__restrict__ ping, size_t ping_stride,
              const xyzz_t *__restrict__ pong, size_t pong_stride, const uint32_t *__restrict__ plan, size_t plan_stride,
-             xyzz_t *__restrict__ rc , const Link *__restrict__ link, int from_buckets) {
-    constexpr uint32_t SER = 8;
-    __shared__ xyzz_t half[1];
+             xyzz_t *__restrict__ rc , const Link *__restrict__ link, int from_buckets,
+             uint32_t *__restrict__ redo) {
+    __shared__ xyzz29_t part[RC_THREADS / 64];
     const uint32_t m = blockIdx.y, wave = threadIdx.x >> 6, lane = threadIdx.x & 63u;
     const uint32_t q = lane & 3u, vl = lane >> 2;
     const uint32_t *hdr = plan + (size_t)m * plan_stride + plan_stride - 4;
@@ -1410,99 +1459,97 @@
     using E29 = Ec29<C>;
     xyzz_t *out = rc + (size_t)m * (RED_ROWS + RED_COLS);
     const bool is_row = blockIdx.x < RED_ROWS / 2;
-    xyzz29_t acc;
+    const uint32_t group = is_row ? 4u : 8u, first = wave & ~(group - 1u);
+    const xyzz_t *src;
+    size_t step;
+    xyzz_t *dst;
     if (is_row) {
-        const uint32_t hi = blockIdx.x * 2 + wave;
-        const xyzz_t *src = B + (size_t)hi * RED_COLS + vl * SER;
-        acc = E29::unpack(src[0]);
-        xyzz_t nx = src[1];
-        for (uint32_t j = 1; j < SER; ++j) {
-            xyzz_t cur = nx;
-            if (j + 1 < SER) nx = src[j + 1];
-            acc = E29::add_quad(acc, E29::unpack(cur), q);
-        }
+        const uint32_t hi = blockIdx.x * 2 + (wave >> 2);
+        src = B + (size_t)hi * RED_COLS + ((wave & 3u) * 16 + vl) * RC_SER;
+        step = 1;
+        dst = out + hi;
     } else {
-        const uint32_t lo = blockIdx.x - RED_ROWS / 2, sub = wave * 16 + vl;
-        const xyzz_t *src = B + (size_t)(sub * SER) * RED_COLS + lo;
-        acc = E29::unpack(src[0]);
-        xyzz_t nx = src[RED_COLS];
-        for (uint32_t j = 1; j < SER; ++j) {
-            xyzz_t cur = nx;
-            if (j + 1 < SER) nx = src[(size_t)(j + 1) * RED_COLS];
-            acc = E29::add_quad(acc, E29::unpack(cur), q);
-        }
-    }
-    for (unsigned d = 8; d >= 1; d >>= 1) {
-        xyzz29_t o = shfl_down_point29(acc, 4 * d, 64);
-        if (vl < d) acc = E29::add_quad(acc, o, q);
-    }
-    if (is_row) {
-        if (lane == 0) out[blockIdx.x * 2 + wave] = E29::pack(acc);
-        return;
-    }
-    if (wave == 1 && lane == 0) half[0] = E29::pack(acc);
-    __syncthreads();
-    if (wave == 0 && vl == 0) {
-        acc = E29::add_quad(acc, E29::unpack(half[0]), q);
-        if (q == 0) out[RED_ROWS + (blockIdx.x - RED_ROWS / 2)] = E29::pack(acc);
-    }
+        const uint32_t lo = blockIdx.x - RED_ROWS / 2;
+        src = B + (size_t)((wave * 16 + vl) * RC_SER) * RED_COLS + lo;
+        step = RED_COLS;
+        dst = out + RED_ROWS + lo;
+    }
+    fast_then_complete(redo, [&](auto fast, bool &exc) {
+        constexpr bool FAST = decltype(fast)::value;
+        xyzz_t el[RC_SER];
+#pragma unroll
+        for (uint32_t j = 0; j < RC_SER; ++j) el[j] = src[j * step];
+        xyzz29_t acc = E29::unpack(el[0]);
+#pragma unroll
+        for (uint32_t j = 1; j < RC_SER; ++j) acc = E29::template add_quad_as<FAST>(acc, E29::unpack(el[j]), q, exc);
+        acc = wave_tree_sum<C, FAST>(acc, 16, vl, q, exc);
+        if (lane == 0) part[wave] = acc;
+        __syncthreads();
+        if (wave == first) {
+            xyzz29_t x = vl < group ? part[first + vl] : E29::identity();
+            x = wave_tree_sum<C, FAST>(x, group, vl, q, exc);
+            if (lane == 0) *dst = E29::pack(x);
+        }
+    });
 }
 
 template <class C>
 __global__ void SRS_KERNEL_BOUNDS(RED_THREADS, 1)
-    k_reduce_final(const xyzz_t *__restrict__ rc, xyzz_t *__restrict__ out) {
-    constexpr uint32_t N = RED_COLS;
+    k_reduce_final(const xyzz_t *__restrict__ rc, xyzz_t *__restrict__ out, uint32_t *__restrict__ redo) {
+    constexpr uint32_t NW = RED_THREADS / 64;
+    static_assert(RED_COLS == NW * 16, "k_reduce_final: one quad per element");
     using E29 = Ec29<C>;
-    __shared__ xyzz29_t v[N];
+    __shared__ xyzz29_t tot[NW], behind[NW], sum[NW];
     const uint32_t m = blockIdx.y, t = threadIdx.x >> 2, q = threadIdx.x & 3u, which = blockIdx.x;
+    const uint32_t wave = t >> 4, vl = t & 15u;
     const xyzz_t *rows = rc + (size_t)m * (RED_ROWS + RED_COLS), *cols = rows + RED_ROWS;
-    xyzz29_t x;
-    if (which == 0) x = E29::add_quad(E29::unpack(rows[2 * t]), E29::unpack(rows[2 * t + 1]), q);
-    else if (which == 1 || which == 3) x = E29::unpack(cols[t]);
-    else x = E29::unpack(rows[2 * t + 1]);
-    if (which < 2) {
-        if (q == 0) v[t] = x;
+    xyzz_t *dst = out + (size_t)m * gridDim.x + which;
+    fast_then_complete(redo, [&](auto fast, bool &exc) {
+        constexpr bool FAST = decltype(fast)::value;
+        xyzz29_t x;
+        if (which == 0) x = E29::template add_quad_as<FAST>(E29::unpack(rows[2 * t]), E29::unpack(rows[2 * t + 1]), q, exc);
+        else if (which == 1 || which == 3) x = E29::unpack(cols[t]);
+        else x = E29::unpack(rows[2 * t + 1]);
+        if (which < 2) {
+            x = wave_suffix_scan<C, FAST>(x, 16, vl, q, exc);
+            if (vl == 0 && q == 0) tot[wave] = x;
+            __syncthreads();
+            if (wave == 0) {
+                xyzz29_t u = vl < NW ? tot[vl] : E29::identity();
+                u = wave_suffix_scan<C, FAST>(u, NW, vl, q, exc);
+                if (vl < NW && q == 0) behind[vl] = u;
+            }
+            __syncthreads();
+            if (wave + 1 < NW) x = E29::template add_quad_as<FAST>(x, behind[wave + 1], q, exc);
+            if (which == 0 && t == 0) x = E29::identity();
+        }
+        x = wave_tree_sum<C, FAST>(x, 16, vl, q, exc);
+        if (vl == 0 && q == 0) sum[wave] = x;
         __syncthreads();
-        for (uint32_t s = 1; s < N; s <<= 1) {
-            const bool has = t + s < N;
-            xyzz29_t o = has ? v[t + s] : E29::identity();
-            __syncthreads();
-            if (has) x = E29::add_quad(x, o, q);
-            if (q == 0) v[t] = x;
-            __syncthreads();
-        }
-        if (which == 0 && t == 0) x = E29::identity();
-    }
-    if (q == 0) v[t] = x;
-    __syncthreads();
-    for (uint32_t s = N >> 1; s >= 1; s >>= 1) {
-        if (t < s) {
-            x = E29::add_quad(x, v[t + s], q);
-            if (q == 0) v[t] = x;
-        }
-        __syncthreads();
-    }
-    if (threadIdx.x == 0) out[(size_t)m * gridDim.x + which] = E29::pack(v[0]);
+        if (wave == 0) {
+            xyzz29_t y = vl < NW ? sum[vl] : E29::identity();
+            y = wave_tree_sum<C, FAST>(y, NW, vl, q, exc);
+            if (threadIdx.x == 0) *dst = E29::pack(y);
+        }
+    });
 }
 
 template <class C>
 __global__ void SRS_KERNEL_BOUNDS(256, 1)
-    k_wide_combine(const xyzz_t *__restrict__ in , xyzz_t *__restrict__ out ) {
+    k_wide_combine(const xyzz_t *__restrict__ in , xyzz_t *__restrict__ out , uint32_t *__restrict__ redo) {
+    static_assert(NSEG_W == 16, "k_wide_combine: one quad per segment, one wavefront per sum");
     using E29 = Ec29<C>;
     const uint32_t which = threadIdx.x >> 6, lane = threadIdx.x & 63u, q = lane & 3u, vl = lane >> 2;
-    xyzz29_t x = E29::unpack(in[vl * 4 + which]);
-    if (which == 3) {
-        for (uint32_t s = 1; s < NSEG_W; s <<= 1) {
-            xyzz29_t o = shfl_down_point29(x, 4 * s, 64);
-            if (vl + s < NSEG_W) x = E29::add_quad(x, o, q);
-        }
-        if (vl == 0) x = E29::identity();
-    }
-    for (unsigned d = NSEG_W / 2; d >= 1; d >>= 1) {
-        xyzz29_t o = shfl_down_point29(x, 4 * d, 64);
-        if (vl < d) x = E29::add_quad(x, o, q);
-    }
-    if (lane == 0) out[which] = E29::pack(x);
+    fast_then_complete(redo, [&](auto fast, bool &exc) {
+        constexpr bool FAST = decltype(fast)::value;
+        xyzz29_t x = E29::unpack(in[vl * 4 + which]);
+        if (which == 3) {
+            x = wave_suffix_scan<C, FAST>(x, NSEG_W, vl, q, exc);
+            if (vl == 0) x = E29::identity();
+        }
+        x = wave_tree_sum<C, FAST>(x, NSEG_W, vl, q, exc);
+        if (lane == 0) out[which] = E29::pack(x);
+    });
 }
 
 static inline uint32_t ceil_div(uint64_t a, uint64_t b) { return (uint32_t)((a + b - 1) / b); }
@@ -1862,7 +1909,7 @@
 };
 
 template <class C>
-static void accum_levels(const Parts &p, const LevelShape &h, uint64_t cap_inc, uint32_t batch, hipStream_t stream) {
+static void accum_levels(const Parts &p, const LevelShape &h, uint64_t cap_inc, uint32_t batch, uint32_t *redo, hipStream_t stream) {
     xyzz_t *cur = p.ping, *nxt = p.pong;
     size_t cur_stride = p.stride0, nxt_stride = p.stride1;
     uint64_t cap = h.cap0;
@@ -1870,7 +1917,7 @@
         cap = cap / ACC_L1 + cap_inc;
         SRS_LAUNCH((k_accum1<C>), (ceil_div(std::max<uint64_t>(cap, 4 * std::min<uint64_t>(cap, h.quad_max)), ACC_THREADS), batch),
                    (ACC_THREADS), 0, stream, (const xyzz_t *)cur, cur_stride, p.plan, h.plan_stride, level, nxt, nxt_stride, (uint32_t)ACC_L1,
-                   p.link, h.quad_max);
+                   p.link, h.quad_max, redo);
         std::swap(cur, nxt);
         std::swap(cur_stride, nxt_stride);
     }
@@ -1878,10 +1925,23 @@
 
 template <class C>
 static void reduce_buckets(const Parts &p, uint32_t nmsm, const xyzz_t *from, int from_buckets, xyzz_t *rc, uint32_t sums, xyzz_t *d_sums,
-                           hipStream_t stream) {
-    SRS_LAUNCH((k_rowcol<C>), (RED_ROWS / 2 + RED_COLS, nmsm), (128), 0, stream, from, (const xyzz_t *)p.ping, p.stride0,
-               (const xyzz_t *)p.pong, p.stride1, p.plan, p.plan_stride, rc, p.link, from_buckets);
-    SRS_LAUNCH((k_reduce_final<C>), (sums, nmsm), (RED_THREADS), 0, stream, (const xyzz_t *)rc, d_sums);
+                           uint32_t *redo, hipStream_t stream) {
+    SRS_LAUNCH((k_rowcol<C>), (RED_ROWS / 2 + RED_COLS, nmsm), (RC_THREADS), 0, stream, from, (const xyzz_t *)p.ping, p.stride0,
+               (const xyzz_t *)p.pong, p.stride1, p.plan, p.plan_stride, rc, p.link, from_buckets, redo);
+    SRS_LAUNCH((k_reduce_final<C>), (sums, nmsm), (RED_THREADS), 0, stream, (const xyzz_t *)rc, d_sums, redo);
+}
+
+static uint32_t *recompute_counter(Key &k, hipStream_t stream) {
+    if (!k.recomputes) {
+        SRS_HIP_CHECK(hipMalloc((void **)&k.recomputes, sizeof(uint32_t)));
+        SRS_HIP_CHECK(hipMemsetAsync(k.recomputes, 0, sizeof(uint32_t), stream));
+    }
+    return k.recomputes;
+}
+uint64_t recomputes(const Key &k) {
+    uint32_t v = 0;
+    if (k.recomputes) SRS_HIP_CHECK(hipMemcpy(&v, k.recomputes, sizeof(v), hipMemcpyDeviceToHost));
+    return v;
 }
 
 static void land(Key &k, const xyzz_t *d_out, size_t n, uint32_t slot, hipStream_t stream) {
@@ -1901,12 +1961,13 @@
                    h.levels, h.l0_log, (uint32_t)ACC_L1_LOG, (const uint32_t *)nullptr);
     }, false, 1u);
     const Parts p{b.plan, h.plan_stride, b.ping, (size_t)h.cap0, b.pong, (size_t)h.cap1, nullptr};
+    uint32_t *const redo = recompute_counter(k, stream);
     const uint64_t units = std::accumulate(n_host, n_host + batch, (uint64_t)0);
     const auto accum0 = k.compact ? &k_accum0c<C> : &k_accum0<C>;
     SRS_LAUNCH_TIMED("msm_accum0", units, accum0, (ceil_div(h.cap0, ACC_THREADS), batch), (ACC_THREADS), 0, stream,
                      (const uint32_t *)b.sorted, (size_t)h.M, p.plan, p.plan_stride, (const uint16_t *)b.tb, p.stride0,
-                     (const affine_t *)k.table, p.ping, p.stride0, 1u << h.l0_log, p.link);
-    accum_levels<C>(p, h, NBUCKET + 1, batch, stream);
+                     (const affine_t *)k.table, p.ping, p.stride0, 1u << h.l0_log, p.link, redo);
+    accum_levels<C>(p, h, NBUCKET + 1, batch, redo, stream);
     SRS_LAUNCH((k_accum_final<C>), (NBUCKET / (FINAL_THREADS / 64), batch), (FINAL_THREADS), 0, stream, (const xyzz_t *)p.ping, p.stride0,
                (const xyzz_t *)p.pong, p.stride1, p.plan, p.plan_stride, b.buckets, p.link);
     const xyzz_t *red_from = b.buckets;
@@ -1919,7 +1980,7 @@
         red_from = k.fold_buckets;
         from_buckets = 1;
     }
-    reduce_buckets<C>(p, batch, red_from, from_buckets, b.rc, 3, b.d_out, stream);
+    reduce_buckets<C>(p, batch, red_from, from_buckets, b.rc, 3, b.d_out, redo, stream);
     land(k, b.d_out, 3 * (size_t)batch, slot, stream);
     k.landing[slot].wide = false;
     return true;
@@ -1972,13 +2033,14 @@
                    h.levels, S, (uint32_t)ACC_L1_LOG, used_prev, used_next, first ? 1 : 0, k.h_ovf + (size_t)slot * BATCH_ARGS, slot_want_cap());
     }, true, arr);
     const Parts p{b.plan, h.plan_stride, b.ping, (size_t)h.cap0, b.pong, (size_t)h.cap1, nullptr};
+    uint32_t *const redo = recompute_counter(k, stream);
     const uint64_t units = std::accumulate(n_host, n_host + batch, (uint64_t)0);
     const auto accum0s = k.compact ? &k_accum0sc<C> : &k_accum0s<C>;
     SRS_LAUNCH_TIMED("msm_accum0", units, accum0s, (ceil_div(h.cap0, ACC_THREADS), batch), (ACC_THREADS), 0, stream,
                      (const uint32_t *)b.sorted, (size_t)h.M, p.plan, p.plan_stride, arr, (const uint16_t *)b.tb, p.stride0,
-                     (const affine_t *)k.table, k.slots, S, used_prev, first ? 1 : 0, p.ping, p.stride0);
+                     (const affine_t *)k.table, k.slots, S, used_prev, first ? 1 : 0, p.ping, p.stride0, redo);
     if (k.commit_ovf) {
-        accum_levels<C>(p, h, NBUCKET + 1, batch, stream);
+        accum_levels<C>(p, h, NBUCKET + 1, batch, redo, stream);
         SRS_LAUNCH((k_ovf_final<C>), (NBUCKET / (FINAL_THREADS / 64), batch), (FINAL_THREADS), 0, stream, (const xyzz_t *)p.ping, p.stride0,
                    (const xyzz_t *)p.pong, p.stride1, p.plan, p.plan_stride, k.slots, S, first ? 1 : 0);
     }
@@ -1995,15 +2057,15 @@
         const int extra = (l == 0 && k.commit_ovf) ? (int)S - 1 : -1;
         if (l + 1 == h.nred) {
             SRS_LAUNCH((k_slot_reduce<C, true>), (ceil_div((uint64_t)n_out * 4, 256), batch), (256), 0, stream, in, in_pb, used, (size_t)NBUCKET, extra,
-                       out, out_pb);
+                       out, out_pb, redo);
         } else {
             SRS_LAUNCH((k_slot_reduce<C, false>), (ceil_div(n_out, 256), batch), (256), 0, stream, in, in_pb, used, (size_t)NBUCKET, extra, out,
-                       out_pb);
+                       out_pb, redo);
         }
         in = out;
         in_pb = out_pb;
     }
-    reduce_buckets<C>(p, batch, in, 1, b.rc, 3, b.d_out, stream);
+    reduce_buckets<C>(p, batch, in, 1, b.rc, 3, b.d_out, redo, stream);
     land(k, b.d_out, 3 * (size_t)batch, slot, stream);
     return true;
 }
@@ -2082,15 +2144,16 @@
                (const uint32_t *)b.gpay2, (const uint32_t *)seg_off, (const uint32_t *)tile_base2, b.cursor, b.sorted);
     SRS_LAUNCH(k_link, (1), (64), 0, stream, (const uint32_t *)b.plan, w.plan_stride, w.levels, b.link);
     const Parts p{b.plan, w.plan_stride, b.ping, 0, b.pong, 0, b.link};
+    uint32_t *const redo = recompute_counter(k, stream);
     SRS_LAUNCH(k_expand, (NBUCKET / 4, NSEG_W), (256), 0, stream, p.plan, p.plan_stride, b.tb, (size_t)0, p.link, 1u);
     SRS_LAUNCH_TIMED("msm_accum0", n, (k_accum0<C>), (ceil_div(w.cap0, ACC_THREADS)), (ACC_THREADS), 0, stream, (const uint32_t *)b.sorted,
                      (size_t)0, p.plan, p.plan_stride, (const uint16_t *)b.tb, (size_t)0, (const affine_t *)k.table_w, p.ping, (size_t)0,
-                     1u << w.l0_log, p.link);
-    accum_levels<C>(p, w, (uint64_t)NSEG_W * (NBUCKET + 1), 1, stream);
+                     1u << w.l0_log, p.link, redo);
+    accum_levels<C>(p, w, (uint64_t)NSEG_W * (NBUCKET + 1), 1, redo, stream);
     SRS_LAUNCH((k_accum_final<C>), (NBUCKET / (FINAL_THREADS / 64), NSEG_W), (FINAL_THREADS), 0, stream, (const xyzz_t *)p.ping, p.stride0,
                (const xyzz_t *)p.pong, p.stride1, p.plan, p.plan_stride, b.buckets, p.link);
-    reduce_buckets<C>(p, NSEG_W, b.buckets, 0, b.rc, 4, b.d_seg, stream);
-    SRS_LAUNCH((k_wide_combine<C>), (1), (256), 0, stream, (const xyzz_t *)b.d_seg, b.d_out);
+    reduce_buckets<C>(p, NSEG_W, b.buckets, 0, b.rc, 4, b.d_seg, redo, stream);
+    SRS_LAUNCH((k_wide_combine<C>), (1), (256), 0, stream, (const xyzz_t *)b.d_seg, b.d_out, redo);
     land(k, b.d_out, 4, slot, stream);
     k.landing[slot].wide = true;
     return true;
@@ -2176,6 +2239,8 @@
     k.slots_pts = 0;
     if (k.used) (void)hipFree(k.used);
     k.used = nullptr;
+    if (k.recomputes) (void)hipFree(k.recomputes);
+    k.recomputes = nullptr;
     if (k.h_ovf) (void)hipHostFree(k.h_ovf);
     k.h_ovf = nullptr;
     k.arena.release();
```
